# olehskip/resnet.c

Measured on AMD Instinct MI355X. Metric: images/sec ResNet-50 224x224 fp32 batch=256, higher is better.
Workload: dtype f32; 1 GPU; resnet50 fp32 forward, batch 256 per GPU, 224x224 (BASELINE.json configs[2]); global_batch=256, batch_per_gpu=256, mode=fused conv+bn+relu(+add) epilogues, streams_per_gpu=2, streams_configured=library default, front_parts=1, parallelism=batch split over 1 GPU(s), weights replicated, no collective

## Files before the change

### include/rn_hip.h

```cpp
#ifndef RN_HIP_H
#define RN_HIP_H

#include <stddef.h>
#include <stdint.h>

#ifdef __cplusplus
extern "C" {
#endif

#if defined(__GNUC__)
#define RN_API __attribute__((visibility("default")))
#else
#define RN_API
#endif

typedef struct rn_ctx rn_ctx;
typedef struct rn_model rn_model;
typedef struct rn_event rn_event;

enum {
    RN_OK = 0,
    RN_ERR_INVALID = 1,
    RN_ERR_HIP = 2,
    RN_ERR_IO = 3,
    RN_ERR_NOMEM = 4,
    RN_ERR_UNSUPPORTED = 5
};

enum { RN_LAYOUT_NCHW = 0, RN_LAYOUT_NHWC = 1 };

enum { RN_DTYPE_F32 = 0, RN_DTYPE_BF16 = 1 };

enum {
    RN_FWD_REFERENCE_OPS = 0,
    RN_FWD_FUSED = 1
};

RN_API int rn_ctx_create(rn_ctx **out, int device, void *hip_stream );
RN_API int rn_ctx_destroy(rn_ctx *ctx);
RN_API int rn_ctx_set_layout(rn_ctx *ctx, int layout);
RN_API int rn_ctx_get_layout(const rn_ctx *ctx);
RN_API int rn_ctx_set_sync_each_op(rn_ctx *ctx, int on);
RN_API int rn_ctx_set_deferred(rn_ctx *ctx, int on);
RN_API int rn_ctx_get_deferred(const rn_ctx *ctx);
RN_API int rn_flush(rn_ctx *ctx);
RN_API int rn_observe(rn_ctx *ctx, const void *dev_ptr);
RN_API int rn_ctx_deferred_stats(const rn_ctx *ctx, uint64_t *pending_ops, uint64_t *nhwc_buffers,
                                 uint64_t *fused_launches, uint64_t *literal_launches,
                                 uint64_t *transposes);
RN_API int rn_ctx_set_weight_cache(rn_ctx *ctx, int on);
RN_API uint64_t rn_ctx_launch_count(const rn_ctx *ctx);
RN_API int rn_conv_tile_candidates(void);
RN_API int rn_ctx_set_conv_tile(rn_ctx *ctx, int candidate);
RN_API int rn_ctx_set_split_k(rn_ctx *ctx, int max_splits);
RN_API int rn_ctx_set_stem_items(rn_ctx *ctx, int items);
RN_API int rn_ctx_set_xcd_groups(rn_ctx *ctx, int groups);
RN_API int rn_ctx_set_nchw_taps(rn_ctx *ctx, int mode);
RN_API int rn_ctx_set_tap_skip(rn_ctx *ctx, int mode);
RN_API int rn_ctx_tap_skip_stats(const rn_ctx *ctx, uint64_t *launches, uint64_t *k_tiles_skipped);
RN_API int rn_conv_tap_skip_plan(int dtype, uint64_t B, uint64_t in_channels, uint64_t out_channels, uint64_t H,
                                 uint64_t W, uint64_t kernel_size, uint64_t stride, uint64_t padding,
                                 uint64_t dilation, int tile, uint64_t *m_tiles, uint64_t *k_tiles,
                                 uint64_t *k_tiles_skipped, int *rule);
RN_API int rn_ctx_set_debug_stamps(rn_ctx *ctx, void *dev_buffer);
RN_API void *rn_ctx_stream(rn_ctx *ctx);
RN_API int rn_ctx_device(const rn_ctx *ctx);
RN_API int rn_sync(rn_ctx *ctx);
RN_API const char *rn_last_error(const rn_ctx *ctx);
RN_API const char *rn_status_string(int status);
RN_API int rn_device_count(int *count);
RN_API int rn_device_locality(int device, char *pci_bus_id, uint64_t pci_cap, int *numa_node,
                              char *cpulist, uint64_t cpulist_cap);
RN_API const char *rn_version(void);

RN_API int rn_malloc(rn_ctx *ctx, void **dev_ptr, uint64_t bytes);
RN_API int rn_free(rn_ctx *ctx, void *dev_ptr);
RN_API int rn_memcpy_h2d(rn_ctx *ctx, void *dev_dst, const void *host_src, uint64_t bytes);
RN_API int rn_memcpy_d2h(rn_ctx *ctx, void *host_dst, const void *dev_src, uint64_t bytes);
RN_API int rn_memcpy_d2d(rn_ctx *ctx, void *dev_dst, const void *dev_src, uint64_t bytes);
RN_API int rn_memset(rn_ctx *ctx, void *dev_ptr, int byte_value, uint64_t bytes);
RN_API int rn_load_f32_file(rn_ctx *ctx, const char *path, float **dev_ptr, uint64_t *numel);
RN_API int rn_save_f32_file(rn_ctx *ctx, const char *path, const float *dev_ptr, uint64_t numel);

RN_API int rn_event_create(rn_ctx *ctx, rn_event **out);
RN_API int rn_event_destroy(rn_event *ev);
RN_API int rn_event_record(rn_ctx *ctx, rn_event *ev);
RN_API int rn_event_elapsed_ms(rn_event *start, rn_event *stop, float *ms);

RN_API uint64_t rn_conv_output_size(uint64_t x, uint64_t kernel_size, uint64_t stride,
                                    uint64_t padding);
RN_API int rn_conv2d_forward(rn_ctx *ctx, const float *inp, float *out, const float *weight,
                             uint64_t kernel_size, uint64_t stride, uint64_t padding,
                             uint64_t h_out, uint64_t w_out, uint64_t B, uint64_t in_channels,
                             uint64_t out_channels, uint64_t H, uint64_t W);
RN_API int rn_maxpool2d_forward(rn_ctx *ctx, const float *inp, float *out, uint64_t kernel_size,
                                uint64_t stride, uint64_t padding, uint64_t h_out, uint64_t w_out,
                                uint64_t B, uint64_t channels, uint64_t H, uint64_t W);
RN_API int rn_avgpool2d_forward(rn_ctx *ctx, const float *inp, float *out, uint64_t kernel_size,
                                uint64_t stride, uint64_t padding, uint64_t h_out, uint64_t w_out,
                                uint64_t B, uint64_t channels, uint64_t H, uint64_t W);
RN_API int rn_linear_forward(rn_ctx *ctx, const float *inp, float *out, const float *weight,
                             const float *bias , uint64_t B, uint64_t in_features,
                             uint64_t out_features);
RN_API int rn_relu_forward(rn_ctx *ctx, const float *inp, float *out, uint64_t N);
RN_API int rn_batchnorm2d_forward(rn_ctx *ctx, const float *inp, float *out, const float *weight,
                                  const float *bias, const float *mean, const float *var,
                                  uint64_t B, uint64_t C, uint64_t N);
RN_API int rn_add_forward(rn_ctx *ctx, const float *inp1, const float *inp2, float *out,
                          uint64_t N);
RN_API int rn_argmax_forward(rn_ctx *ctx, const float *logits, uint64_t *idx, uint64_t B,
                             uint64_t classes);

RN_API int rn_softmax_forward(rn_ctx *ctx, const float *logits, float *probs, uint64_t B, uint64_t classes);
RN_API int rn_topk_forward(rn_ctx *ctx, const float *x, float *values, uint64_t *indices, uint64_t B,
                           uint64_t classes, uint64_t k);
RN_API int rn_softmax_topk_forward(rn_ctx *ctx, const float *logits, float *probs , float *topk_prob,
                                   uint64_t *topk_idx, uint64_t B, uint64_t classes, uint64_t k);

RN_API int rn_nchw_to_nhwc(rn_ctx *ctx, const float *src, float *dst, uint64_t B, uint64_t C,
                           uint64_t H, uint64_t W);
RN_API int rn_nhwc_to_nchw(rn_ctx *ctx, const float *src, float *dst, uint64_t B, uint64_t C,
                           uint64_t H, uint64_t W);
RN_API int rn_nhwc_to_nchw_dt(rn_ctx *ctx, int dtype, const void *src_nhwc, float *dst_nchw, uint64_t B,
                              uint64_t C, uint64_t H, uint64_t W);
RN_API uint64_t rn_conv2d_input_channels(uint64_t in_channels);
RN_API int rn_nchw_to_nhwc_pad(rn_ctx *ctx, const float *src, float *dst, uint64_t B, uint64_t C,
                               uint64_t H, uint64_t W, uint64_t Cpad);
RN_API uint64_t rn_conv2d_packed_weight_numel(uint64_t in_channels, uint64_t out_channels,
                                              uint64_t kernel_size);
RN_API int rn_conv2d_pack_weight(rn_ctx *ctx, const float *weight_oihw, float *packed,
                                 uint64_t in_channels, uint64_t out_channels,
                                 uint64_t kernel_size);
RN_API int rn_batchnorm2d_fold(rn_ctx *ctx, const float *weight, const float *bias,
                               const float *mean, const float *var, float *scale, float *shift,
                               uint64_t C);

typedef struct rn_epilogue {
    const float *scale;
    const float *shift;
    const void *residual;
    int relu;
} rn_epilogue;

RN_API int rn_conv2d_nhwc_forward(rn_ctx *ctx, const float *inp, float *out,
                                  const float *packed_weight, uint64_t kernel_size,
                                  uint64_t stride, uint64_t padding, uint64_t h_out,
                                  uint64_t w_out, uint64_t B, uint64_t in_channels,
                                  uint64_t out_channels, uint64_t H, uint64_t W,
                                  const rn_epilogue *epilogue );

RN_API uint64_t rn_conv2d_packed_weight_numel_dt(int dtype, uint64_t in_channels,
                                                 uint64_t out_channels, uint64_t kernel_size);
RN_API int rn_conv2d_pack_weight_dt(rn_ctx *ctx, int dtype, const float *weight_oihw, void *packed,
                                    uint64_t in_channels, uint64_t out_channels,
                                    uint64_t kernel_size);
RN_API int rn_nchw_to_nhwc_pad_dt(rn_ctx *ctx, int dtype, const float *src, void *dst, uint64_t B,
                                  uint64_t C, uint64_t H, uint64_t W, uint64_t Cpad,
                                  uint64_t border);
RN_API int rn_image_u8_to_nhwc_pad_dt(rn_ctx *ctx, int dtype, const uint8_t *img, void *dst,
                                      uint64_t B, uint64_t H, uint64_t W, uint64_t Cpad,
                                      uint64_t border, const float mean[3], const float std[3]);
RN_API int rn_resize_crop_geometry(uint64_t H, uint64_t W, uint64_t resize, uint64_t crop, uint64_t *nh,
                                   uint64_t *nw, uint64_t *top, uint64_t *left);
RN_API int rn_resize_coefficients(uint64_t in_size, uint64_t out_size, uint64_t first, uint64_t count,
                                  int32_t *bounds_out, int32_t *coeffs_out, uint64_t cap, uint64_t *ksize);
RN_API int rn_image_u8_resize_crop(rn_ctx *ctx, const uint8_t *packed_dev, const uint64_t *offsets,
                                   const uint64_t *heights, const uint64_t *widths, uint64_t B,
                                   uint8_t *dst_dev, uint64_t resize, uint64_t crop);
RN_API int rn_image_u8_resize_crop_table(const uint64_t *offsets, const uint64_t *heights,
                                         const uint64_t *widths, uint64_t B, uint64_t resize, uint64_t crop,
                                         void *table, uint64_t cap, uint64_t *bytes);
RN_API int rn_image_u8_resize_crop_launch(rn_ctx *ctx, const uint8_t *packed_dev, const void *table_dev,
                                          uint64_t B, uint8_t *dst_dev, uint64_t crop);
RN_API int rn_conv2d_nhwc_forward_dt(rn_ctx *ctx, int dtype, int out_dtype, const void *inp,
                                     void *out, const void *packed_weight, uint64_t kernel_size,
                                     uint64_t stride, uint64_t padding, uint64_t h_out,
                                     uint64_t w_out, uint64_t B, uint64_t in_channels,
                                     uint64_t out_channels, uint64_t H, uint64_t W,
                                     const rn_epilogue *epilogue );
RN_API int rn_maxpool2d_nhwc_forward_dt(rn_ctx *ctx, int dtype, const void *inp, void *out,
                                        uint64_t kernel_size, uint64_t stride, uint64_t padding,
                                        uint64_t h_out, uint64_t w_out, uint64_t B,
                                        uint64_t channels, uint64_t H, uint64_t W);
RN_API int rn_avgpool2d_nhwc_forward_dt(rn_ctx *ctx, int dtype, const void *inp, void *out,
                                        uint64_t kernel_size, uint64_t stride, uint64_t padding,
                                        uint64_t h_out, uint64_t w_out, uint64_t B,
                                        uint64_t channels, uint64_t H, uint64_t W);
RN_API int rn_global_avgpool_nhwc_forward_dt(rn_ctx *ctx, int dtype, const void *inp, void *out, uint64_t B,
                                             uint64_t channels, uint64_t H, uint64_t W);

RN_API int rn_conv2d_grouped_forward(rn_ctx *ctx, const float *inp, float *out, const float *weight,
                                     uint64_t kernel_size, uint64_t stride, uint64_t padding,
                                     uint64_t h_out, uint64_t w_out, uint64_t B, uint64_t in_channels,
                                     uint64_t out_channels, uint64_t H, uint64_t W, uint64_t groups);
RN_API uint64_t rn_conv2d_grouped_packed_weight_numel_dt(int dtype, uint64_t in_channels,
                                                         uint64_t out_channels, uint64_t kernel_size,
                                                         uint64_t groups);
RN_API int rn_conv2d_grouped_pack_weight_dt(rn_ctx *ctx, int dtype, const float *weight_oihw,
                                            void *packed, uint64_t in_channels, uint64_t out_channels,
                                            uint64_t kernel_size, uint64_t groups);
RN_API int rn_conv2d_grouped_nhwc_forward_dt(rn_ctx *ctx, int dtype, int out_dtype, const void *inp,
                                             void *out, const void *packed_weight, uint64_t kernel_size,
                                             uint64_t stride, uint64_t padding, uint64_t h_out,
                                             uint64_t w_out, uint64_t B, uint64_t in_channels,
                                             uint64_t out_channels, uint64_t H, uint64_t W,
                                             uint64_t groups, const rn_epilogue *epilogue );

#define RN_CONV_MAX_DILATION 1024
RN_API uint64_t rn_conv_output_size_dilated(uint64_t x, uint64_t kernel_size, uint64_t stride,
                                            uint64_t padding, uint64_t dilation);
RN_API int rn_conv2d_dilated_forward(rn_ctx *ctx, const float *inp, float *out, const float *weight,
                                     uint64_t kernel_size, uint64_t stride, uint64_t padding,
                                     uint64_t dilation, uint64_t h_out, uint64_t w_out, uint64_t B,
                                     uint64_t in_channels, uint64_t out_channels, uint64_t H, uint64_t W,
                                     uint64_t groups);
RN_API int rn_conv2d_dilated_nhwc_forward_dt(rn_ctx *ctx, int dtype, int out_dtype, const void *inp,
                                             void *out, const void *packed_weight, uint64_t kernel_size,
                                             uint64_t stride, uint64_t padding, uint64_t dilation,
                                             uint64_t h_out, uint64_t w_out, uint64_t B,
// ... 226 lines not shown
```

### resnet.c_amd/_lib.py

```python
from __future__ import annotations

import ctypes
import os
from ctypes import POINTER, c_char_p, c_double, c_float, c_int, c_uint64, c_void_p

_HERE = os.path.dirname(os.path.abspath(__file__))
LIB_PATH = os.environ.get("RN_HIP_LIB") or os.path.join(_HERE, "librn_hip.so")

RN_OK = 0
RN_ERR_INVALID, RN_ERR_HIP, RN_ERR_IO, RN_ERR_NOMEM, RN_ERR_UNSUPPORTED = 1, 2, 3, 4, 5
RN_LAYOUT_NCHW, RN_LAYOUT_NHWC = 0, 1
RN_FWD_REFERENCE_OPS, RN_FWD_FUSED = 0, 1
RN_DTYPE_F32, RN_DTYPE_BF16 = 0, 1
RN_CONV_MAX_DILATION = 1024

u64 = c_uint64
fptr = c_void_p


class ConvSecond(ctypes.Structure):
    _fields_ = [("inp", c_void_p), ("in_channels", c_uint64), ("H", c_uint64), ("W", c_uint64),
                ("stride", c_uint64)]


class ModelOutputs(ctypes.Structure):
    _fields_ = [("logits", c_void_p), ("features", c_void_p), ("probs", c_void_p), ("topk_prob", c_void_p),
                ("topk_idx", c_void_p), ("k", c_uint64)]


class ModelMaps(ctypes.Structure):
    _fields_ = [("layer", c_void_p * 4)]


class SegOutputs(ctypes.Structure):
    _fields_ = [("labels", c_void_p), ("scores", c_void_p)]


class FpnOutputs(ctypes.Structure):
    _fields_ = [("level", c_void_p * 5)]


class Epilogue(ctypes.Structure):
    _fields_ = [("scale", c_void_p), ("shift", c_void_p), ("residual", c_void_p),
                ("relu", c_int)]


SIGNATURES = {
    "rn_ctx_create": (c_int, [POINTER(c_void_p), c_int, c_void_p]),
    "rn_ctx_destroy": (c_int, [c_void_p]),
    "rn_ctx_set_layout": (c_int, [c_void_p, c_int]),
    "rn_ctx_get_layout": (c_int, [c_void_p]),
    "rn_ctx_set_sync_each_op": (c_int, [c_void_p, c_int]),
    "rn_ctx_set_deferred": (c_int, [c_void_p, c_int]),
    "rn_ctx_get_deferred": (c_int, [c_void_p]),
    "rn_flush": (c_int, [c_void_p]),
    "rn_observe": (c_int, [c_void_p, c_void_p]),
    "rn_ctx_deferred_stats": (c_int, [c_void_p] + [POINTER(u64)] * 5),
    "rn_ctx_set_weight_cache": (c_int, [c_void_p, c_int]),
    "rn_ctx_launch_count": (u64, [c_void_p]),
    "rn_conv_tile_candidates": (c_int, []),
    "rn_ctx_set_conv_tile": (c_int, [c_void_p, c_int]),
    "rn_ctx_set_split_k": (c_int, [c_void_p, c_int]),
    "rn_ctx_set_stem_items": (c_int, [c_void_p, c_int]),
    "rn_ctx_set_xcd_groups": (c_int, [c_void_p, c_int]),
    "rn_ctx_set_nchw_taps": (c_int, [c_void_p, c_int]),
    "rn_ctx_set_tap_skip": (c_int, [c_void_p, c_int]),
    "rn_ctx_tap_skip_stats": (c_int, [c_void_p, POINTER(u64), POINTER(u64)]),
    "rn_conv_tap_skip_plan": (c_int, [c_int] + [u64] * 9 + [c_int] + [POINTER(u64)] * 3 + [POINTER(c_int)]),
    "rn_ctx_set_debug_stamps": (c_int, [c_void_p, c_void_p]),
    "rn_ctx_stream": (c_void_p, [c_void_p]),
    "rn_ctx_device": (c_int, [c_void_p]),
    "rn_sync": (c_int, [c_void_p]),
    "rn_last_error": (c_char_p, [c_void_p]),
    "rn_status_string": (c_char_p, [c_int]),
    "rn_device_count": (c_int, [POINTER(c_int)]),
    "rn_device_locality": (c_int, [c_int, c_char_p, u64, POINTER(c_int), c_char_p, u64]),
    "rn_version": (c_char_p, []),
    "rn_malloc": (c_int, [c_void_p, POINTER(c_void_p), u64]),
    "rn_free": (c_int, [c_void_p, c_void_p]),
    "rn_memcpy_h2d": (c_int, [c_void_p, c_void_p, c_void_p, u64]),
    "rn_memcpy_d2h": (c_int, [c_void_p, c_void_p, c_void_p, u64]),
    "rn_memcpy_d2d": (c_int, [c_void_p, c_void_p, c_void_p, u64]),
    "rn_memset": (c_int, [c_void_p, c_void_p, c_int, u64]),
    "rn_load_f32_file": (c_int, [c_void_p, c_char_p, POINTER(c_void_p), POINTER(u64)]),
    "rn_save_f32_file": (c_int, [c_void_p, c_char_p, c_void_p, u64]),
    "rn_event_create": (c_int, [c_void_p, POINTER(c_void_p)]),
    "rn_event_destroy": (c_int, [c_void_p]),
    "rn_event_record": (c_int, [c_void_p, c_void_p]),
    "rn_event_elapsed_ms": (c_int, [c_void_p, c_void_p, POINTER(c_float)]),
    "rn_conv_output_size": (u64, [u64, u64, u64, u64]),
    "rn_conv2d_forward": (c_int, [c_void_p, fptr, fptr, fptr] + [u64] * 10),
    "rn_maxpool2d_forward": (c_int, [c_void_p, fptr, fptr] + [u64] * 9),
    "rn_avgpool2d_forward": (c_int, [c_void_p, fptr, fptr] + [u64] * 9),
    "rn_linear_forward": (c_int, [c_void_p, fptr, fptr, fptr, fptr] + [u64] * 3),
    "rn_relu_forward": (c_int, [c_void_p, fptr, fptr, u64]),
    "rn_batchnorm2d_forward": (c_int, [c_void_p] + [fptr] * 6 + [u64] * 3),
    "rn_add_forward": (c_int, [c_void_p, fptr, fptr, fptr, u64]),
    "rn_argmax_forward": (c_int, [c_void_p, fptr, c_void_p, u64, u64]),
    "rn_softmax_forward": (c_int, [c_void_p, fptr, fptr, u64, u64]),
    "rn_topk_forward": (c_int, [c_void_p, fptr, fptr, c_void_p, u64, u64, u64]),
    "rn_softmax_topk_forward": (c_int, [c_void_p, fptr, fptr, fptr, c_void_p, u64, u64, u64]),
    "rn_nchw_to_nhwc": (c_int, [c_void_p, fptr, fptr] + [u64] * 4),
    "rn_nhwc_to_nchw": (c_int, [c_void_p, fptr, fptr] + [u64] * 4),
    "rn_nhwc_to_nchw_dt": (c_int, [c_void_p, c_int, fptr, fptr] + [u64] * 4),
    "rn_conv2d_input_channels": (u64, [u64]),
    "rn_nchw_to_nhwc_pad": (c_int, [c_void_p, fptr, fptr] + [u64] * 5),
    "rn_conv2d_packed_weight_numel": (u64, [u64, u64, u64]),
    "rn_conv2d_pack_weight": (c_int, [c_void_p, fptr, fptr, u64, u64, u64]),
    "rn_batchnorm2d_fold": (c_int, [c_void_p] + [fptr] * 6 + [u64]),
    "rn_conv2d_nhwc_forward": (c_int, [c_void_p, fptr, fptr, fptr] + [u64] * 10
                               + [POINTER(Epilogue)]),
    "rn_conv2d_packed_weight_numel_dt": (u64, [c_int, u64, u64, u64]),
    "rn_conv2d_pack_weight_dt": (c_int, [c_void_p, c_int, fptr, fptr, u64, u64, u64]),
    "rn_nchw_to_nhwc_pad_dt": (c_int, [c_void_p, c_int, fptr, fptr] + [u64] * 6),
    "rn_image_u8_to_nhwc_pad_dt": (c_int, [c_void_p, c_int, c_void_p, c_void_p] + [u64] * 5
                                   + [POINTER(c_float), POINTER(c_float)]),
    "rn_resize_crop_geometry": (c_int, [u64] * 4 + [POINTER(u64)] * 4),
    "rn_resize_coefficients": (c_int, [u64] * 4 + [c_void_p, c_void_p, u64, POINTER(u64)]),
    "rn_image_u8_resize_crop": (c_int, [c_void_p, c_void_p, POINTER(u64), POINTER(u64), POINTER(u64), u64,
                                        c_void_p, u64, u64]),
    "rn_image_u8_resize_crop_table": (c_int, [POINTER(u64), POINTER(u64), POINTER(u64), u64, u64, u64, c_void_p,
                                              u64, POINTER(u64)]),
    "rn_image_u8_resize_crop_launch": (c_int, [c_void_p, c_void_p, c_void_p, u64, c_void_p, u64]),
    "rn_conv2d_nhwc_forward_dt": (c_int, [c_void_p, c_int, c_int, fptr, fptr, fptr] + [u64] * 10
                                  + [POINTER(Epilogue)]),
    "rn_conv2d_grouped_forward": (c_int, [c_void_p, fptr, fptr, fptr] + [u64] * 11),
    "rn_conv2d_grouped_packed_weight_numel_dt": (u64, [c_int, u64, u64, u64, u64]),
    "rn_conv2d_grouped_pack_weight_dt": (c_int, [c_void_p, c_int, fptr, fptr, u64, u64, u64, u64]),
    "rn_conv2d_grouped_nhwc_forward_dt": (c_int, [c_void_p, c_int, c_int, fptr, fptr, fptr] + [u64] * 11
                                          + [POINTER(Epilogue)]),
    "rn_conv_output_size_dilated": (u64, [u64, u64, u64, u64, u64]),
    "rn_conv2d_dilated_forward": (c_int, [c_void_p, fptr, fptr, fptr] + [u64] * 12),
    "rn_conv2d_dilated_nhwc_forward_dt": (c_int, [c_void_p, c_int, c_int, fptr, fptr, fptr] + [u64] * 12
                                          + [POINTER(Epilogue)]),
    "rn_conv2d_packed_weight_numel_exact": (u64, [u64, u64, u64]),
    "rn_conv2d_pack_weight_exact": (c_int, [c_void_p, fptr, fptr, u64, u64, u64]),
    "rn_conv2d_nhwc_exact_forward": (c_int, [c_void_p, fptr, fptr, fptr] + [u64] * 9
                                     + [POINTER(Epilogue)]),
    "rn_conv2d_packed_pair_weight_numel": (u64, [u64, u64, u64, u64]),
    "rn_conv2d_pack_weight_pair_dt": (c_int, [c_void_p, c_int, fptr, fptr, fptr, fptr, fptr]
                                      + [u64] * 4),
    "rn_conv2d_nhwc_pair_forward_dt": (c_int, [c_void_p, c_int, c_int, fptr, fptr, fptr] + [u64] * 10
                                       + [POINTER(ConvSecond), POINTER(Epilogue)]),
    "rn_model_set_pair_fusion": (c_int, [c_void_p, c_int]),
    "rn_model_set_stem_exact": (c_int, [c_void_p, c_int]),
    "rn_stem_pool_packed_weight_numel": (u64, [c_int]),
    "rn_stem_pool_pack_weight_dt": (c_int, [c_void_p, c_int, fptr, fptr, u64]),
    "rn_stem_pool_forward_dt": (c_int, [c_void_p, c_int, fptr, fptr, fptr, fptr, fptr, c_int, u64, u64, u64]),
    "rn_stem_pool_nchw_forward_dt": (c_int, [c_void_p, c_int, fptr, fptr, fptr, fptr, fptr, c_int, u64, u64, u64, u64]),
    "rn_stem_conv_pool_nchw_forward": (c_int, [c_void_p] + [fptr] * 6 + [u64] * 4),
    "rn_conv_chain_forward_dt": (c_int, [c_void_p, c_int] + [fptr] * 10 + [u64] * 4),
    "rn_conv_chain_pair_forward_dt": (c_int, [c_void_p, c_int] + [fptr] * 9 + [u64] * 5),
    "rn_model_set_chain": (c_int, [c_void_p, c_int]),
    "rn_model_set_stem_pool_fusion": (c_int, [c_void_p, c_int]),
    "rn_model_set_streams": (c_int, [c_void_p, c_int]),
    "rn_model_get_streams": (c_int, [c_void_p]),
    "rn_model_parts": (c_int, [c_void_p, u64]),
    "rn_model_set_front_parts": (c_int, [c_void_p, c_int]),
    "rn_maxpool2d_nhwc_forward_dt": (c_int, [c_void_p, c_int, fptr, fptr] + [u64] * 9),
    "rn_avgpool2d_nhwc_forward_dt": (c_int, [c_void_p, c_int, fptr, fptr] + [u64] * 9),
    "rn_global_avgpool_nhwc_forward_dt": (c_int, [c_void_p, c_int, fptr, fptr] + [u64] * 4),
    "rn_model_set_input_size": (c_int, [c_void_p, u64, u64]),
    "rn_model_input_size": (c_int, [c_void_p, POINTER(u64), POINTER(u64)]),
    "rn_model_max_sub_batch": (u64, [c_void_p]),
    "rn_model_set_dilation": (c_int, [c_void_p, c_int, c_int, c_int]),
    "rn_model_dilation": (c_int, [c_void_p, POINTER(c_int)]),
    "rn_model_output_stride": (c_int, [c_void_p]),
    "rn_model_create": (c_int, [c_void_p, POINTER(c_void_p), c_int]),
    "rn_model_create_ex": (c_int, [c_void_p, POINTER(c_void_p), c_int, c_int, c_int]),
    "rn_model_set_dtype": (c_int, [c_void_p, c_int]),
    "rn_model_set_classes": (c_int, [c_void_p, u64]),
    "rn_model_classes": (u64, [c_void_p]),
    "rn_model_features": (u64, [c_void_p]),
    "rn_model_forward_outputs": (c_int, [c_void_p, fptr, u64, POINTER(ModelOutputs), c_int]),
    "rn_model_forward_outputs_u8": (c_int, [c_void_p, c_void_p, u64, POINTER(ModelOutputs), c_int]),
    "rn_model_stage_shape": (c_int, [c_void_p, c_int, POINTER(u64), POINTER(u64), POINTER(u64)]),
    "rn_model_forward_maps": (c_int, [c_void_p, fptr, u64, POINTER(ModelOutputs), POINTER(ModelMaps), c_int]),
    "rn_model_forward_maps_u8": (c_int, [c_void_p, c_void_p, u64, POINTER(ModelOutputs), POINTER(ModelMaps), c_int]),
    "rn_upsample_bilinear_forward": (c_int, [c_void_p, fptr] + [u64] * 7 + [fptr, c_void_p]),
    "rn_seg_head_create": (c_int, [c_void_p, POINTER(c_void_p), u64, u64, u64]),
    "rn_concat_channels_forward_dt": (c_int, [c_void_p, c_int, u64, POINTER(c_void_p), POINTER(u64), c_void_p, u64,
                                              c_void_p, u64, u64]),
    "rn_seg_head_create_deeplab": (c_int, [c_void_p, POINTER(c_void_p), u64, u64, u64, u64, POINTER(u64)]),
    "rn_seg_head_set_center_tap": (c_int, [c_void_p, c_int]),
    "rn_seg_head_set_dtype": (c_int, [c_void_p, c_int]),
    "rn_seg_head_set_tensor": (c_int, [c_void_p, c_char_p, c_void_p, u64]),
    "rn_seg_head_finalize": (c_int, [c_void_p]),
    "rn_seg_head_destroy": (c_int, [c_void_p]),
    "rn_seg_head_forward": (c_int, [c_void_p, c_void_p] + [u64] * 5 + [fptr, c_void_p]),
    "rn_model_forward_segment": (c_int, [c_void_p, c_void_p, fptr, u64, POINTER(ModelOutputs), POINTER(SegOutputs),
                                         c_int]),
    "rn_model_forward_segment_u8": (c_int, [c_void_p, c_void_p, c_void_p, u64, POINTER(ModelOutputs),
                                            POINTER(SegOutputs), c_int]),
    "rn_upsample_nearest_add_forward_dt": (c_int, [c_void_p, c_int, c_void_p] + [u64] * 4 + [c_void_p, c_void_p, u64, u64]),
    "rn_fpn_create": (c_int, [c_void_p, POINTER(c_void_p), u64, POINTER(u64), u64, c_int]),
    "rn_fpn_set_dtype": (c_int, [c_void_p, c_int]),
    "rn_fpn_set_tensor": (c_int, [c_void_p, c_char_p, c_void_p, u64]),
    "rn_fpn_finalize": (c_int, [c_void_p]),
    "rn_fpn_destroy": (c_int, [c_void_p]),
    "rn_fpn_level_shape": (c_int, [c_void_p, c_int, u64, u64, POINTER(u64), POINTER(u64), POINTER(u64)]),
    "rn_fpn_forward": (c_int, [c_void_p, POINTER(c_void_p), u64, POINTER(u64), POINTER(u64), POINTER(c_void_p)]),
    "rn_model_forward_fpn": (c_int, [c_void_p, c_void_p, fptr, u64, POINTER(ModelOutputs), POINTER(c_int),
                                     POINTER(FpnOutputs), c_int]),
    "rn_model_forward_fpn_u8": (c_int, [c_void_p, c_void_p, c_void_p, u64, POINTER(ModelOutputs), POINTER(c_int),
                                        POINTER(FpnOutputs), c_int]),
    "rn_model_destroy": (c_int, [c_void_p]),
    "rn_model_set_tensor": (c_int, [c_void_p, c_char_p, c_void_p, u64]),
    "rn_model_load_dir": (c_int, [c_void_p, c_char_p]),
    "rn_model_finalize": (c_int, [c_void_p]),
    "rn_model_tensor_key": (c_char_p, [c_void_p, u64, POINTER(u64)]),
    "rn_model_forward": (c_int, [c_void_p, fptr, u64, fptr, c_int]),
    "rn_model_forward_u8": (c_int, [c_void_p, c_void_p, u64, fptr, c_int]),
    "rn_model_forward_images_u8": (c_int, [c_void_p, c_void_p, POINTER(u64), POINTER(u64), POINTER(u64), u64, fptr,
                                           c_int]),
    "rn_model_tune": (c_int, [c_void_p, fptr, u64, fptr, c_int]),
    "rn_model_export_tuning": (c_int, [c_void_p, POINTER(u64), u64, POINTER(u64)]),
    "rn_model_import_tuning": (c_int, [c_void_p, POINTER(u64), u64]),
    "rn_model_set_profiling": (c_int, [c_void_p, c_int]),
    "rn_model_profile_count": (u64, [c_void_p]),
    "rn_model_profile_get": (c_int, [c_void_p, u64, POINTER(c_char_p), POINTER(c_char_p),
                                     POINTER(c_float), POINTER(c_double), POINTER(c_double)]),
# ... 99 lines not shown
```

### resnet.c_amd/csrc/rn_conv.hip

```cpp
#include <type_traits>

#include "rn_conv_params.h"
#include "rn_private.h"

bool rn_conv_is_c4(uint64_t Cin, uint64_t k);

using namespace rn_gemm;

namespace {

constexpr int ROW_FLOATS = 32;

constexpr int tile_blocks_per_cu(int BM, int BN) { return BM * BN <= 64 * 64 ? 4 : BM * BN <= 64 * 128 ? 3 : 2; }

template <typename T, typename TO, int BM, int BN, bool DUAL = false, bool XK = false, bool CHUNK = false,
          bool DIL = false, bool PM = false>
__global__ __launch_bounds__(256, tile_blocks_per_cu(BM, BN)) void conv_gemm_kernel(const GemmParams p)
{
    constexpr int CH = Elem<T>::CH, ES = (int)sizeof(T);
    constexpr int AP = BM / 32;
    constexpr int BP = BN / 32;
    constexpr int MI = BM / 64;
    constexpr int NI = BN / 64;
    constexpr int STAGE = (BM + BN) * ROW_FLOATS;
// ... 604 lines not shown
            q /= (uint64_t)p.Wo;
            oh = (int)(q % (uint64_t)p.Ho);
            b = q / (uint64_t)p.Ho;
        } else {
            ow = (int)(i % (uint64_t)p.Wo);
            uint64_t q = i / (uint64_t)p.Wo;
            oh = (int)(q % (uint64_t)p.Ho);
            q /= (uint64_t)p.Ho;
            oc = (int)(q % (uint64_t)p.Cout);
            b = q / (uint64_t)p.Cout;
        }
        const int ih0 = oh * p.stride - p.pad, iw0 = ow * p.stride - p.pad;
        float sum = 0.f;
        for (int ic = 0; ic < p.Cin; ++ic) {
            for (int kh = 0; kh < p.k; ++kh) {
                const int ih = ih0 + kh * p.dil;
                if (ih < 0 || ih >= p.H) continue;
                for (int kw = 0; kw < p.k; ++kw) {
                    const int iw = iw0 + kw * p.dil;
                    if (iw < 0 || iw >= p.W) continue;
                    const uint64_t ii = p.nhwc ? (((b * p.H + ih) * p.W + iw) * p.Cs + ic)
                                               : (((b * p.Cin + ic) * p.H + ih) * p.W + iw);
                    uint64_t wi;
                    if (p.w_packed == 0)
                        wi = (((uint64_t)oc * p.Cin + ic) * p.k + kh) * p.k + kw;
                    else if (p.w_packed == 1)
                        wi = (((uint64_t)oc * p.k + kh) * p.k + kw) * p.Cin + ic;
                    else
                        wi = (((uint64_t)oc * p.k + kh) * 8 + kw) * 4 + ic;
                    sum = fmaf(p.in[ii], p.w[wi], sum);
                }
            }
        }
        if (p.scale) {
            sum = fmaf(sum, p.scale[oc], p.shift ? p.shift[oc] : 0.f);
        } else if (p.shift) {
            sum += p.shift[oc];
        }
        if (p.residual) sum += p.residual[i];
        if (p.relu) sum = fmaxf(sum, 0.f);
        p.out[i] = sum;
    }
}

struct FinishParams {
    const float *partial;
    void *out;
    const float *scale, *shift;
    const void *residual;
    int relu, splits, Cout;
    uint64_t slice;
    uint64_t stride;
};

template <typename TO>
__global__ __launch_bounds__(256) void splitk_finish_kernel(const FinishParams p)
{
    const uint64_t n4 = p.slice / 4, gstride = (uint64_t)gridDim.x * 256;
    for (uint64_t i = (uint64_t)blockIdx.x * 256 + threadIdx.x; i < n4; i += gstride) {
        float4 v = *reinterpret_cast<const float4 *>(p.partial + 4 * i);
        for (int s = 1; s < p.splits; ++s) {
            const float4 x = *reinterpret_cast<const float4 *>(p.partial + (uint64_t)s * p.stride + 4 * i);
            v.x += x.x, v.y += x.y, v.z += x.z, v.w += x.w;
        }
        const int n = (int)((4 * i) % (uint64_t)p.Cout);
        float y[4] = {v.x, v.y, v.z, v.w};
#pragma unroll
        for (int j = 0; j < 4; ++j) {
            const float sc = p.scale ? p.scale[n + j] : 1.f;
            const float sh = p.shift ? p.shift[n + j] : -0.f;
            float r = fmaf(y[j], sc, sh);
            if (p.residual) r += OutVec<TO>::load1(p.residual, 4 * i + j);
            y[j] = p.relu ? fmaxf(r, 0.f) : r;
        }
#pragma unroll
        for (int j = 0; j < 4; ++j) OutVec<TO>::store1(p.out, 4 * i + j, y[j]);
    }
}

bool fits_i32(uint64_t v) { return v < (1ull << 31); }

template <typename P>
void set_epilogue(P &p, const rn_epilogue *ep)
{
    p.scale = ep ? ep->scale : nullptr;
    p.shift = ep ? ep->shift : nullptr;
    p.residual = ep ? static_cast<decltype(p.residual)>(ep->residual) : nullptr;
    p.relu = ep ? ep->relu : 0;
}

struct Contraction {
    int dt_in, dt_out;
    const void *inp;
    void *out;
    const void *packed;
    uint64_t k, stride, pad, dil, h_out, w_out, B, Cin, Cout, H, W;
    const rn_epilogue *ep;
    const rn_conv_second *second;
    bool exact;
    bool out_nchw;
    const char *what;
};

GemmParams describe(const rn_ctx *ctx, const Contraction &d)
{
    const int es = d.dt_in == RN_DTYPE_BF16 ? 2 : 4;
    const int bke = 128 / es;
    const uint64_t k = d.k, Cin = d.Cin;
    GemmParams p{};
    p.out_nchw = d.out_nchw && d.dt_out == RN_DTYPE_F32 && !(d.ep && d.ep->residual) && d.h_out * d.w_out > 1;
    p.in = d.inp, p.w = d.packed, p.out = d.out;
    set_epilogue(p, d.ep);
    const bool c4 = !d.exact && rn_conv_is_c4(Cin, k);
    p.H = (int)d.H, p.W = (int)d.W, p.Cs = c4 ? 4 : (int)Cin;
    p.Ho = (int)d.h_out, p.Wo = (int)d.w_out, p.Cout = (int)d.Cout;
    const bool c4pair = c4 && d.dt_in == RN_DTYPE_BF16;
    p.tap_rows = c4pair ? 2 : 1, p.k_rows = (int)k;
    p.KH = c4pair ? (int)rn_ceil_div(k, 2) : (int)k;
    p.KW = c4 ? 1 : (int)k;
    p.stride = (int)d.stride, p.pad = (int)d.pad;
    p.dil = (int)d.dil;
    p.cseg = c4 ? 1 : (int)(Cin / bke);
    p.chunk_dw = c4 ? 16 / (4 * es) : 0;
    p.c4_chunks = c4 ? (int)rn_ceil_div(k, p.chunk_dw) : 0;
    p.M = (int)(d.B * d.h_out * d.w_out);
    p.nk = p.KH * p.KW * p.cseg;
    p.nk1 = p.nk;
    if (const rn_conv_second *s = d.second) {
        p.in2 = s->inp;
        p.H2 = (int)s->H, p.W2 = (int)s->W, p.Cs2 = (int)s->in_channels, p.stride2 = (int)s->stride;
        p.in2_bytes = (int)(d.B * s->H * s->W * s->in_channels * es);
        p.nk += (int)(s->in_channels / bke);
    }
    p.Ktot = p.nk * bke;
    if (d.exact) {
        p.kreal = (int)(k * k * Cin), p.kc = (int)(k * Cin), p.kskip = (int)((d.W - k) * Cin);
        p.nk = p.nk1 = (int)rn_ceil_div((uint64_t)p.kreal, 32);
        p.Ktot = p.nk * 32, p.cseg = 1;
        rn_fast_div((unsigned)p.kc, &p.mul_kc, &p.shr_kc);
    }
    p.HoWo = p.Ho * p.Wo;
    rn_fast_div((unsigned)p.HoWo, &p.mul_hw, &p.shr_hw);
    rn_fast_div((unsigned)p.Wo, &p.mul_w, &p.shr_w);
    rn_fast_div((unsigned)p.cseg, &p.mul_cs, &p.shr_cs);
    rn_fast_div((unsigned)p.KW, &p.mul_kw, &p.shr_kw);
    p.stamps = (unsigned long long *)ctx->debug_stamps;
    p.in_bytes = (int)(d.B * d.H * d.W * (uint64_t)p.Cs * es);
    p.w_bytes = (int)(d.Cout * (uint64_t)p.Ktot * es);
    p.out_bytes = (int)(d.B * d.h_out * d.w_out * d.Cout * (uint64_t)(d.dt_out == RN_DTYPE_BF16 ? 2 : 4));
    return p;
}

struct Choice {
    enum Family { STRIP, WIDE, FOUR_WAVE } family;
    int which;
    int BM, BN;
    bool persistent;
    bool chunked;
    bool pm;
};

Choice choose_four_wave(int conv_tile, const Contraction &d, const GemmParams &p)
{
    static const int cand[4][2] = {{128, 128}, {128, 64}, {64, 128}, {64, 64}};
    static const double eff_f32[4] = {0.84, 0.95, 0.96, 1.00}, eff_bf16[4] = {1.00, 0.92, 0.95, 0.80};
    const double *cand_eff = d.dt_in == RN_DTYPE_BF16 ? eff_bf16 : eff_f32;
    Choice c{};
    c.family = Choice::FOUR_WAVE, c.BM = c.BN = 128;
    if (conv_tile >= 1 && conv_tile <= 8) {
        c.BM = cand[(conv_tile - 1) & 3][0], c.BN = cand[(conv_tile - 1) & 3][1];
        c.persistent = conv_tile > 4;
    } else {
        double best = 1e300;
        for (int ci = 0; ci < 4; ++ci) {
            const uint64_t tm = rn_ceil_div((uint64_t)p.M, cand[ci][0]);
            const uint64_t tn = rn_ceil_div(d.Cout, cand[ci][1]);
            const double rounds = (double)rn_ceil_div(tm * tn, 256);
            const double cost = rounds * cand[ci][0] * cand[ci][1] / cand_eff[ci];
            if (cost < best * 0.999) {
                best = cost;
                c.BM = cand[ci][0], c.BN = cand[ci][1];
            }
        }
        c.persistent = true;
    }
    const bool chunk_bf16 = d.dt_in == RN_DTYPE_BF16 && d.dt_out == RN_DTYPE_F32;
    c.chunked = ((d.dt_in == RN_DTYPE_F32 && d.dt_out == RN_DTYPE_F32) || chunk_bf16) && !d.second && !d.exact &&
                p.nk >= 32 && d.Cout % 4 == 0;
    if (c.chunked && c.BM == 128 && c.BN == 128) c.BN = 64;
    if (c.chunked && chunk_bf16) c.BM = c.BN = 64;
    return c;
}

Choice choose(const rn_ctx *ctx, const Contraction &d, const GemmParams &p)
{
    if (d.dt_in == RN_DTYPE_BF16 && d.dt_out == RN_DTYPE_BF16 && ctx->split_k <= 1) {
        const int nwide = rn_conv_wide_count();
        Choice c{};
        if ((ctx->conv_tile == 9 + nwide || (ctx->conv_tile == 0 && p.M >= 256 * 256)) && d.second == nullptr &&
            rn_conv_strip_eligible(p)) {
            c.family = Choice::STRIP;
            return c;
        }
        c.family = Choice::WIDE, c.which = -1;
        if (ctx->conv_tile > 8 && ctx->conv_tile <= 8 + nwide) {
            if (rn_conv_wide_eligible(p, ctx->conv_tile - 9)) c.which = ctx->conv_tile - 9;
        } else if (ctx->conv_tile == 0 && p.nk >= 8 && d.Cout >= 128) {
            static const double eff_wide[6] = {1.00, 0.80, 0.80, 0.50, 0.90, 0.55};
            double best = 1e300;
            for (int wi = 0; wi < nwide; ++wi) {
                int bm, bn;
                rn_conv_wide_tile(wi, &bm, &bn);
                if (!rn_conv_wide_eligible(p, wi) || (uint64_t)bn > 2 * d.Cout) continue;
                const uint64_t tiles = rn_ceil_div((uint64_t)p.M, bm) * rn_ceil_div(d.Cout, bn);
                if (tiles < 128) continue;
                const double cost = (double)rn_ceil_div(tiles, 256) * bm * bn / eff_wide[wi];
                if (cost < best * 0.999) {
                    best = cost;
                    c.which = wi;
                }
            }
        }
        if (c.which >= 0) {
            rn_conv_wide_tile(c.which, &c.BM, &c.BN);
            return c;
        }
    }
    return choose_four_wave(ctx->conv_tile, d, p);
}

struct TapSkipPlan {
    bool eligible;
    bool rule;
    uint64_t m_tiles, k_tiles, k_skipped;
};

constexpr double kTapSkipMinShare = 0.02, kTapSkipMaxWaste = 0.02;
constexpr uint64_t kTapSkipMinStridedPixels = 784;

TapSkipPlan plan_tap_skip(const Contraction &d, const GemmParams &p, int BM, int BN, bool split_k)
{
    TapSkipPlan t{};
    if (d.dt_in != RN_DTYPE_F32 || d.dt_out != RN_DTYPE_F32 || d.k <= 1 || d.pad == 0 || d.Cin % 32 != 0 ||
        d.dil != 1 || d.second || d.exact || p.out_nchw || split_k)
        return t;
    uint64_t sum[2] = {0, 0};
    const uint64_t n_out[2] = {d.h_out, d.w_out}, n_in[2] = {d.H, d.W};
    for (int ax = 0; ax < 2; ++ax)
        for (uint64_t o = 0; o < n_out[ax]; ++o) {
            const int64_t x0 = (int64_t)(o * d.stride) - (int64_t)d.pad;
            const int64_t lo = x0 < 0 ? -x0 : 0, hi = (int64_t)n_in[ax] - x0 < (int64_t)d.k ? (int64_t)n_in[ax] - x0 : (int64_t)d.k;
            if (hi <= lo) return t;
            sum[ax] += (uint64_t)(hi - lo);
        }
    const uint64_t blocks = rn_ceil_div(d.B, (uint64_t)BM), tiles_n = rn_ceil_div(d.Cout, (uint64_t)BN);
    const uint64_t pixels = d.h_out * d.w_out, cseg = d.Cin / 32;
    t.eligible = true;
    t.m_tiles = pixels * blocks;
    t.k_tiles = t.m_tiles * tiles_n * (d.k * d.k * cseg);
    t.k_skipped = blocks * tiles_n * cseg * (pixels * d.k * d.k - sum[0] * sum[1]);
    const double share = (double)t.k_skipped / (double)t.k_tiles;
    const double waste = 1.0 - (double)d.B / (double)(blocks * (uint64_t)BM);
    t.rule = share >= kTapSkipMinShare && waste <= kTapSkipMaxWaste &&
             (d.stride == 1 || pixels >= kTapSkipMinStridedPixels);
    return t;
}

bool split_whole_tiles(GemmParams &p, int BM, int BN)
{
    p.tiles_n = (int)rn_ceil_div((uint64_t)p.Cout, BN);
    const uint64_t total = rn_ceil_div((uint64_t)p.M, BM) * (uint64_t)p.tiles_n;
    if (!fits_i32(total)) return false;
    p.total_tiles = p.total_work = p.grid_items = p.full_tiles = (unsigned)total;
    p.ksplit = 1, p.kchunk = p.chunk_L = p.nk;
    return true;
}

bool split_pixel_major(GemmParams &p, const Contraction &d, int BM, int BN)
{
    p.tiles_n = (int)rn_ceil_div((uint64_t)p.Cout, BN);
    const uint64_t total = (uint64_t)p.HoWo * rn_ceil_div(d.B, (uint64_t)BM) * (uint64_t)p.tiles_n;
    if (!fits_i32(total * (uint64_t)BM / (uint64_t)p.tiles_n)) return false;
    if (!fits_i32(total)) return false;
    p.total_tiles = p.total_work = p.grid_items = p.full_tiles = (unsigned)total;
    p.ksplit = 1, p.kchunk = p.nk;
    return true;
}

FinishParams finish_params(const Contraction &d, const void *partial, int splits, uint64_t row0, uint64_t slice)
{
    const uint64_t skip = row0 * d.Cout * (d.dt_out == RN_DTYPE_BF16 ? 2 : 4);
    FinishParams f{};
    set_epilogue(f, d.ep);
    f.partial = (const float *)partial;
    f.out = (char *)d.out + skip;
    if (f.residual) f.residual = (const char *)f.residual + skip;
    f.splits = splits, f.Cout = (int)d.Cout, f.slice = f.stride = slice;
    return f;
}

int split_k_loop(rn_ctx *ctx, const Contraction &d, GemmParams &p, FinishParams *fin)
{
    if (!(ctx->split_k > 1 && p.total_tiles < 512 && p.nk >= 8 && d.Cout % 4 == 0 && !p.out_nchw &&
          !(d.second && d.dt_in == RN_DTYPE_BF16)))
        return RN_OK;
    int S = (int)rn_ceil_div(1024, p.total_tiles);
    if (S > ctx->split_k) S = ctx->split_k;
    if (S > p.nk / 4) S = p.nk / 4;
    if (S <= 1) return RN_OK;
    const int chunk = (int)rn_ceil_div((uint64_t)p.nk, (uint64_t)S);
    S = (int)rn_ceil_div((uint64_t)p.nk, (uint64_t)chunk);
    const uint64_t slice = (uint64_t)p.M * d.Cout;
    void *ws = nullptr;
    RN_TRY(rn_scratch(ctx, 4, (uint64_t)S * slice * sizeof(float), &ws));
    *fin = finish_params(d, ws, S, 0, slice);
    p.out = ws;
    set_epilogue(p, nullptr);
    p.ksplit = S, p.kchunk = chunk;
    p.total_work = p.grid_items = p.total_tiles * (unsigned)S;
    p.split_stride = (long long)(slice * sizeof(float));
    p.out_bytes = (int)(slice * sizeof(float));
    return RN_OK;
}

int split_chunked_tail(rn_ctx *ctx, const Contraction &d, int BM, GemmParams &p, FinishParams *fin)
{
    p.chunk_L = 2 * (int)rn_ceil_div((uint64_t)p.nk, 16);
    const int S = (int)rn_ceil_div((uint64_t)p.nk, (uint64_t)p.chunk_L);
    unsigned tail = p.total_tiles > 256 ? p.total_tiles % 256 : p.total_tiles;
    tail -= tail % (unsigned)p.tiles_n;
    const bool cut = ctx->split_k <= 1 && tail > 0 && !p.out_nchw &&
                     rn_ceil_div((uint64_t)tail * S, 256) < (uint64_t)S;
    if (!cut) return RN_OK;
    const uint64_t row0 = (uint64_t)((p.total_tiles - tail) / (unsigned)p.tiles_n) * (uint64_t)BM;
    const uint64_t tail_elems = ((uint64_t)p.M - row0) * d.Cout;
    void *ws = nullptr;
    RN_TRY(rn_scratch(ctx, 4, (uint64_t)S * tail_elems * sizeof(float), &ws));
    *fin = finish_params(d, ws, S, row0, tail_elems);
    p.ws = reinterpret_cast<void *>(reinterpret_cast<uintptr_t>(ws) - row0 * d.Cout * sizeof(float));
    p.ws_stride = (long long)(tail_elems * sizeof(float));
    p.tail_tiles = tail, p.full_tiles = p.total_tiles - tail;
    p.total_work = p.grid_items = p.full_tiles + tail * (unsigned)S;
    return RN_OK;
}

void choose_tile_order(rn_ctx *ctx, GemmParams &p, unsigned remap_tiles, int BM, int BN)
{
    const unsigned tn = (unsigned)p.tiles_n;
    if (tn < 2 || remap_tiles < 8 * tn) return;
    int groups = ctx->xcd_groups;
    if (groups <= 0) {
        const double es = p.w_bytes / ((double)p.Cout * p.Ktot);
        const double w_slab = (double)BN * p.Ktot * es;
        const double a_slab = (double)BM * es * (p.Cs + (p.in2 ? p.Cs2 : 0));
        const double R = 32.0 * tile_blocks_per_cu(BM, BN);
        const double A = (double)p.in_bytes + (p.in2 ? (double)p.in2_bytes / (p.stride2 * p.stride2) : 0.0);
        const double Wb = (double)p.w_bytes, MB = 1024.0 * 1024.0;
        const double panels = (double)(remap_tiles / tn);
        const bool taps = p.KH * p.KW > 1;
        auto cost = [&](int g) {
            const double nt = (double)tn / g, mp = R / nt < 1 ? 1 : R / nt;
            const bool stays = taps ? nt * w_slab + mp * a_slab <= 3.8 * MB : nt * w_slab <= 2.5 * MB;
            const double generations = panels / (8.0 / g) / mp;
            const double again = stays ? 1.0 : 3.0 * (generations < 1 ? 1 : generations);
            if (taps && !stays && g > 1) return 1e300;
            return (g > 1 ? 1.3 : 1.0) * g * A + 8.0 * (Wb / g) * again;
        };
        groups = 1;
        double best = cost(1);
        for (int g = 2; g <= 8; g *= 2) {
            if (tn % (unsigned)g) break;
            const double c = cost(g);
            if (c < 0.8 * best) best = c, groups = g;
        }
    }
    if (groups > 8) groups = 8;
    while (groups > 1 && tn % (unsigned)groups) groups /= 2;
    if (groups <= 1) return;
    p.xg = (int)(tn / (unsigned)groups);
    p.xrows = remap_tiles / tn;
}

template <typename T, typename TO, int BM, int BN, bool DUAL, bool XK, bool CHUNK, bool DIL, bool PM>
void launch_one(rn_ctx *ctx, const GemmParams &p, bool persistent, int *occupancy)
{
    unsigned grid = p.grid_items;
    if (persistent) {
        if (*occupancy == 0) {
            int nb = 0;
            if (hipOccupancyMaxActiveBlocksPerMultiprocessor(
                    &nb, conv_gemm_kernel<T, TO, BM, BN, DUAL, XK, CHUNK, DIL, PM>, 256, 0) != hipSuccess ||
                nb < 1)
                nb = 1;
            *occupancy = nb;
        }
        const unsigned slots = 256u * (unsigned)*occupancy;
        if (grid > slots) grid = slots;
    }
    conv_gemm_kernel<T, TO, BM, BN, DUAL, XK, CHUNK, DIL, PM><<<dim3(grid), dim3(256), 0, ctx->stream>>>(p);
}

struct KernelRow {
    int dt_in, dt_out, BM, BN;
    bool dual, xk, chunk, dil, pm;
    void (*launch)(rn_ctx *, const GemmParams &, bool persistent, int *occupancy);
};

template <typename T>
constexpr int dtype_of = std::is_same<T, float>::value ? RN_DTYPE_F32 : RN_DTYPE_BF16;

template <int BM, int BN, typename T, typename TO, bool DUAL = false, bool XK = false, bool CHUNK = false,
          bool DIL = false, bool PM = false>
constexpr KernelRow row()
{
    return {dtype_of<T>, dtype_of<TO>, BM, BN, DUAL, XK, CHUNK, DIL, PM,
            launch_one<T, TO, BM, BN, DUAL, XK, CHUNK, DIL, PM>};
}
#define FOUR_TILES(...) \
    row<128, 128, __VA_ARGS__>(), row<128, 64, __VA_ARGS__>(), row<64, 128, __VA_ARGS__>(), row<64, 64, __VA_ARGS__>()

constexpr KernelRow kKernels[] = {
    FOUR_TILES(float, float, false, false, false, false),   FOUR_TILES(float, float, false, false, false, true),
    FOUR_TILES(float, float, true, false, false, false),    FOUR_TILES(float, float, true, false, false, true),
    FOUR_TILES(float, float, false, true, false, false),
    FOUR_TILES(bf16_t, bf16_t, false, false, false, false), FOUR_TILES(bf16_t, bf16_t, false, false, false, true),
    FOUR_TILES(bf16_t, bf16_t, true, false, false, false),  FOUR_TILES(bf16_t, bf16_t, true, false, false, true),
    FOUR_TILES(bf16_t, float, false, false, false, false),  FOUR_TILES(bf16_t, float, false, false, false, true),
    row<128, 64, float, float, false, false, true, false>(), row<128, 64, float, float, false, false, true, true>(),
    row<64, 128, float, float, false, false, true, false>(), row<64, 128, float, float, false, false, true, true>(),
    row<64, 64, float, float, false, false, true, false>(),  row<64, 64, float, float, false, false, true, true>(),
    row<64, 64, bf16_t, float, false, false, true, false>(), row<64, 64, bf16_t, float, false, false, true, true>(),
    FOUR_TILES(float, float, false, false, false, false, true),
    row<128, 64, float, float, false, false, true, false, true>(),
    row<64, 128, float, float, false, false, true, false, true>(),
    row<64, 64, float, float, false, false, true, false, true>(),
};
#undef FOUR_TILES
static_assert(sizeof(kKernels) / sizeof(kKernels[0]) == RN_CONV_GEMM_KERNELS, "one rn_ctx::occupancy slot per row");

int dispatch(rn_ctx *ctx, const Contraction &d, const Choice &c, const GemmParams &p, bool fp32_partials)
{
    const bool xk = d.exact, dual = d.second && !xk;
    const int dt_out = fp32_partials ? RN_DTYPE_F32 : d.dt_out;
    const bool chunk = c.chunked && !fp32_partials, dil = p.dil != 1 && !xk;
    for (const KernelRow &r : kKernels) {
        if (r.dt_in != d.dt_in || r.dt_out != dt_out || r.BM != c.BM || r.BN != c.BN || r.dual != dual ||
            r.xk != xk || r.chunk != chunk || r.dil != dil || r.pm != c.pm)
            continue;
        r.launch(ctx, p, c.persistent, &ctx->occupancy[&r - kKernels]);
        return rn_after_launch(ctx, d.what);
    }
    if (d.second) return rn_set_error(ctx, RN_ERR_UNSUPPORTED, "%s: fused pair needs equal in/out dtype", d.what);
    return rn_set_error(ctx, RN_ERR_UNSUPPORTED, "%s: dtype combination %d -> %d", d.what, d.dt_in, d.dt_out);
}

int launch_gemm(rn_ctx *ctx, const Contraction &d)
{
    GemmParams p = describe(ctx, d);
    const Choice c = choose(ctx, d, p);
    if (c.family == Choice::STRIP) {
        rn_conv_strip_launch(ctx, p);
        return rn_after_launch(ctx, d.what);
    }
    if (c.family == Choice::FOUR_WAVE && ctx->tap_skip != 1) {
        const TapSkipPlan t = plan_tap_skip(d, p, c.BM, c.BN, ctx->split_k > 1);
        if (t.eligible && (ctx->tap_skip == 2 || t.rule)) {
            Choice cp = c;
            cp.pm = true;
            RN_REQUIRE(ctx, split_pixel_major(p, d, c.BM, c.BN), "too many tiles");
            if (c.chunked) p.chunk_L = 2 * (int)rn_ceil_div((uint64_t)p.nk, 16);
            else p.chunk_L = p.nk;
            choose_tile_order(ctx, p, p.full_tiles, c.BM, c.BN);
            RN_TRY(dispatch(ctx, d, cp, p, false));
            ctx->tap_skip_launches += 1, ctx->tap_skip_k_tiles += t.k_skipped;
            return RN_OK;
        }
    }
    RN_REQUIRE(ctx, split_whole_tiles(p, c.BM, c.BN), "too many tiles");
    if (c.family == Choice::WIDE) {
        rn_conv_wide_launch(ctx, p, c.which, d.second != nullptr);
        return rn_after_launch(ctx, d.what);
    }
    FinishParams fin{};
    RN_TRY(split_k_loop(ctx, d, p, &fin));
    const bool k_split = fin.splits > 0;
    if (!k_split) {
        if (c.chunked) RN_TRY(split_chunked_tail(ctx, d, c.BM, p, &fin));
        choose_tile_order(ctx, p, p.full_tiles, c.BM, c.BN);
    }
    RN_TRY(dispatch(ctx, d, c, p, k_split));
    if (fin.splits == 0) return RN_OK;
    const unsigned fgrid = rn_stream_grid(fin.slice / 4, 256);
    if (d.dt_out == RN_DTYPE_BF16)
        splitk_finish_kernel<bf16_t><<<fgrid, 256, 0, ctx->stream>>>(fin);
    else
        splitk_finish_kernel<float><<<fgrid, 256, 0, ctx->stream>>>(fin);
    return rn_after_launch(ctx, d.what);
}

int launch_direct(rn_ctx *ctx, const float *inp, float *out, const float *w, uint64_t k,
                  uint64_t stride, uint64_t pad, uint64_t h_out, uint64_t w_out, uint64_t B,
                  uint64_t Cin, uint64_t Cs, uint64_t Cout, uint64_t H, uint64_t W, int nhwc,
                  int w_packed, const rn_epilogue *ep, const char *what, uint64_t dil)
{
    DirectParams p;
    p.in = inp, p.w = w, p.out = out;
    set_epilogue(p, ep);
    p.k = (int)k, p.stride = (int)stride, p.pad = (int)pad, p.dil = (int)dil;
    p.Ho = (int)h_out, p.Wo = (int)w_out, p.H = (int)H, p.W = (int)W;
    p.Cin = (int)Cin, p.Cs = (int)Cs, p.Cout = (int)Cout;
    p.nhwc = nhwc, p.w_packed = w_packed;
    p.total = B * Cout * h_out * w_out;
    conv_direct_kernel<<<rn_stream_grid(p.total, 256), 256, 0, ctx->stream>>>(p);
    return rn_after_launch(ctx, what);
}

int check_conv_args(rn_ctx *ctx, const float *inp, const float *out, const float *weight,
                    uint64_t k, uint64_t stride, uint64_t pad, uint64_t h_out, uint64_t w_out,
                    uint64_t B, uint64_t Cin, uint64_t Cout, uint64_t H, uint64_t W)
{
    RN_REQUIRE(ctx, inp && out && weight, "null tensor");
    RN_REQUIRE(ctx, inp != out, "conv2d cannot run in place");
    RN_REQUIRE(ctx, k >= 1 && stride >= 1, "kernel_size and stride must be >= 1");
    RN_REQUIRE(ctx, k < (1u << 12) && stride < (1u << 12) && pad < (1u << 12), "dimension too large");
    const uint64_t cs = Cin < 4 ? 4 : Cin;
    RN_REQUIRE(ctx, fits_i32(B * H * W * cs) && fits_i32(B * h_out * w_out * Cout) &&
                        fits_i32(Cout * k * k * cs + 64),
               "tensor has 2^31 or more elements");
    return RN_OK;
}

bool gemm_eligible(const void *inp, const void *out, const void *w, uint64_t Cin, uint64_t k,
                   uint64_t in_elems, uint64_t w_elems, uint64_t out_elems)
{
    if (in_elems >= (1ull << 29) || w_elems >= (1ull << 29) || out_elems >= (1ull << 29))
        return false;
    const bool al = ((reinterpret_cast<uintptr_t>(inp) | reinterpret_cast<uintptr_t>(out) |
                      reinterpret_cast<uintptr_t>(w)) & 15) == 0;
    return al && k <= 15 && (Cin % 32 == 0 || rn_conv_is_c4(Cin, k));
}

bool epilogue_aligned(const rn_epilogue *ep, uintptr_t mask)
{
    return !ep || ((reinterpret_cast<uintptr_t>(ep->scale) | reinterpret_cast<uintptr_t>(ep->shift) |
                    reinterpret_cast<uintptr_t>(ep->residual)) & mask) == 0;
}

int nhwc_forward(rn_ctx *ctx, const float *inp, float *out, const float *packed_weight,
                 uint64_t kernel_size, uint64_t stride, uint64_t padding, uint64_t dil, uint64_t h_out,
                 uint64_t w_out, uint64_t B, uint64_t in_channels, uint64_t out_channels,
                 uint64_t H, uint64_t W, const rn_epilogue *epilogue)
{
    RN_ENTER(ctx);
    if (B * out_channels * h_out * w_out == 0) return RN_OK;
    RN_TRY(check_conv_args(ctx, inp, out, packed_weight, kernel_size, stride, padding, h_out, w_out,
                           B, in_channels, out_channels, H, W));
    RN_REQUIRE(ctx, in_channels >= 1, "in_channels must be >= 1");
    RN_REQUIRE(ctx, epilogue_aligned(epilogue, 3),
               "misaligned scale / shift / residual (fp32 tensors sit on 4-byte boundaries)");
    if (epilogue_aligned(epilogue, 15) && (dil == 1 || in_channels % 32 == 0) &&
        gemm_eligible(inp, out, packed_weight, in_channels, kernel_size,
                      B * H * W * rn_conv2d_input_channels(in_channels),
                      rn_conv2d_packed_weight_numel(in_channels, out_channels, kernel_size),
                      B * h_out * w_out * out_channels)) {
        Contraction d{};
        d.dt_in = d.dt_out = RN_DTYPE_F32, d.inp = inp, d.out = out, d.packed = packed_weight;
        d.k = kernel_size, d.stride = stride, d.pad = padding, d.dil = dil, d.h_out = h_out, d.w_out = w_out;
        d.B = B, d.Cin = in_channels, d.Cout = out_channels, d.H = H, d.W = W;
        d.ep = epilogue, d.what = "rn_conv2d_nhwc_forward";
        return launch_gemm(ctx, d);
    }
    const bool c4 = rn_conv_is_c4(in_channels, kernel_size);
    return launch_direct(ctx, inp, out, packed_weight, kernel_size, stride, padding, h_out, w_out,
                         B, in_channels, rn_conv2d_input_channels(in_channels), out_channels, H, W,
                         1, c4 ? 2 : 1, epilogue, "rn_conv2d_nhwc_forward(direct)", dil);
}

int conv2d_forward(rn_ctx *ctx, const float *inp, float *out, const float *weight,
                   uint64_t kernel_size, uint64_t stride, uint64_t padding, uint64_t dil, uint64_t h_out,
                   uint64_t w_out, uint64_t B, uint64_t in_channels, uint64_t out_channels,
                   uint64_t H, uint64_t W)
{
    if (!ctx) return RN_ERR_INVALID;
    if (B * out_channels * h_out * w_out == 0) return RN_OK;
    RN_TRY(check_conv_args(ctx, inp, out, weight, kernel_size, stride, padding, h_out, w_out, B,
                           in_channels, out_channels, H, W));
    RN_REQUIRE(ctx, in_channels >= 1, "in_channels must be >= 1");
    if (dil == 1 && RN_DEFERS(ctx))
        return rn_defer_conv(ctx, inp, out, weight, kernel_size, stride, padding, h_out, w_out, B, in_channels,
                             out_channels, H, W);
    RN_ENTER(ctx);
    const bool c4 = dil == 1 && rn_conv_is_c4(in_channels, kernel_size);
    const bool fast = (in_channels % 32 == 0 || c4) && kernel_size <= 15 &&
                      B * H * W * rn_conv2d_input_channels(in_channels) < (1ull << 29) &&
                      B * h_out * w_out * out_channels < (1ull << 29) &&
                      rn_conv2d_packed_weight_numel(in_channels, out_channels, kernel_size) <
                          (1ull << 29);
    if (!fast || (ctx->layout == RN_LAYOUT_NHWC && in_channels < 4)) {
        return launch_direct(ctx, inp, out, weight, kernel_size, stride, padding, h_out, w_out, B,
                             in_channels, in_channels, out_channels, H, W,
                             ctx->layout == RN_LAYOUT_NHWC, 0, nullptr,
                             "rn_conv2d_forward(direct)", dil);
    }
    const bool native = dil == 1 && ctx->layout == RN_LAYOUT_NCHW && h_out == (H + 2 * padding - kernel_size) / stride + 1 &&
                        w_out == (W + 2 * padding - kernel_size) / stride + 1 &&
                        rn_conv_nchw_eligible(kernel_size, stride, padding, B, in_channels, out_channels, H, W);
    if (native && kernel_size == 1 && padding == 0 && (reinterpret_cast<uintptr_t>(weight) & 15) == 0)
        return rn_conv_nchw_launch(ctx, inp, out, weight, 1, stride, 0, B, in_channels, out_channels, H, W);
    const bool taps = native && (ctx->nchw_taps >= 2 || (ctx->nchw_taps == 1 && H * W >= 2048));
    const uintptr_t wide = ctx->layout == RN_LAYOUT_NHWC
                               ? (reinterpret_cast<uintptr_t>(inp) | reinterpret_cast<uintptr_t>(out))
                               : reinterpret_cast<uintptr_t>(out);
    if (!taps && (wide & 15) != 0)
        return launch_direct(ctx, inp, out, weight, kernel_size, stride, padding, h_out, w_out, B, in_channels,
                             in_channels, out_channels, H, W, ctx->layout == RN_LAYOUT_NHWC, 0, nullptr,
                             "rn_conv2d_forward(direct)", dil);
    const uint64_t wn = rn_conv2d_packed_weight_numel(in_channels, out_channels, kernel_size);
    void *wp = ctx->wcache_on ? rn_wcache_find(ctx, weight, in_channels, out_channels, kernel_size) : nullptr;
    if (!wp) {
        if (ctx->wcache_on)
            RN_TRY(rn_wcache_add(ctx, weight, in_channels, out_channels, kernel_size, wn * sizeof(float), &wp));
        else
            RN_TRY(rn_scratch(ctx, 1, wn * sizeof(float), &wp));
        const int pst = rn_conv2d_pack_weight(ctx, weight, (float *)wp, in_channels, out_channels, kernel_size);
        if (pst != RN_OK) {
            if (ctx->wcache_on) rn_wcache_remove(ctx, wp);
            return pst;
        }
    }
    Contraction d{};
    d.dt_in = d.dt_out = RN_DTYPE_F32, d.inp = inp, d.out = out, d.packed = wp;
    d.k = kernel_size, d.stride = stride, d.pad = padding, d.dil = dil, d.h_out = h_out, d.w_out = w_out;
    d.B = B, d.Cin = in_channels, d.Cout = out_channels, d.H = H, d.W = W;
    d.what = "rn_conv2d_forward(nhwc)";
    if (ctx->layout == RN_LAYOUT_NHWC) return launch_gemm(ctx, d);
    if (taps)
        return rn_conv_nchw_launch(ctx, inp, out, (const float *)wp, kernel_size, stride, padding, B, in_channels,
                                   out_channels, H, W);
    const uint64_t cs = rn_conv2d_input_channels(in_channels);
    void *xin = nullptr;
    RN_TRY(rn_scratch(ctx, 2, B * H * W * cs * sizeof(float), &xin));
    if (cs != in_channels) {
        RN_TRY(rn_nchw_to_nhwc_pad(ctx, inp, (float *)xin, B, in_channels, H, W, cs));
    } else {
        RN_TRY(rn_nchw_to_nhwc(ctx, inp, (float *)xin, B, in_channels, H, W));
    }
    d.inp = xin, d.out_nchw = true, d.what = "rn_conv2d_forward(gemm)";
    return launch_gemm(ctx, d);
}

int nhwc_forward_dt(rn_ctx *ctx, int dtype, int out_dtype, const void *inp, void *out,
                    const void *packed_weight, uint64_t kernel_size, uint64_t stride,
                    uint64_t padding, uint64_t dil, uint64_t h_out, uint64_t w_out, uint64_t B,
                    uint64_t in_channels, uint64_t out_channels, uint64_t H, uint64_t W,
                    const rn_epilogue *epilogue)
{
    RN_ENTER(ctx);
    if (dtype == RN_DTYPE_F32) {
        RN_REQUIRE(ctx, out_dtype == RN_DTYPE_F32, "fp32 input implies fp32 output");
        return nhwc_forward(ctx, (const float *)inp, (float *)out, (const float *)packed_weight, kernel_size,
                            stride, padding, dil, h_out, w_out, B, in_channels, out_channels, H, W, epilogue);
    }
    RN_REQUIRE(ctx, dtype == RN_DTYPE_BF16, "unknown dtype");
    if (B * out_channels * h_out * w_out == 0) return RN_OK;
    RN_REQUIRE(ctx, inp && out && packed_weight && inp != out, "null or aliased tensor");
    RN_REQUIRE(ctx, kernel_size >= 1 && kernel_size <= 15 && stride >= 1 && stride < (1u << 12) &&
                        padding < (1u << 12),
               "kernel_size / stride / padding out of range");
    const bool c4 = rn_conv_is_c4(in_channels, kernel_size);
    const uint64_t cs = c4 ? 4 : in_channels;
    if (c4 && dil != 1)
        return rn_set_error(ctx, RN_ERR_UNSUPPORTED, "the bf16 small-Cin form has no dilation");
    if (c4) {
        RN_REQUIRE(ctx, padding == 0 && stride % 2 == 0 && W % 2 == 0,
                   "bf16 small-Cin form needs a physically padded image, even stride and width");
    } else if (in_channels % 64 != 0) {
        return rn_set_error(ctx, RN_ERR_UNSUPPORTED,
                            "bf16 convolution needs in_channels %% 64 == 0 (got %llu)",
                            (unsigned long long)in_channels);
    }
    const uint64_t ktot = c4 ? rn_ceil_div(kernel_size, 2) * 64 : kernel_size * kernel_size * in_channels;
    RN_REQUIRE(ctx, B * H * W * cs < (1ull << 30) && out_channels * ktot < (1ull << 30) &&
                        B * h_out * w_out * out_channels < (1ull << 29),
               "tensor too large");
    RN_REQUIRE(ctx, ((reinterpret_cast<uintptr_t>(inp) | reinterpret_cast<uintptr_t>(out) |
                      reinterpret_cast<uintptr_t>(packed_weight)) & 15) == 0,
               "bf16 tensors must be 16-byte aligned");
    RN_REQUIRE(ctx, epilogue_aligned(epilogue, 15), "misaligned scale / shift / residual (16-byte alignment)");
    Contraction d{};
    d.dt_in = RN_DTYPE_BF16, d.dt_out = out_dtype, d.inp = inp, d.out = out, d.packed = packed_weight;
    d.k = kernel_size, d.stride = stride, d.pad = padding, d.dil = dil, d.h_out = h_out, d.w_out = w_out;
    d.B = B, d.Cin = in_channels, d.Cout = out_channels, d.H = H, d.W = W;
    d.ep = epilogue, d.what = "rn_conv2d_nhwc_forward_dt";
    return launch_gemm(ctx, d);
}

int check_dilation(rn_ctx *ctx, uint64_t k, uint64_t stride, uint64_t pad, uint64_t *dil, uint64_t h_out,
                   uint64_t w_out, uint64_t H, uint64_t W)
{
    RN_REQUIRE(ctx, *dil >= 1 && *dil <= RN_CONV_MAX_DILATION, "dilation must be 1..RN_CONV_MAX_DILATION");
    RN_REQUIRE(ctx, k >= 1 && k < (1u << 12) && stride >= 1 && stride < (1u << 12) && pad < (1u << 12),
               "kernel_size / stride / padding out of range");
    RN_REQUIRE(ctx, H < (1ull << 31) && W < (1ull << 31), "dimension too large");
    RN_REQUIRE(ctx, rn_conv_output_size_dilated(H, k, stride, pad, *dil) == h_out &&
                        rn_conv_output_size_dilated(W, k, stride, pad, *dil) == w_out,
               "h_out / w_out are not the dilated convolution's output size");
    if (k == 1) *dil = 1;
    return RN_OK;
}

}

extern "C" {

uint64_t rn_conv_output_size_dilated(uint64_t x, uint64_t kernel_size, uint64_t stride, uint64_t padding,
                                     uint64_t dilation)
{
    if (kernel_size == 0 || stride == 0 || dilation == 0) return 0;
    const uint64_t span = dilation * (kernel_size - 1) + 1;
    if (x + 2 * padding < span) return 0;
    return (x + 2 * padding - span) / stride + 1;
}

int rn_conv_tap_skip_plan(int dtype, uint64_t B, uint64_t in_channels, uint64_t out_channels, uint64_t H, uint64_t W,
                          uint64_t kernel_size, uint64_t stride, uint64_t padding, uint64_t dilation, int tile,
                          uint64_t *m_tiles, uint64_t *k_tiles, uint64_t *k_tiles_skipped, int *rule)
{
    if (m_tiles) *m_tiles = 0;
    if (k_tiles) *k_tiles = 0;
    if (k_tiles_skipped) *k_tiles_skipped = 0;
    if (rule) *rule = 0;
    if ((dtype != RN_DTYPE_F32 && dtype != RN_DTYPE_BF16) || tile < 0 || tile > 8 || B == 0 || in_channels == 0 ||
        out_channels == 0 || kernel_size == 0 || kernel_size > 15 || stride == 0 || dilation == 0)
        return -1;
    const uint64_t h_out = rn_conv_output_size_dilated(H, kernel_size, stride, padding, dilation);
    const uint64_t w_out = rn_conv_output_size_dilated(W, kernel_size, stride, padding, dilation);
    if (h_out == 0 || w_out == 0) return -1;
    if (dtype != RN_DTYPE_F32 || in_channels % 32 != 0 ||
        !gemm_eligible(nullptr, nullptr, nullptr, in_channels, kernel_size, B * H * W * in_channels,
                       out_channels * kernel_size * kernel_size * in_channels, B * h_out * w_out * out_channels))
        return 0;
    Contraction d{};
    d.dt_in = d.dt_out = dtype;
    d.k = kernel_size, d.stride = stride, d.pad = padding, d.dil = kernel_size == 1 ? 1 : dilation;
    d.h_out = h_out, d.w_out = w_out, d.B = B, d.Cin = in_channels, d.Cout = out_channels, d.H = H, d.W = W;
    rn_ctx none{};
    const GemmParams p = describe(&none, d);
    const Choice c = choose_four_wave(tile, d, p);
    const TapSkipPlan t = plan_tap_skip(d, p, c.BM, c.BN, false);
    if (!t.eligible) return 0;
    if (m_tiles) *m_tiles = t.m_tiles;
    if (k_tiles) *k_tiles = t.k_tiles;
    if (k_tiles_skipped) *k_tiles_skipped = t.k_skipped;
    if (rule) *rule = t.rule ? 1 : 0;
    return 1;
}

int rn_conv2d_nhwc_forward(rn_ctx *ctx, const float *inp, float *out, const float *packed_weight,
                           uint64_t kernel_size, uint64_t stride, uint64_t padding, uint64_t h_out,
                           uint64_t w_out, uint64_t B, uint64_t in_channels, uint64_t out_channels,
                           uint64_t H, uint64_t W, const rn_epilogue *epilogue)
{
    return nhwc_forward(ctx, inp, out, packed_weight, kernel_size, stride, padding, 1, h_out, w_out, B, in_channels,
                        out_channels, H, W, epilogue);
}

int rn_conv2d_forward(rn_ctx *ctx, const float *inp, float *out, const float *weight,
                      uint64_t kernel_size, uint64_t stride, uint64_t padding, uint64_t h_out,
                      uint64_t w_out, uint64_t B, uint64_t in_channels, uint64_t out_channels,
                      uint64_t H, uint64_t W)
{
    return conv2d_forward(ctx, inp, out, weight, kernel_size, stride, padding, 1, h_out, w_out, B, in_channels,
                          out_channels, H, W);
}

int rn_conv2d_nhwc_forward_dt(rn_ctx *ctx, int dtype, int out_dtype, const void *inp, void *out,
                              const void *packed_weight, uint64_t kernel_size, uint64_t stride,
                              uint64_t padding, uint64_t h_out, uint64_t w_out, uint64_t B,
                              uint64_t in_channels, uint64_t out_channels, uint64_t H, uint64_t W,
                              const rn_epilogue *epilogue)
{
    return nhwc_forward_dt(ctx, dtype, out_dtype, inp, out, packed_weight, kernel_size, stride, padding, 1, h_out,
                           w_out, B, in_channels, out_channels, H, W, epilogue);
}

int rn_conv2d_dilated_forward(rn_ctx *ctx, const float *inp, float *out, const float *weight, uint64_t kernel_size,
                              uint64_t stride, uint64_t padding, uint64_t dilation, uint64_t h_out, uint64_t w_out,
                              uint64_t B, uint64_t in_channels, uint64_t out_channels, uint64_t H, uint64_t W,
                              uint64_t groups)
{
    if (!ctx) return RN_ERR_INVALID;
    RN_TRY(check_dilation(ctx, kernel_size, stride, padding, &dilation, h_out, w_out, H, W));
    if (groups != 1)
        return rn_conv_group_forward(ctx, inp, out, weight, kernel_size, stride, padding, dilation, h_out, w_out, B,
                                     in_channels, out_channels, H, W, groups);
    return conv2d_forward(ctx, inp, out, weight, kernel_size, stride, padding, dilation, h_out, w_out, B, in_channels,
                          out_channels, H, W);
}

int rn_conv2d_dilated_nhwc_forward_dt(rn_ctx *ctx, int dtype, int out_dtype, const void *inp, void *out,
                                      const void *packed_weight, uint64_t kernel_size, uint64_t stride,
                                      uint64_t padding, uint64_t dilation, uint64_t h_out, uint64_t w_out, uint64_t B,
                                      uint64_t in_channels, uint64_t out_channels, uint64_t H, uint64_t W,
                                      uint64_t groups, const rn_epilogue *epilogue)
{
    if (!ctx) return RN_ERR_INVALID;
    RN_TRY(check_dilation(ctx, kernel_size, stride, padding, &dilation, h_out, w_out, H, W));
    if (groups != 1)
        return rn_conv_group_nhwc_forward_dt(ctx, dtype, out_dtype, inp, out, packed_weight, kernel_size, stride,
                                             padding, dilation, h_out, w_out, B, in_channels, out_channels, H, W,
                                             groups, epilogue);
    return nhwc_forward_dt(ctx, dtype, out_dtype, inp, out, packed_weight, kernel_size, stride, padding, dilation,
                           h_out, w_out, B, in_channels, out_channels, H, W, epilogue);
}

int rn_conv_dense_nhwc_forward_dt(rn_ctx *ctx, int dtype, int out_dtype, const void *inp, void *out,
                                  const void *packed_weight, uint64_t kernel_size, uint64_t stride, uint64_t padding,
                                  uint64_t dilation, uint64_t h_out, uint64_t w_out, uint64_t B, uint64_t in_channels,
                                  uint64_t out_channels, uint64_t H, uint64_t W, const rn_epilogue *epilogue)
{
    return nhwc_forward_dt(ctx, dtype, out_dtype, inp, out, packed_weight, kernel_size, stride, padding, dilation,
                           h_out, w_out, B, in_channels, out_channels, H, W, epilogue);
}

int rn_conv2d_nhwc_exact_forward(rn_ctx *ctx, const float *inp_padded, float *out,
                                 const float *packed_exact_weight, uint64_t kernel_size,
                                 uint64_t stride, uint64_t h_out, uint64_t w_out, uint64_t B,
                                 uint64_t in_channels, uint64_t out_channels, uint64_t Hp,
                                 uint64_t Wp, const rn_epilogue *epilogue)
{
    RN_ENTER(ctx);
    if (B * out_channels * h_out * w_out == 0) return RN_OK;
    RN_REQUIRE(ctx, inp_padded && out && packed_exact_weight && inp_padded != out,
               "null or aliased tensor");
    RN_REQUIRE(ctx, kernel_size >= 1 && kernel_size <= 15 && stride >= 1 && stride < (1u << 12) &&
                        in_channels >= 1 && in_channels <= 16,
               "kernel_size / stride / in_channels out of range");
    RN_REQUIRE(ctx, Hp >= kernel_size && Wp >= kernel_size &&
                        rn_conv_output_size(Hp, kernel_size, stride, 0) == h_out &&
                        rn_conv_output_size(Wp, kernel_size, stride, 0) == w_out,
               "h_out / w_out do not match the padded image");
    const uint64_t ktot = rn_ceil_div(kernel_size * kernel_size * in_channels, 32) * 32;
    RN_REQUIRE(ctx, B * Hp * Wp * in_channels < (1ull << 29) && out_channels * ktot < (1ull << 29) &&
                        B * h_out * w_out * out_channels < (1ull << 29),
               "tensor too large");
    RN_REQUIRE(ctx, ((reinterpret_cast<uintptr_t>(out) |
                      reinterpret_cast<uintptr_t>(packed_exact_weight)) & 15) == 0 &&
                        (reinterpret_cast<uintptr_t>(inp_padded) & 3) == 0,
               "misaligned tensor");
    RN_REQUIRE(ctx, epilogue_aligned(epilogue, 15), "misaligned scale / shift / residual (16-byte alignment)");
    Contraction d{};
    d.dt_in = d.dt_out = RN_DTYPE_F32, d.inp = inp_padded, d.out = out, d.packed = packed_exact_weight;
    d.k = kernel_size, d.stride = stride, d.pad = 0, d.dil = 1, d.h_out = h_out, d.w_out = w_out;
    d.B = B, d.Cin = in_channels, d.Cout = out_channels, d.H = Hp, d.W = Wp;
    d.ep = epilogue, d.exact = true, d.what = "rn_conv2d_nhwc_exact_forward";
    return launch_gemm(ctx, d);
}

int rn_conv2d_nhwc_pair_forward_dt(rn_ctx *ctx, int dtype, int out_dtype, const void *inp, void *out,
                                   const void *packed_pair_weight, uint64_t kernel_size,
                                   uint64_t stride, uint64_t padding, uint64_t h_out,
                                   uint64_t w_out, uint64_t B, uint64_t in_channels,
                                   uint64_t out_channels, uint64_t H, uint64_t W,
                                   const rn_conv_second *second, const rn_epilogue *epilogue)
{
    RN_ENTER(ctx);
    RN_REQUIRE(ctx, second && second->inp, "second source missing");
    RN_REQUIRE(ctx, dtype == RN_DTYPE_F32 || dtype == RN_DTYPE_BF16, "unknown dtype");
    RN_REQUIRE(ctx, out_dtype == dtype, "the fused pair keeps one element type");
    if (B * out_channels * h_out * w_out == 0) return RN_OK;
    RN_REQUIRE(ctx, inp && out && packed_pair_weight && inp != out && second->inp != out,
               "null or aliased tensor");
    RN_REQUIRE(ctx, kernel_size >= 1 && kernel_size <= 15 && stride >= 1 && stride < (1u << 12) &&
                        padding < (1u << 12) && second->stride >= 1 && second->stride < (1u << 12),
               "kernel_size / stride / padding out of range");
    const uint64_t seg = dtype == RN_DTYPE_BF16 ? 64 : 32;
    if (in_channels % seg != 0 || second->in_channels % seg != 0 || in_channels == 0 ||
        second->in_channels == 0)
        return rn_set_error(ctx, RN_ERR_UNSUPPORTED,
                            "fused pair needs both channel counts to be multiples of %llu",
                            (unsigned long long)seg);
    RN_REQUIRE(ctx, rn_conv_output_size(H, kernel_size, stride, padding) == h_out &&
                        rn_conv_output_size(W, kernel_size, stride, padding) == w_out,
               "h_out / w_out do not match the first convolution");
    RN_REQUIRE(ctx, rn_conv_output_size(second->H, 1, second->stride, 0) == h_out &&
                        rn_conv_output_size(second->W, 1, second->stride, 0) == w_out,
               "the second (1x1) convolution has a different output size");
    const uint64_t ktot = kernel_size * kernel_size * in_channels + second->in_channels;
    RN_REQUIRE(ctx, B * H * W * in_channels < (1ull << 29) &&
                        B * second->H * second->W * second->in_channels < (1ull << 29) &&
                        out_channels * ktot < (1ull << 29) &&
                        B * h_out * w_out * out_channels < (1ull << 29),
               "tensor too large");
    RN_REQUIRE(ctx, ((reinterpret_cast<uintptr_t>(inp) | reinterpret_cast<uintptr_t>(out) |
                      reinterpret_cast<uintptr_t>(packed_pair_weight) |
                      reinterpret_cast<uintptr_t>(second->inp)) & 15) == 0,
               "tensors must be 16-byte aligned");
    RN_REQUIRE(ctx, epilogue_aligned(epilogue, 15), "misaligned scale / shift / residual (16-byte alignment)");
    Contraction d{};
    d.dt_in = dtype, d.dt_out = out_dtype, d.inp = inp, d.out = out, d.packed = packed_pair_weight;
    d.k = kernel_size, d.stride = stride, d.pad = padding, d.dil = 1, d.h_out = h_out, d.w_out = w_out;
    d.B = B, d.Cin = in_channels, d.Cout = out_channels, d.H = H, d.W = W;
    d.ep = epilogue, d.second = second, d.what = "rn_conv2d_nhwc_pair_forward_dt";
    return launch_gemm(ctx, d);
}

int rn_linear_forward(rn_ctx *ctx, const float *inp, float *out, const float *weight,
// ... 44 lines not shown
```

### resnet.c_amd/csrc/rn_conv_params.h

```cpp
#ifndef RN_CONV_PARAMS_H
#define RN_CONV_PARAMS_H

#include "rn_internal.h"

namespace rn_gemm {

typedef float f32x16 __attribute__((ext_vector_type(16)));
typedef unsigned int u32x4 __attribute__((ext_vector_type(4)));

struct GemmParams {
    const void *in;
    const void *w;
    void *out;
    const float *scale;
    const float *shift;
    const void *residual;
    int relu;
    int H, W, Cs;
    int Ho, Wo, Cout;
    int KH, KW;
    int stride, pad;
    int cseg;
    int chunk_dw;
    int c4_chunks;
    int tap_rows, k_rows;
    int M;
    int Ktot;
    int nk;
    int tiles_n;
    unsigned total_tiles;
    int xg;
    unsigned xrows;
    int HoWo;
    unsigned mul_hw, shr_hw, mul_w, shr_w;
    unsigned mul_cs, shr_cs, mul_kw, shr_kw;
    int in_bytes, w_bytes, out_bytes;
    const void *in2;
    int in2_bytes, H2, W2, Cs2, stride2, nk1;
    int ksplit, kchunk;
    unsigned total_work;
    unsigned grid_items;
    long long split_stride;
    int chunk_L;
    unsigned full_tiles, tail_tiles;
    void *ws;
    long long ws_stride;
    int kc, kskip, kreal;
    unsigned mul_kc, shr_kc;
    int out_nchw;
    unsigned long long *stamps;
    int dil;
};

typedef __bf16 bf16_t;
typedef bf16_t bf16x8 __attribute__((ext_vector_type(8)));

template <typename T>
struct Elem;
template <>
struct Elem<float> {
    static constexpr int CH = 4;
};
template <>
struct Elem<bf16_t> {
    static constexpr int CH = 8;
};

#ifdef __HIPCC__
__device__ __forceinline__ int tap_mask(int x0, int K, int X, int d)
{
    int m = 0;
    for (int t = 0; t < K; ++t) {
        const int x = x0 + t * d;
        if (x >= 0 && x < X) m |= 1 << t;
    }
    return m;
}
#endif

}

#include "rn_tile.h"

inline void rn_fast_div(unsigned d, unsigned *mul, unsigned *shr)
{
    if (d <= 1) {
        *mul = 0;
        *shr = 0;
        return;
    }
    unsigned lg = 0;
    while ((1u << lg) < d) ++lg;
    const unsigned p = 31 + lg;
    const uint64_t m = ((1ull << p) + d - 1) / d;
    *mul = (unsigned)m;
    *shr = p - 32;
}

int rn_conv_wide_count(void);
bool rn_conv_wide_eligible(const rn_gemm::GemmParams &p, int which);
void rn_conv_wide_tile(int which, int *bm, int *bn);
void rn_conv_wide_launch(rn_ctx *ctx, rn_gemm::GemmParams &p, int which, bool dual);
bool rn_conv_strip_eligible(const rn_gemm::GemmParams &p);
void rn_conv_strip_launch(rn_ctx *ctx, const rn_gemm::GemmParams &p);

bool rn_conv_nchw_eligible(uint64_t kernel_size, uint64_t stride, uint64_t padding, uint64_t B, uint64_t Cin,
                           uint64_t Cout, uint64_t H, uint64_t W);
int rn_conv_nchw_launch(rn_ctx *ctx, const float *inp, float *out, const float *weight, uint64_t kernel_size,
                        uint64_t stride, uint64_t padding, uint64_t B, uint64_t Cin, uint64_t Cout, uint64_t H, uint64_t W);

#endif
```

### resnet.c_amd/csrc/rn_ctx.hip

```cpp
#include <errno.h>
#include <stdarg.h>
#include <stdio.h>
#include <stdlib.h>
#include <string.h>

#include "rn_conv_params.h"
#include "rn_private.h"

int rn_set_error(rn_ctx *ctx, int status, const char *fmt, ...)
{
    if (ctx) {
        va_list ap;
        va_start(ap, fmt);
        vsnprintf(ctx->err, sizeof(ctx->err), fmt, ap);
        va_end(ap);
    }
    return status;
}

int rn_check_hip(rn_ctx *ctx, hipError_t e, const char *what)
{
    if (e == hipSuccess) return RN_OK;
    return rn_set_error(ctx, RN_ERR_HIP, "HIP error %d (%s) in %s", (int)e, hipGetErrorString(e),
                        what);
// ... 33 lines not shown
{
    for (int i = 0; i < ctx->wcache_n; ++i) {
        const rn_wcache_entry &e = ctx->wcache[i];
        if (e.key == weight && e.cin == cin && e.cout == cout && e.k == k) return e.packed;
    }
    return nullptr;
}

int rn_wcache_add(rn_ctx *ctx, const void *weight, uint64_t cin, uint64_t cout, uint64_t k,
                  uint64_t bytes, void **packed)
{
    if (ctx->wcache_n == ctx->wcache_cap) {
        const int ncap = ctx->wcache_cap ? 2 * ctx->wcache_cap : 64;
        rn_wcache_entry *ne = (rn_wcache_entry *)realloc(ctx->wcache, (size_t)ncap * sizeof(rn_wcache_entry));
        if (!ne) return rn_set_error(ctx, RN_ERR_NOMEM, "weight cache table");
        ctx->wcache = ne;
        ctx->wcache_cap = ncap;
    }
    void *p = nullptr;
    RN_HIP_TRY(ctx, hipMalloc(&p, bytes));
    rn_wcache_entry &e = ctx->wcache[ctx->wcache_n++];
    e.key = weight;
    e.cin = cin;
    e.cout = cout;
    e.k = k;
    e.packed = p;
    *packed = p;
    return RN_OK;
}

void rn_wcache_remove(rn_ctx *ctx, const void *packed)
{
    for (int i = 0; i < ctx->wcache_n; ++i) {
        if (ctx->wcache[i].packed != packed) continue;
        (void)hipStreamSynchronize(ctx->stream);
        (void)hipFree(ctx->wcache[i].packed);
        ctx->wcache[i] = ctx->wcache[--ctx->wcache_n];
        return;
    }
}

void rn_wcache_drop(rn_ctx *ctx, const void *lo, uint64_t bytes)
{
    const uintptr_t a = (uintptr_t)lo;
    const uintptr_t b = bytes >= ~(uintptr_t)0 - a ? ~(uintptr_t)0 : a + (bytes ? bytes : 1);
    int kept = 0, dropped = 0;
    for (int i = 0; i < ctx->wcache_n; ++i) {
        const rn_wcache_entry &e = ctx->wcache[i];
        const uintptr_t key = (uintptr_t)e.key;
        const uintptr_t end = key + (uintptr_t)(e.cin * e.cout * e.k * e.k * sizeof(float));
        if (key < b && end > a) {
            if (!dropped++) (void)hipStreamSynchronize(ctx->stream);
            (void)hipFree(ctx->wcache[i].packed);
        } else {
            ctx->wcache[kept++] = ctx->wcache[i];
        }
    }
    ctx->wcache_n = kept;
}

int rn_bind_device(rn_ctx *ctx)
{
    int cur = -1;
    if (hipGetDevice(&cur) == hipSuccess && cur == ctx->device) return RN_OK;
    return rn_check_hip(ctx, hipSetDevice(ctx->device), "hipSetDevice");
}

extern "C" {

const char *rn_version(void) { return "resnet.c_amd 0.1 (gfx950)"; }

const char *rn_status_string(int status)
{
    switch (status) {
        case RN_OK: return "ok";
        case RN_ERR_INVALID: return "invalid argument";
        case RN_ERR_HIP: return "HIP runtime error";
        case RN_ERR_IO: return "I/O error";
        case RN_ERR_NOMEM: return "out of memory";
        case RN_ERR_UNSUPPORTED: return "unsupported";
        default: return "unknown status";
    }
}

int rn_device_count(int *count)
{
    if (!count) return RN_ERR_INVALID;
    hipError_t e = hipGetDeviceCount(count);
    if (e != hipSuccess) {
        *count = 0;
        return RN_ERR_HIP;
    }
    return RN_OK;
}

int rn_device_locality(int device, char *pci_bus_id, uint64_t pci_cap, int *numa_node, char *cpulist,
                       uint64_t cpulist_cap)
{
    char addr[32] = {0}, path[128];
    if (numa_node) *numa_node = -1;
    if (cpulist && cpulist_cap) cpulist[0] = 0;
    if (pci_bus_id && pci_cap) pci_bus_id[0] = 0;
    if (hipDeviceGetPCIBusId(addr, (int)sizeof(addr) - 1, device) != hipSuccess) return RN_ERR_HIP;
    for (char *c = addr; *c; ++c)
        if (*c >= 'A' && *c <= 'F') *c = (char)(*c - 'A' + 'a');
    if (pci_bus_id && pci_cap) snprintf(pci_bus_id, (size_t)pci_cap, "%s", addr);
    snprintf(path, sizeof(path), "/sys/bus/pci/devices/%s/numa_node", addr);
    if (FILE *f = fopen(path, "r")) {
        int node = -1;
        if (fscanf(f, "%d", &node) == 1 && numa_node) *numa_node = node;
        fclose(f);
    }
    snprintf(path, sizeof(path), "/sys/bus/pci/devices/%s/local_cpulist", addr);
    if (FILE *f = fopen(path, "r")) {
        if (cpulist && cpulist_cap && fgets(cpulist, (int)cpulist_cap, f)) {
            for (char *c = cpulist; *c; ++c)
                if (*c == '\n') *c = 0;
        }
        fclose(f);
    }
    return RN_OK;
}

int rn_ctx_create(rn_ctx **out, int device, void *hip_stream)
{
    if (!out) return RN_ERR_INVALID;
    *out = nullptr;
    int n = 0;
    if (hipGetDeviceCount(&n) != hipSuccess || n <= 0) return RN_ERR_HIP;
    if (device < 0 || device >= n) return RN_ERR_INVALID;
    if (hipSetDevice(device) != hipSuccess) return RN_ERR_HIP;
    rn_ctx *ctx = (rn_ctx *)calloc(1, sizeof(rn_ctx));
    if (!ctx) return RN_ERR_NOMEM;
    ctx->device = device;
    ctx->cus = 256;
    {
        int v = 0;
        if (hipDeviceGetAttribute(&v, hipDeviceAttributeMultiprocessorCount, device) == hipSuccess && v > 0) ctx->cus = v;
    }
    ctx->layout = RN_LAYOUT_NCHW;
    if (const char *xg = getenv("RN_XCD_NGROUPS")) {
        const int g = atoi(xg);
        if (g == 1 || g == 2 || g == 4 || g == 8) ctx->xcd_groups = g;
    }
    ctx->nchw_taps = 1;
    if (const char *nt = getenv("RN_NCHW_TAPS")) {
        const int v = atoi(nt);
        if (v >= 0 && v <= 2) ctx->nchw_taps = v;
    }
    if (const char *ts = getenv("RN_TAP_SKIP")) {
        const int v = atoi(ts);
        if (v >= 0 && v <= 2) ctx->tap_skip = v;
    }
    if (hip_stream) {
        ctx->stream = (hipStream_t)hip_stream;
        ctx->own_stream = false;
    } else {
        if (hipStreamCreateWithFlags(&ctx->stream, hipStreamNonBlocking) != hipSuccess) {
            free(ctx);
            return RN_ERR_HIP;
        }
        ctx->own_stream = true;
    }
    *out = ctx;
    return RN_OK;
}

int rn_ctx_destroy(rn_ctx *ctx)
{
    if (!ctx) return RN_OK;
    (void)hipSetDevice(ctx->device);
    (void)rn_defer_flush(ctx);
    (void)hipStreamSynchronize(ctx->stream);
    rn_defer_destroy(ctx);
    for (int i = 0; i < 6; ++i) {
        if (ctx->scratch[i]) (void)hipFree(ctx->scratch[i]);
    }
    for (int i = 0; i < ctx->wcache_n; ++i) (void)hipFree(ctx->wcache[i].packed);
    free(ctx->wcache);
    if (ctx->own_stream) (void)hipStreamDestroy(ctx->stream);
    free(ctx);
    return RN_OK;
}

int rn_ctx_set_layout(rn_ctx *ctx, int layout)
{
    if (!ctx) return RN_ERR_INVALID;
    if (layout != RN_LAYOUT_NCHW && layout != RN_LAYOUT_NHWC)
        return rn_set_error(ctx, RN_ERR_INVALID, "unknown layout %d", layout);
    if (ctx->ds && !ctx->defer_running && layout != ctx->layout) {
        RN_TRY(rn_bind_device(ctx));
        RN_TRY(rn_defer_barrier(ctx));
    }
    ctx->layout = layout;
    return RN_OK;
}

int rn_ctx_get_layout(const rn_ctx *ctx) { return ctx ? ctx->layout : -1; }

int rn_ctx_set_sync_each_op(rn_ctx *ctx, int on)
{
    if (!ctx) return RN_ERR_INVALID;
    ctx->sync_each_op = on ? 1 : 0;
    return RN_OK;
}

int rn_ctx_set_conv_tile(rn_ctx *ctx, int candidate)
{
    if (!ctx) return RN_ERR_INVALID;
    if (candidate < 0 || candidate > rn_conv_tile_candidates())
        return rn_set_error(ctx, RN_ERR_INVALID, "conv tile candidate %d out of range", candidate);
    ctx->conv_tile = candidate;
    return RN_OK;
}

int rn_conv_tile_candidates(void) { return 8 + rn_conv_wide_count() + 1; }

int rn_ctx_graphs_live(const rn_ctx *ctx) { return ctx ? ctx->graphs_live : 0; }
int rn_ctx_tap_skip_mode(const rn_ctx *ctx) { return ctx ? ctx->tap_skip : 0; }
int rn_ctx_scratch_slot(rn_ctx *ctx, int slot, uint64_t bytes, void **ptr)
{
    if (!ctx || !ptr) return RN_ERR_INVALID;
    RN_TRY(rn_bind_device(ctx));
    return rn_scratch(ctx, slot, bytes, ptr);
}
int rn_ctx_set_error(rn_ctx *ctx, int status, const char *msg) { return rn_set_error(ctx, status, "%s", msg); }

int rn_ctx_is_capturing(rn_ctx *ctx)
{
    hipStreamCaptureStatus cap = hipStreamCaptureStatusNone;
    if (!ctx || rn_bind_device(ctx) != RN_OK) return 0;
    if (hipStreamIsCapturing(ctx->stream, &cap) != hipSuccess) return 0;
    return cap != hipStreamCaptureStatusNone;
}
int rn_ctx_upload_sync(rn_ctx *ctx, void *dev, const void *host, uint64_t bytes)
{
    if (!ctx || !dev || !host) return RN_ERR_INVALID;
    RN_TRY(rn_bind_device(ctx));
    RN_HIP_TRY(ctx, hipMemcpyAsync(dev, host, bytes, hipMemcpyHostToDevice, ctx->stream));
    RN_HIP_TRY(ctx, hipStreamSynchronize(ctx->stream));
    return RN_OK;
}

int rn_ctx_set_split_k(rn_ctx *ctx, int max_splits)
{
    if (!ctx) return RN_ERR_INVALID;
    if (max_splits < 0 || max_splits > 64)
        return rn_set_error(ctx, RN_ERR_INVALID, "split_k %d out of range [0, 64]", max_splits);
    ctx->split_k = max_splits <= 1 ? 0 : max_splits;
    return RN_OK;
}

int rn_ctx_set_xcd_groups(rn_ctx *ctx, int groups)
{
    if (!ctx) return RN_ERR_INVALID;
    if (groups != 0 && groups != 1 && groups != 2 && groups != 4 && groups != 8)
        return rn_set_error(ctx, RN_ERR_INVALID, "xcd groups %d: 0 (chosen per launch), 1, 2, 4 or 8", groups);
    ctx->xcd_groups = groups;
    return RN_OK;
}

int rn_ctx_set_nchw_taps(rn_ctx *ctx, int mode)
{
    if (!ctx) return RN_ERR_INVALID;
    if (mode < 0 || mode > 2) return rn_set_error(ctx, RN_ERR_INVALID, "nchw taps mode %d: 0 (never), 1 (large planes) or 2 (always)", mode);
    ctx->nchw_taps = mode;
    return RN_OK;
}

int rn_ctx_set_tap_skip(rn_ctx *ctx, int mode)
{
    if (!ctx) return RN_ERR_INVALID;
    if (mode < 0 || mode > 2)
        return rn_set_error(ctx, RN_ERR_INVALID, "tap skip mode %d: 0 (the library's rule), 1 (never) or 2 (wherever eligible)", mode);
    ctx->tap_skip = mode;
    return RN_OK;
}

int rn_ctx_tap_skip_stats(const rn_ctx *ctx, uint64_t *launches, uint64_t *k_tiles_skipped)
{
    if (!ctx) return RN_ERR_INVALID;
    if (launches) *launches = ctx->tap_skip_launches;
    if (k_tiles_skipped) *k_tiles_skipped = ctx->tap_skip_k_tiles;
    return RN_OK;
}

int rn_ctx_set_stem_items(rn_ctx *ctx, int items)
{
    if (!ctx) return RN_ERR_INVALID;
    if (items < 0) return rn_set_error(ctx, RN_ERR_INVALID, "stem items %d: 0 (chosen per launch) or a positive count", items);
    ctx->stem_items = items;
    return RN_OK;
}

int rn_ctx_wait_event(rn_ctx *ctx, rn_event *ev)
{
    if (!ctx || !ev) return RN_ERR_INVALID;
    RN_TRY(rn_bind_device(ctx));
    RN_HIP_TRY(ctx, hipStreamWaitEvent(ctx->stream, ev->ev, 0));
    return RN_OK;
}

uint64_t rn_ctx_launch_count(const rn_ctx *ctx) { return ctx ? ctx->launches : 0; }

int rn_ctx_set_weight_cache(rn_ctx *ctx, int on)
{
    if (!ctx) return RN_ERR_INVALID;
    ctx->wcache_on = on ? 1 : 0;
    if (!on && ctx->wcache_n) {
        RN_TRY(rn_bind_device(ctx));
        rn_wcache_drop(ctx, nullptr, ~(uint64_t)0);
    }
    return RN_OK;
}

int rn_ctx_set_debug_stamps(rn_ctx *ctx, void *dev_buffer)
{
    if (!ctx) return RN_ERR_INVALID;
    ctx->debug_stamps = dev_buffer;
    return RN_OK;
}

void *rn_ctx_stream(rn_ctx *ctx) { return ctx ? (void *)ctx->stream : nullptr; }
int rn_ctx_device(const rn_ctx *ctx) { return ctx ? ctx->device : -1; }

int rn_sync(rn_ctx *ctx)
{
    if (!ctx) return RN_ERR_INVALID;
    RN_TRY(rn_bind_device(ctx));
    RN_TRY(rn_defer_flush(ctx));
    RN_HIP_TRY(ctx, hipStreamSynchronize(ctx->stream));
    RN_HIP_TRY(ctx, hipGetLastError());
    return RN_OK;
}

const char *rn_last_error(const rn_ctx *ctx) { return ctx ? ctx->err : "no context"; }

int rn_malloc(rn_ctx *ctx, void **dev_ptr, uint64_t bytes)
{
    if (!ctx || !dev_ptr) return RN_ERR_INVALID;
    *dev_ptr = nullptr;
    if (bytes == 0) return RN_OK;
    RN_TRY(rn_bind_device(ctx));
    hipError_t e = hipMalloc(dev_ptr, bytes);
    if (e == hipErrorOutOfMemory) {
        (void)hipGetLastError();
        return rn_set_error(ctx, RN_ERR_NOMEM, "hipMalloc(%llu) out of memory",
                            (unsigned long long)bytes);
    }
    return rn_check_hip(ctx, e, "hipMalloc");
}

int rn_free(rn_ctx *ctx, void *dev_ptr)
{
    if (!ctx) return RN_ERR_INVALID;
    RN_TRY(rn_bind_device(ctx));
    if (!dev_ptr) return RN_OK;
    if (ctx->ds) {
        hipDeviceptr_t base = nullptr;
        size_t size = 0;
        if (hipMemGetAddressRange(&base, &size, dev_ptr) == hipSuccess) {
            RN_TRY(rn_defer_before_write(ctx, base, size, 1));
        } else {
            (void)hipGetLastError();
            RN_TRY(rn_defer_before_write(ctx, dev_ptr, 1, 1));
        }
    }
    RN_HIP_TRY(ctx, hipStreamSynchronize(ctx->stream));
    if (ctx->wcache_n) {
        hipDeviceptr_t base = nullptr;
        size_t size = 0;
        if (hipMemGetAddressRange(&base, &size, dev_ptr) == hipSuccess)
            rn_wcache_drop(ctx, base, size);
        else
            (void)hipGetLastError(), rn_wcache_drop(ctx, dev_ptr, 1);
    }
    RN_HIP_TRY(ctx, hipFree(dev_ptr));
    return RN_OK;
}

int rn_memcpy_h2d(rn_ctx *ctx, void *dev_dst, const void *host_src, uint64_t bytes)
{
    if (!ctx || (bytes && (!dev_dst || !host_src))) return RN_ERR_INVALID;
    RN_TRY(rn_bind_device(ctx));
    if (!bytes) return RN_OK;
    if (ctx->ds) RN_TRY(rn_defer_before_write(ctx, dev_dst, bytes, 0));
    if (ctx->wcache_n) rn_wcache_drop(ctx, dev_dst, bytes);
    RN_HIP_TRY(ctx, hipMemcpyAsync(dev_dst, host_src, bytes, hipMemcpyHostToDevice, ctx->stream));
    RN_HIP_TRY(ctx, hipStreamSynchronize(ctx->stream));
    return RN_OK;
}

int rn_memcpy_d2h(rn_ctx *ctx, void *host_dst, const void *dev_src, uint64_t bytes)
{
    if (!ctx || (bytes && (!host_dst || !dev_src))) return RN_ERR_INVALID;
    RN_TRY(rn_bind_device(ctx));
    if (!bytes) return RN_OK;
    if (ctx->ds) RN_TRY(rn_defer_before_read(ctx, dev_src, bytes, &dev_src));
    RN_HIP_TRY(ctx, hipMemcpyAsync(host_dst, dev_src, bytes, hipMemcpyDeviceToHost, ctx->stream));
    RN_HIP_TRY(ctx, hipStreamSynchronize(ctx->stream));
    return RN_OK;
}

int rn_memcpy_d2d(rn_ctx *ctx, void *dev_dst, const void *dev_src, uint64_t bytes)
{
    if (!ctx || (bytes && (!dev_dst || !dev_src))) return RN_ERR_INVALID;
    RN_TRY(rn_bind_device(ctx));
    if (!bytes) return RN_OK;
    if (ctx->ds) {
        RN_TRY(rn_defer_before_read(ctx, dev_src, bytes, nullptr));
        RN_TRY(rn_defer_before_write(ctx, dev_dst, bytes, 0));
    }
    if (ctx->wcache_n) rn_wcache_drop(ctx, dev_dst, bytes);
    RN_HIP_TRY(ctx,
               hipMemcpyAsync(dev_dst, dev_src, bytes, hipMemcpyDeviceToDevice, ctx->stream));
    return RN_OK;
}

int rn_memset(rn_ctx *ctx, void *dev_ptr, int byte_value, uint64_t bytes)
{
    if (!ctx || (bytes && !dev_ptr)) return RN_ERR_INVALID;
    RN_TRY(rn_bind_device(ctx));
    if (!bytes) return RN_OK;
    if (ctx->ds) RN_TRY(rn_defer_before_write(ctx, dev_ptr, bytes, 0));
    if (ctx->wcache_n) rn_wcache_drop(ctx, dev_ptr, bytes);
    RN_HIP_TRY(ctx, hipMemsetAsync(dev_ptr, byte_value, bytes, ctx->stream));
    return RN_OK;
}

int rn_load_f32_file(rn_ctx *ctx, const char *path, float **dev_ptr, uint64_t *numel)
{
    if (!ctx || !path || !dev_ptr || !numel) return RN_ERR_INVALID;
    *dev_ptr = nullptr;
    *numel = 0;
    FILE *f = fopen(path, "rb");
    if (!f) return rn_set_error(ctx, RN_ERR_IO, "Can't open %s: %s", path, strerror(errno));
// ... 97 lines not shown
```

### resnet.c_amd/csrc/rn_internal.h

```cpp
#ifndef RN_INTERNAL_H
#define RN_INTERNAL_H

#include <hip/hip_runtime.h>
#include <stdint.h>
#include <stdio.h>

#include "rn_hip.h"

struct rn_wcache_entry {
    const void *key;
    uint64_t cin, cout, k;
    void *packed;
};

#define RN_CONV_GEMM_KERNELS 59

struct rn_ctx {
    int device;
    int cus;
    hipStream_t stream;
    bool own_stream;
    int layout;
    int sync_each_op;
    int conv_tile;
    int graphs_live;
    int split_k;
    int stem_items;
    int nchw_taps;
    int xcd_groups;
    int tap_skip;
    uint64_t tap_skip_launches, tap_skip_k_tiles;
    void *debug_stamps;
    void *scratch[6];
    uint64_t scratch_bytes[6];
    int occupancy[RN_CONV_GEMM_KERNELS];
    int stem_lds_allowed[5];
    uint64_t launches;
    int wcache_on, wcache_n, wcache_cap;
    struct rn_wcache_entry *wcache;
    int defer;
    int defer_running;
    struct rn_defer_state *ds;
    char err[512];
};

struct rn_event {
    hipEvent_t ev;
};

int rn_set_error(rn_ctx *ctx, int status, const char *fmt, ...);
int rn_bind_device(rn_ctx *ctx);
int rn_check_hip(rn_ctx *ctx, hipError_t e, const char *what);
int rn_scratch(rn_ctx *ctx, int slot, uint64_t bytes, void **ptr);
void *rn_wcache_find(rn_ctx *ctx, const void *weight, uint64_t cin, uint64_t cout, uint64_t k);
int rn_wcache_add(rn_ctx *ctx, const void *weight, uint64_t cin, uint64_t cout, uint64_t k,
                  uint64_t bytes, void **packed);
void rn_wcache_remove(rn_ctx *ctx, const void *packed);
void rn_wcache_drop(rn_ctx *ctx, const void *lo, uint64_t bytes);
int rn_after_launch(rn_ctx *ctx, const char *what);

#define RN_HIP_TRY(ctx, expr)                                  \
    do {                                                       \
        int rn_st_ = rn_check_hip((ctx), (expr), #expr);       \
        if (rn_st_ != RN_OK) return rn_st_;                    \
    } while (0)

int rn_defer_flush(rn_ctx *ctx);
int rn_defer_barrier(rn_ctx *ctx);
int rn_defer_before_write(rn_ctx *ctx, const void *ptr, uint64_t bytes, int whole_allocation);
int rn_defer_before_read(rn_ctx *ctx, const void *ptr, uint64_t bytes, const void **alt);
void rn_defer_destroy(rn_ctx *ctx);
int rn_defer_conv(rn_ctx *ctx, const float *inp, float *out, const float *w, uint64_t k, uint64_t s, uint64_t p,
                  uint64_t ho, uint64_t wo, uint64_t B, uint64_t Cin, uint64_t Cout, uint64_t H, uint64_t W);
int rn_defer_bn(rn_ctx *ctx, const float *inp, float *out, const float *w, const float *b, const float *mean,
                const float *var, uint64_t B, uint64_t C, uint64_t N);
int rn_defer_eltwise(rn_ctx *ctx, int is_add, const float *a, const float *b, float *out, uint64_t N);
int rn_defer_pool(rn_ctx *ctx, int is_max, const float *inp, float *out, uint64_t k, uint64_t s, uint64_t p,
                  uint64_t ho, uint64_t wo, uint64_t B, uint64_t C, uint64_t H, uint64_t W);
int rn_defer_linear(rn_ctx *ctx, const float *inp, float *out, const float *w, const float *b, uint64_t B,
                    uint64_t in_f, uint64_t out_f);
#define RN_DEFERS(ctx) ((ctx)->defer && !(ctx)->defer_running && (ctx)->layout == RN_LAYOUT_NCHW)

#define RN_ENTER(ctx)                                  \
    do {                                               \
        if (!(ctx)) return RN_ERR_INVALID;             \
        int rn_en_ = rn_bind_device(ctx);              \
        if (rn_en_ != RN_OK) return rn_en_;            \
        if ((ctx)->ds && !(ctx)->defer_running) {      \
            rn_en_ = rn_defer_barrier(ctx);            \
            if (rn_en_ != RN_OK) return rn_en_;        \
        }                                              \
    } while (0)

#define RN_TRY(expr)                       \
    do {                                   \
        int rn_st_ = (expr);               \
        if (rn_st_ != RN_OK) return rn_st_; \
    } while (0)

#define RN_REQUIRE(ctx, cond, msg)                                   \
    do {                                                             \
        if (!(cond)) return rn_set_error((ctx), RN_ERR_INVALID, "%s: %s", __func__, (msg)); \
    } while (0)

static inline uint64_t rn_ceil_div(uint64_t a, uint64_t b) { return (a + b - 1) / b; }

static inline unsigned rn_stream_grid(uint64_t work_items, unsigned block)
{
    uint64_t g = rn_ceil_div(work_items, block);
    if (g > 2048) g = 2048;
    if (g == 0) g = 1;
    return (unsigned)g;
}

bool rn_conv_is_c4(uint64_t Cin, uint64_t k);


#endif
```

### resnet.c_amd/csrc/rn_model.c

```c
#include <stdio.h>
#include <stdlib.h>
#include <string.h>

#include "rn_hip.h"
#include "rn_private.h"

#define RN_MAX_KEY 96
#define RN_DEFAULT_SIDE 224
#define RN_MIN_SIDE 32
#define RN_MAX_SIDE 2048
#define RN_RESIZE_SIDE 256
#define RN_STEM_WIDTH 64
#define RN_DEFAULT_CLASSES 1000
#define RN_MAX_CLASSES 65536

#define RN_MAX_STREAMS 4

typedef struct {
    char key[RN_MAX_KEY];
    uint64_t numel;
    float *dev;
    int is_set;
} rn_param;

// ... 774 lines not shown
{
    struct rn_model_share *sh = (struct rn_model_share *)cell;
    if (!sh) return;
    --sh->pipelines;
    if (!sh->model_alive && sh->pipelines == 0) free(sh);
}

void rn_model_graph_ref(rn_model *m, int delta)
{
    if (m) m->graphs_live += delta;
}

int rn_model_set_pair_fusion(rn_model *m, int on)
{
    if (!m) return RN_ERR_INVALID;
    m->pair_fusion = on ? 1 : 0;
    m->tuned_B = 0;
    return RN_OK;
}

int rn_model_set_streams(rn_model *m, int streams)
{
    if (!m || (streams != 0 && streams != 1 && streams != 2 && streams != 4)) return RN_ERR_INVALID;
    if (streams == 0) {
        m->streams = 2;
        m->streams_set = 0;
        return RN_OK;
    }
    m->streams = streams;
    m->streams_set = 1;
    return RN_OK;
}

int rn_model_get_streams(const rn_model *m) { return m ? m->streams : 0; }

static int parts_of(const rn_model *m, uint64_t B);
int rn_model_parts(const rn_model *m, uint64_t B) { return m && B ? parts_of(m, B) : 0; }

int rn_model_set_stem_pool_fusion(rn_model *m, int on)
{
    if (!m) return RN_ERR_INVALID;
    m->stem_pool = on < 0 ? 0 : on > 2 ? 2 : on;
    m->tuned_B = 0;
    return RN_OK;
}

int rn_model_set_chain(rn_model *m, int on)
{
    if (!m) return RN_ERR_INVALID;
    m->chain = on ? 1 : 0;
    return RN_OK;
}

int rn_model_set_front_parts(rn_model *m, int parts)
{
    if (!m || parts < 1 || parts > 16 || (parts & (parts - 1))) return RN_ERR_INVALID;
    m->front_parts = parts;
    m->tuned_B = 0;
    return RN_OK;
}

int rn_model_set_stem_exact(rn_model *m, int on)
{
    if (!m) return RN_ERR_INVALID;
    m->stem_exact = on ? 1 : 0;
    m->tuned_B = 0;
    return RN_OK;
}

int rn_model_profiling_enabled(const rn_model *m) { return m ? m->profiling : 0; }

static int prof_begin(rn_model *m, const char *op, const char *layer, double flops, double bytes)
{
    rn_prof *r;
    if (!m->profiling) return RN_OK;
    if (m->n_prof == m->cap_prof) {
        const uint64_t ncap = m->cap_prof ? m->cap_prof * 2 : 256;
        rn_prof *np = (rn_prof *)realloc(m->prof, ncap * sizeof(rn_prof));
        uint64_t i;
        if (!np) return RN_ERR_NOMEM;
        m->prof = np;
        for (i = m->cap_prof; i < ncap; ++i) {
            int st;
            memset(&np[i], 0, sizeof(rn_prof));
            st = rn_event_create(m->run.ctx, &np[i].start);
            if (st == RN_OK) st = rn_event_create(m->run.ctx, &np[i].stop);
            if (st != RN_OK) {
                m->cap_prof = i;
                return st;
            }
        }
        m->cap_prof = ncap;
    }
    r = &m->prof[m->n_prof];
    r->op = op;
    snprintf(r->layer, RN_MAX_KEY, "%s", layer);
    r->flops = flops;
    r->bytes = bytes;
    r->ms = -1.f;
    return rn_event_record(m->run.ctx, r->start);
}

static int prof_end(rn_model *m)
{
    if (!m->profiling) return RN_OK;
    return rn_event_record(m->run.ctx, m->prof[m->n_prof++].stop);
}

int rn_model_set_profiling(rn_model *m, int on)
{
    if (!m) return RN_ERR_INVALID;
    m->profiling = on ? 1 : 0;
    return RN_OK;
}

uint64_t rn_model_profile_count(const rn_model *m) { return m ? m->n_prof : 0; }

int rn_model_profile_get(const rn_model *m, uint64_t index, const char **op_name,
                         const char **layer_name, float *ms, double *flops, double *bytes)
{
    rn_prof *r;
    if (!m || index >= m->n_prof) return RN_ERR_INVALID;
    r = &m->prof[index];
    if (r->ms < 0.f) {
        int st = rn_event_elapsed_ms(r->start, r->stop, &r->ms);
        if (st != RN_OK) return st;
    }
    if (op_name) *op_name = r->op;
    if (layer_name) *layer_name = r->layer;
    if (ms) *ms = r->ms;
    if (flops) *flops = r->flops;
    if (bytes) *bytes = r->bytes;
    return RN_OK;
}

#define TRY(expr)                   \
    do {                            \
        int st_ = (expr);           \
        if (st_ != RN_OK) return st_; \
    } while (0)

static rn_conv_call *next_call(rn_model *m)
{
    if (m->n_calls == m->cap_calls) {
        const int ncap = 2 * m->cap_calls + 16;
        rn_conv_call *nc = (rn_conv_call *)realloc(m->calls, (size_t)ncap * sizeof(rn_conv_call));
        if (!nc) return NULL;
        m->calls = nc;
        m->cap_calls = ncap;
    }
    return &m->calls[m->n_calls++];
}

static int tuned_tile(const rn_model *m, const int tile[2], const uint64_t tile_B[2], uint64_t B)
{
    if (!m->tuned_B || m->tuned_mode != m->run.mode) return 0;
    return tile_B[0] == B ? tile[0] : tile_B[1] == B ? tile[1] : 0;
}

static int launch_call(const rn_model *m, rn_ctx *ctx, const rn_conv_call *k)
{
    const rn_conv *cv = &m->convs[k->conv];
    const rn_epilogue *ep = k->has_ep ? &k->ep : NULL;
    const uint64_t ho = conv_side(cv, k->H, k->pad), wo = conv_side(cv, k->W, k->pad);
    if (k->pair_block >= 0) {
        const rn_block *pb = &m->blocks[k->pair_block];
        const rn_conv *cd = &m->convs[pb->ds];
        rn_conv_second second;
        second.inp = k->x2; second.in_channels = cd->cin; second.H = k->H2; second.W = k->W2;
        second.stride = cd->stride;
        return rn_conv2d_nhwc_pair_forward_dt(ctx, m->dtype, m->dtype, k->x, k->y, pb->pair_packed, cv->k,
                                              cv->stride, k->pad, ho, wo, k->B, cv->cin, cv->cout, k->H, k->W,
                                              &second, ep);
    }
    if (k->exact)
        return rn_conv2d_nhwc_exact_forward(ctx, (const float *)k->x, (float *)k->y, m->stem_packed_exact, cv->k,
                                            cv->stride, ho, wo, k->B, cv->cin, cv->cout, k->H, k->W, ep);
    if (cv->dil > 1)
        return rn_conv2d_dilated_nhwc_forward_dt(ctx, m->dtype, m->dtype, k->x, k->y, cv->packed, cv->k, cv->stride,
                                                 k->pad, cv->dil, ho, wo, k->B, cv->cin, cv->cout, k->H, k->W,
                                                 cv->groups, ep);
    if (cv->groups > 1)
        return rn_conv2d_grouped_nhwc_forward_dt(ctx, m->dtype, m->dtype, k->x, k->y, cv->packed, cv->k, cv->stride,
                                                 k->pad, ho, wo, k->B, cv->cin, cv->cout, k->H, k->W, cv->groups, ep);
    return rn_conv2d_nhwc_forward_dt(ctx, m->dtype, m->dtype, k->x, k->y, cv->packed, cv->k, cv->stride, k->pad, ho,
                                     wo, k->B, cv->cin, cv->cout, k->H, k->W, ep);
}

static int op_call(rn_model *m, const rn_conv_call *k, const char *op, const char *layer, double flops,
                   double bytes, const int tile[2], const uint64_t tile_B[2])
{
    int st;
    if (m->recording) {
        rn_conv_call *c = next_call(m);
        if (!c) return RN_ERR_NOMEM;
        *c = *k;
    }
    TRY(prof_begin(m, op, layer, flops, bytes));
    rn_ctx_set_conv_tile(m->run.ctx, tuned_tile(m, tile, tile_B, k->B));
    st = launch_call(m, m->run.ctx, k);
    rn_ctx_set_conv_tile(m->run.ctx, 0);
    if (st != RN_OK) return st;
    return prof_end(m);
}

static int op_conv_at(rn_model *m, const rn_conv *cv, const void *x, void *y, uint64_t B, uint64_t H,
                      uint64_t W, const rn_epilogue *ep, uint64_t pad, int exact)
{
    const uint64_t ho = conv_side(cv, H, pad), wo = conv_side(cv, W, pad);
    const double M = (double)(B * ho * wo), K = (double)(cv->cin / cv->groups * cv->k * cv->k);
    const double es = (double)elem_size(m);
    double bytes = es * ((double)(B * H * W * cv->cin) + K * (double)cv->cout +
                         M * (double)cv->cout);
    rn_conv_call k;
    if (ep && ep->residual) bytes += es * M * (double)cv->cout;
    memset(&k, 0, sizeof(k));
    k.conv = (int)(cv - m->convs);
    k.pair_block = -1;
    k.exact = exact;
    k.x = x; k.y = y;
    k.B = B; k.H = H; k.W = W; k.pad = pad;
    k.has_ep = ep != NULL;
    if (ep) k.ep = *ep;
    return op_call(m, &k, ep ? "conv2d+epilogue" : "conv2d", cv->name, 2.0 * M * (double)cv->cout * K, bytes,
                   cv->tile, cv->tile_B);
}

static int op_conv(rn_model *m, const rn_conv *cv, const void *x, void *y, uint64_t B, uint64_t H,
                   uint64_t W, const rn_epilogue *ep)
{
    return op_conv_at(m, cv, x, y, B, H, W, ep, cv->pad, 0);
}

static int op_pair(rn_model *m, rn_block *b, const void *t, const void *x, void *y, uint64_t B,
                   uint64_t H, uint64_t W, uint64_t H2, uint64_t W2)
{
    const rn_conv *c3 = &m->convs[b->tail], *cd = &m->convs[b->ds];
    const double M = (double)(B * H * W), K = (double)(c3->cin * c3->k * c3->k + cd->cin);
    const double es = (double)elem_size(m);
    const double bytes = es * ((double)(B * H * W * c3->cin) + (double)(B * H2 * W2 * cd->cin) +
                               K * (double)c3->cout + M * (double)c3->cout);
    char name[RN_MAX_KEY];
    rn_conv_call k;
    memset(&k, 0, sizeof(k));
    k.conv = b->tail;
    k.pair_block = (int)(b - m->blocks);
    k.x = t; k.x2 = x; k.y = y;
    k.B = B; k.H = H; k.W = W; k.pad = c3->pad; k.H2 = H2; k.W2 = W2;
    k.has_ep = 1;
    k.ep.scale = NULL; k.ep.shift = b->pair_shift; k.ep.residual = NULL; k.ep.relu = 1;
    snprintf(name, sizeof(name), "%.*s+downsample", (int)(RN_MAX_KEY - 12), c3->name);
    return op_call(m, &k, "conv2d+epilogue", name, 2.0 * M * (double)c3->cout * K, bytes, b->pair_tile,
                   b->pair_tile_B);
}

static int chain_applies(const rn_model *m, const rn_block *b, int mode)
{
    const int bi = (int)(b - m->blocks);
    const rn_conv *c3, *n1;
    if (m->basic) return 0;
    c3 = &m->convs[b->conv3];
    if (!m->chain || mode != RN_FWD_FUSED || m->recording) return 0;
    if (b->ds >= 0) {
        const rn_conv *cd = &m->convs[b->ds];
        if (!m->pair_fusion || cd->stride != 1 || cd->cin != 64) return 0;
    }
    if (bi + 1 >= m->n_blocks) return 0;
    if (m->front_parts > 1 && bi + 1 == m->depths[0]) return 0;
    n1 = &m->convs[m->blocks[bi + 1].conv1];
    if (c3->k != 1 || c3->stride != 1 || n1->k != 1 || n1->stride != 1 || n1->cin != c3->cout) return 0;
    if (c3->cin == 64 && c3->cout == 256) return n1->cout == 64 || n1->cout == 128;
    if (m->dtype != RN_DTYPE_BF16 || b->ds >= 0) return 0;
    return c3->cin == 128 && c3->cout == 512 && n1->cout == 128;
}

static int op_chain(rn_model *m, const rn_block *b, const void *t2, const void *shortcut, void *y,
                    uint64_t B, uint64_t H, uint64_t W)
{
    const rn_conv *c3 = &m->convs[b->conv3];
    const rn_conv *n1 = &m->convs[m->blocks[(b - m->blocks) + 1].conv1];
    const double M = (double)(B * H * W), es = (double)elem_size(m);
    char name[RN_MAX_KEY];
    snprintf(name, sizeof(name), "%.*s%s+next.conv1", (int)(RN_MAX_KEY - 24), c3->name, b->ds >= 0 ? "+downsample" : "");
    {
        const double k1 = (double)c3->cin + (b->ds >= 0 ? (double)m->convs[b->ds].cin : 0.0);
        const double op2 = b->ds >= 0 ? (double)m->convs[b->ds].cin : (double)c3->cout;
        TRY(prof_begin(m, "conv2d+epilogue+conv2d", name,
                       2.0 * M * ((double)c3->cout * k1 + (double)n1->cout * (double)n1->cin),
                       es * (M * ((double)c3->cin + op2 + (double)c3->cout + (double)n1->cout) +
                             (double)c3->cout * k1 + (double)(n1->cout * n1->cin))));
    }
    if (b->ds >= 0)
        TRY(rn_conv_chain_pair_forward_dt(m->run.ctx, m->dtype, t2, shortcut, y, b->pair_packed, b->pair_shift,
                                          m->run.t1, n1->packed, n1->scale, n1->shift, B * H * W, c3->cin,
                                          m->convs[b->ds].cin, c3->cout, n1->cout));
    else
        TRY(rn_conv_chain_forward_dt(m->run.ctx, m->dtype, t2, shortcut, y, c3->packed, c3->scale, c3->shift,
                                     m->run.t1, n1->packed, n1->scale, n1->shift, B * H * W, c3->cin,
                                     c3->cout, n1->cout));
    m->run.t1_ready = 1;
    return prof_end(m);
}

static int op_bn(rn_model *m, const rn_conv *cv, float *y, uint64_t B, uint64_t HW)
{
    const double n = (double)(B * cv->cout * HW);
    TRY(prof_begin(m, "batchnorm2d", cv->name, 0.0, 8.0 * n + 16.0 * (double)cv->cout));
    TRY(rn_batchnorm2d_forward(m->run.ctx, y, y, m->params[cv->bn_w].dev, m->params[cv->bn_b].dev,
                               m->params[cv->bn_m].dev, m->params[cv->bn_v].dev, B, cv->cout, HW));
    return prof_end(m);
}

static int op_relu(rn_model *m, const char *layer, float *y, uint64_t n)
{
    TRY(prof_begin(m, "relu", layer, 0.0, 8.0 * (double)n));
    TRY(rn_relu_forward(m->run.ctx, y, y, n));
    return prof_end(m);
}

static int op_add(rn_model *m, const char *layer, float *y, const float *shortcut, uint64_t n)
{
    TRY(prof_begin(m, "add", layer, 0.0, 12.0 * (double)n));
    TRY(rn_add_forward(m->run.ctx, y, shortcut, y, n));
    return prof_end(m);
}

static int op_downsample(rn_model *m, const rn_conv *cd, const float *x, uint64_t B, uint64_t h, uint64_t w,
                         uint64_t HWo)
{
    TRY(op_conv(m, cd, x, m->run.dsb, B, h, w, NULL));
    return op_bn(m, cd, m->run.dsb, B, HWo);
}

static int block_forward(rn_model *m, rn_block *b, const float *x, float *y, uint64_t B,
                         uint64_t *H, uint64_t *W, int mode)
{
    const rn_conv *c1 = &m->convs[b->conv1], *ct = &m->convs[b->tail];
    const rn_conv *c2 = m->basic ? NULL : &m->convs[b->conv2];
    const rn_conv *cd = b->ds >= 0 ? &m->convs[b->ds] : NULL;
    const rn_conv *cs = c2 ? c2 : c1;
    const uint64_t h = *H, w = *W;
    const uint64_t ho = conv_side(cs, h, cs->pad), wo = conv_side(cs, w, cs->pad);
    const uint64_t h1 = c2 ? h : ho, w1 = c2 ? w : wo;
    float *mid = c2 ? m->run.t2 : m->run.t1;
    const float *shortcut = x;
    if (mode == RN_FWD_FUSED) {
        rn_epilogue ep;
        const int pair = cd && m->pair_fusion;
        if (cd && !pair) {
            ep.scale = cd->scale; ep.shift = cd->shift; ep.residual = NULL; ep.relu = 0;
            TRY(op_conv(m, cd, x, m->run.dsb, B, h, w, &ep));
            shortcut = m->run.dsb;
        }
        ep.scale = c1->scale; ep.shift = c1->shift; ep.residual = NULL; ep.relu = 1;
// ... 180 lines not shown
    const int pool = m->fpn_extra && out[n];
    int j;
    for (j = n - 1; j >= 1; --j) TRY(op_fpn(m, RN_FPN_TOPDOWN, j, kFpnTopdownOps[j], NULL, B, NULL));
    for (j = 0; j < n; ++j)
        if (out[j] || (pool && j == n - 1)) TRY(op_fpn(m, RN_FPN_LAYER, j, kFpnLayerOps[j], NULL, B, NULL));
    if (pool) TRY(op_fpn(m, RN_FPN_POOL, n - 1, "fpn_pool", NULL, B, NULL));
    for (j = 0; j <= n; ++j) {
        uint64_t H, W;
        if (j == n ? !pool : !out[j]) continue;
        TRY(rn_fpn_level_shape(m->fpn, j, m->fpn_h[j < n ? j : n - 1], m->fpn_w[j < n ? j : n - 1], NULL, &H, &W));
        TRY(op_fpn(m, RN_FPN_EXPORT, j, j < n ? kFpnExportOps[j] : "fpn_export_pool", NULL, B,
                   out[j] + m->run.img0 * m->fpn_a * H * W));
    }
    return RN_OK;
}

static int run_blocks(rn_model *m, int first, int last, uint64_t B, uint64_t *H, uint64_t *W, int mode)
{
    int bi, li = 0, end = m->depths[0];
    for (bi = first; bi < last; ++bi) {
        TRY(block_forward(m, &m->blocks[bi], block_input(m, bi), block_input(m, bi + 1), B, H, W, mode));
        while (bi >= end) end += m->depths[++li];
        if (m->maps && bi + 1 == end && m->maps->layer[li]) TRY(op_stage_map(m, li, block_input(m, bi + 1), B, *H, *W));
        if (m->seg_head && bi + 1 == m->n_blocks) TRY(op_segment(m, block_input(m, bi + 1), B, *H, *W));
        if (m->fpn && bi + 1 == end) TRY(op_fpn_lateral(m, li, block_input(m, bi + 1), B));
        if (m->fpn && bi + 1 == m->n_blocks) TRY(op_fpn_rest(m, B));
    }
    return RN_OK;
}

static int run_head(rn_model *m, const float *x, uint64_t B, uint64_t H, uint64_t W, float *logits)
{
    const double es = (double)elem_size(m);
    TRY(prof_begin(m, "avgpool2d", "avgpool", 0.0, es * (double)(B * m->feat * (H * W + 1))));
    TRY(rn_global_avgpool_nhwc_forward_dt(m->run.ctx, m->dtype, x, m->run.pooled, B, m->feat, H, W));
    TRY(prof_end(m));
    TRY(prof_begin(m, "linear", "fc", 2.0 * (double)B * (double)m->feat * (double)m->classes,
                   es * ((double)(B * m->feat) + (double)m->feat * (double)m->classes) +
                       4.0 * ((double)m->classes + (double)B * (double)m->classes)));
    if (m->dtype == RN_DTYPE_BF16) {
        rn_epilogue ep;
        ep.scale = NULL; ep.shift = m->params[m->fc_b].dev; ep.residual = NULL; ep.relu = 0;
        TRY(rn_conv2d_nhwc_forward_dt(m->run.ctx, m->dtype, RN_DTYPE_F32, m->run.pooled, logits, m->fc_packed, 1, 1, 0,
                                      1, 1, B, m->feat, m->classes, 1, 1, &ep));
    } else if (m->classes % 4 != 0) {
        TRY(rn_linear_direct_forward(m->run.ctx, m->run.pooled, logits, m->params[m->fc_w].dev,
                                     m->params[m->fc_b].dev, B, m->feat, m->classes));
    } else {
        TRY(rn_linear_forward(m->run.ctx, m->run.pooled, logits, m->params[m->fc_w].dev, m->params[m->fc_b].dev, B,
                              m->feat, m->classes));
    }
    return prof_end(m);
}

static void run_begin(rn_model *m, rn_ctx *ctx, uint64_t img_off, uint64_t slice_off, int mode)
{
    const uint64_t es = elem_size(m);
    const uint64_t p_off = img_off * m->p_img + slice_off * m->s1_img;
    rn_run *r = &m->run;
    img_off += slice_off;
    r->ctx = ctx;
    r->mode = mode;
    r->t1_ready = 0;
    r->img0 = m->maps_done + img_off;
    r->sub0 = img_off;
    r->x4 = (float *)((char *)m->x4 + img_off * m->x4_img * es);
    r->p0 = (float *)((char *)m->p0 + p_off * es);
    r->p1 = (float *)((char *)m->p1 + p_off * es);
    r->dsb = (float *)((char *)m->dsb + img_off * m->ds_img * es);
    r->t1 = (float *)((char *)m->t1 + img_off * m->t1_img * es);
    r->t2 = m->t2 ? (float *)((char *)m->t2 + img_off * m->t2_img * es) : NULL;
    r->pooled = (float *)((char *)m->pooled + img_off * m->feat * es);
}

enum { RN_PHASE_ALL = 0, RN_PHASE_FRONT = 1, RN_PHASE_BACK = 2 };

static int forward_phase(rn_model *m, const void *input, int in_u8, uint64_t B, float *logits, int mode,
                         int phase)
{
    const int first = phase == RN_PHASE_BACK ? m->depths[0] : 0;
    const int last = phase == RN_PHASE_FRONT ? m->depths[0] : m->n_blocks;
    uint64_t H = m->pool_h, W = m->pool_w;
    if (phase != RN_PHASE_BACK) TRY(run_front(m, input, in_u8, B, mode));
    TRY(run_blocks(m, first, last, B, &H, &W, mode));
    if (phase != RN_PHASE_FRONT) TRY(run_head(m, block_input(m, last), B, H, W, logits));
    return RN_OK;
}

static int forward_sub(rn_model *m, rn_ctx *run, uint64_t img_off, uint64_t slice_off, const void *input,
                       int in_u8, uint64_t B, float *logits, int mode, int phase)
{
    const int saved_layout = rn_ctx_get_layout(run);
    int st;
    run_begin(m, run, img_off, slice_off, mode);
    rn_ctx_set_layout(run, RN_LAYOUT_NHWC);
    st = forward_phase(m, input, in_u8, B, logits, mode, phase);
    rn_ctx_set_layout(run, saved_layout);
    return st;
}

#define RN_STREAM_MIN_PART(m) ((m)->dtype == RN_DTYPE_F32 && !(m)->streams_set ? 128u : 64u)

static int parts_of(const rn_model *m, uint64_t B)
{
    int parts = m->streams;
    if (B > m->max_sub) B = m->max_sub;
    while (parts > 1 && B / (uint64_t)parts < RN_STREAM_MIN_PART(m)) parts /= 2;
    return parts;
}
#define RN_FRONT_MIN_SLICE 16

static const void *input_at(const rn_model *m, const void *input, int in_u8, uint64_t lo)
{
    return (const char *)input + lo * 3 * m->H * m->W * (in_u8 ? 1 : sizeof(float));
}

static int forward_part(rn_model *m, rn_ctx *run, uint64_t img_off, const void *input, int in_u8,
                        uint64_t B, float *logits, int mode)
{
    int fp = m->front_parts, j;
    uint64_t lo = 0;
    while (fp > 1 && B / (uint64_t)fp < RN_FRONT_MIN_SLICE) fp /= 2;
    if (fp < 2) return forward_sub(m, run, img_off, 0, input, in_u8, B, logits, mode, RN_PHASE_ALL);
    for (j = 0; j < fp; ++j) {
        const uint64_t hi = B * (uint64_t)(j + 1) / (uint64_t)fp;
        TRY(forward_sub(m, run, img_off, lo, input_at(m, input, in_u8, lo), in_u8, hi - lo, logits, mode,
                        RN_PHASE_FRONT));
        lo = hi;
    }
    return forward_sub(m, run, img_off, 0, input, in_u8, B, logits, mode, RN_PHASE_BACK);
}

static int forward_chunk(rn_model *m, const void *input, int in_u8, uint64_t B, float *logits, int mode,
                         int prof_keep)
{
    uint64_t lo = 0;
    int parts = parts_of(m, B), i;
    TRY(ensure_acts(m, B));
    if (!prof_keep) m->n_prof = 0;
    if (parts < 2 || m->profiling || m->single_stream_only || m->recording)
        return forward_part(m, m->ctx, 0, input, in_u8, B, logits, mode);
    if (!m->ev_fork) TRY(rn_event_create(m->ctx, &m->ev_fork));
    for (i = 0; i < parts - 1; ++i) {
        if (m->ctxn[i]) continue;
        TRY(rn_ctx_create(&m->ctxn[i], rn_ctx_device(m->ctx), NULL));
        TRY(rn_event_create(m->ctxn[i], &m->ev_join[i]));
    }
    TRY(rn_event_record(m->ctx, m->ev_fork));
    for (i = 0; i < parts; ++i) {
        const uint64_t hi = B * (uint64_t)(i + 1) / (uint64_t)parts;
        rn_ctx *run = i == 0 ? m->ctx : m->ctxn[i - 1];
        if (i > 0) {
            TRY(rn_ctx_set_tap_skip(run, rn_ctx_tap_skip_mode(m->ctx)));
            TRY(rn_ctx_wait_event(run, m->ev_fork));
        }
        TRY(forward_part(m, run, lo, input_at(m, input, in_u8, lo), in_u8, hi - lo, logits + lo * m->classes,
                         mode));
        if (i > 0) TRY(rn_event_record(run, m->ev_join[i - 1]));
        lo = hi;
    }
    for (i = 0; i < parts - 1; ++i) TRY(rn_ctx_wait_event(m->ctx, m->ev_join[i]));
    return RN_OK;
}

static int head_outputs(rn_model *m, const rn_model_outputs *o, uint64_t done, uint64_t nb, const float *logits)
{
    const uint64_t C = m->classes;
    m->run.ctx = m->ctx;
    if (o->features) {
        float *dst = o->features + done * m->feat;
        TRY(prof_begin(m, "features", "head", 0.0, (double)(nb * m->feat) * (double)(elem_size(m) + 4)));
        if (m->dtype == RN_DTYPE_BF16)
            TRY(rn_widen_bf16_forward(m->ctx, m->pooled, dst, nb * m->feat));
        else
            TRY(rn_memcpy_d2d(m->ctx, dst, m->pooled, nb * m->feat * sizeof(float)));
        TRY(prof_end(m));
    }
    if (o->k > 0) {
        const double bytes = 4.0 * (double)(nb * C) * (o->probs ? 2.0 : 1.0) + 12.0 * (double)(nb * o->k);
        TRY(prof_begin(m, "softmax_topk", "head", 0.0, bytes));
        TRY(rn_softmax_topk_forward(m->ctx, logits, o->probs ? o->probs + done * C : NULL, o->topk_prob + done * o->k,
                                    o->topk_idx + done * o->k, nb, C, o->k));
        TRY(prof_end(m));
    } else if (o->probs) {
        TRY(prof_begin(m, "softmax", "head", 0.0, 8.0 * (double)(nb * C)));
        TRY(rn_softmax_forward(m->ctx, logits, o->probs + done * C, nb, C));
        TRY(prof_end(m));
    }
    return RN_OK;
}

static int forward_outputs(rn_model *m, const void *input, int in_u8, uint64_t B, float *logits,
                           const rn_model_outputs *outs, int mode, int prof_keep)
{
    uint64_t done = 0;
    if (!m || !input || (!logits && !outs) || B == 0) return RN_ERR_INVALID;
    if (mode != RN_FWD_REFERENCE_OPS && mode != RN_FWD_FUSED) return RN_ERR_INVALID;
    if (!m->finalized) return RN_ERR_INVALID;
    if (m->dtype != RN_DTYPE_F32 && mode != RN_FWD_FUSED) return RN_ERR_UNSUPPORTED;
    if (outs) {
        if (!logits && !outs->features && !outs->probs && outs->k == 0 && !m->maps && !m->seg_head && !m->fpn) return RN_ERR_INVALID;
        if (outs->k > 0 && (!outs->topk_prob || !outs->topk_idx || outs->k > 64 || outs->k > m->classes))
            return RN_ERR_INVALID;
    }
    if (!logits) {
        const uint64_t need = B < m->max_sub ? B : m->max_sub;
        if (need > m->own_logits_cap) {
            if (rn_ctx_is_capturing(m->ctx)) return RN_ERR_UNSUPPORTED;
            if (m->own_logits_cap > 0 && rn_ctx_graphs_live(m->ctx) > 0) return RN_ERR_INVALID;
            if (m->own_logits) TRY(rn_free(m->ctx, m->own_logits));
            m->own_logits = NULL;
            m->own_logits_cap = 0;
            TRY(rn_malloc(m->ctx, (void **)&m->own_logits, need * m->classes * sizeof(float)));
            m->own_logits_cap = need;
        }
    }
    while (done < B) {
        const uint64_t nb = B - done < m->max_sub ? B - done : m->max_sub;
        float *sub = logits ? logits + done * m->classes : m->own_logits;
        m->maps_done = done;
        TRY(forward_chunk(m, input_at(m, input, in_u8, done), in_u8, nb, sub, mode, prof_keep && done == 0));
        if (outs) TRY(head_outputs(m, outs, done, nb, sub));
        done += nb;
    }
    return RN_OK;
}

static int forward_any(rn_model *m, const void *input, int in_u8, uint64_t B, float *logits, int mode,
                       int prof_keep)
{
    return forward_outputs(m, input, in_u8, B, logits, NULL, mode, prof_keep);
}

int rn_model_forward(rn_model *m, const float *input_nchw, uint64_t B, float *logits, int mode)
{
    return forward_any(m, input_nchw, 0, B, logits, mode, 0);
}

int rn_model_forward_u8(rn_model *m, const uint8_t *input_nhwc, uint64_t B, float *logits, int mode)
{
    return forward_any(m, input_nhwc, 1, B, logits, mode, 0);
}

int rn_model_forward_outputs(rn_model *m, const float *input_nchw, uint64_t B, const rn_model_outputs *outs, int mode)
{
    if (!outs) return RN_ERR_INVALID;
    return forward_outputs(m, input_nchw, 0, B, outs->logits, outs, mode, 0);
}

int rn_model_forward_outputs_u8(rn_model *m, const uint8_t *input_nhwc, uint64_t B, const rn_model_outputs *outs,
                                int mode)
{
    if (!outs) return RN_ERR_INVALID;
    return forward_outputs(m, input_nhwc, 1, B, outs->logits, outs, mode, 0);
}

static int forward_maps(rn_model *m, const void *input, int in_u8, uint64_t B, const rn_model_outputs *outs,
                        const rn_model_maps *maps, int mode)
{
    rn_model_outputs none;
    int li, wanted = 0, st;
    if (!m) return RN_ERR_INVALID;
    if (!maps) return rn_ctx_set_error(m->ctx, RN_ERR_INVALID, "rn_model_forward_maps: maps is NULL");
    for (li = 0; li < 4; ++li) {
        if (!maps->layer[li]) continue;
        wanted = 1;
        if ((uintptr_t)maps->layer[li] & 3) {
            char msg[96];
            snprintf(msg, sizeof(msg), "rn_model_forward_maps: the map of layer%d must be 4-byte aligned", li + 1);
            return rn_ctx_set_error(m->ctx, RN_ERR_INVALID, msg);
        }
    }
    if (!wanted && !(outs && (outs->logits || outs->features || outs->probs || outs->k)))
        return rn_ctx_set_error(m->ctx, RN_ERR_INVALID, "rn_model_forward_maps: nothing to write");
    memset(&none, 0, sizeof(none));
    if (!outs) outs = &none;
    m->maps = wanted ? maps : NULL;
    st = forward_outputs(m, input, in_u8, B, outs->logits, outs, mode, 0);
    m->maps = NULL;
    m->maps_done = 0;
    return st;
}

int rn_model_forward_maps(rn_model *m, const float *input_nchw, uint64_t B, const rn_model_outputs *outs,
                          const rn_model_maps *maps, int mode)
{
    return forward_maps(m, input_nchw, 0, B, outs, maps, mode);
}

int rn_model_forward_maps_u8(rn_model *m, const uint8_t *input_nhwc, uint64_t B, const rn_model_outputs *outs,
                             const rn_model_maps *maps, int mode)
{
    return forward_maps(m, input_nhwc, 1, B, outs, maps, mode);
}

static int forward_segment(rn_model *m, rn_seg_head *hd, const void *input, int in_u8, uint64_t B,
                           const rn_model_outputs *outs, const rn_seg_outputs *seg, int mode)
{
    rn_model_outputs none;
    const char *why = NULL;
    uint64_t h = 0, w = 0;
    int st;
    if (!m) return RN_ERR_INVALID;
    if (!seg) return rn_ctx_set_error(m->ctx, RN_ERR_INVALID, "rn_model_forward_segment: seg is NULL");
    if (!seg->labels && !seg->scores)
        return rn_ctx_set_error(m->ctx, RN_ERR_INVALID, "rn_model_forward_segment: seg names nothing (labels and scores are NULL)");
// ... 10 lines not shown
    TRY(rn_model_stage_shape(m, 4, NULL, &h, &w));
    TRY(rn_seg_head_reserve(hd, B < m->max_sub ? B : m->max_sub, h * w));
    memset(&none, 0, sizeof(none));
    if (!outs) outs = &none;
    m->seg_head = hd;
    m->seg = seg;
    st = forward_outputs(m, input, in_u8, B, outs->logits, outs, mode, 0);
    m->seg_head = NULL;
    m->seg = NULL;
    m->maps_done = 0;
    return st;
}

int rn_model_forward_segment(rn_model *m, rn_seg_head *hd, const float *input_nchw, uint64_t B,
                             const rn_model_outputs *outs, const rn_seg_outputs *seg, int mode)
{
    return forward_segment(m, hd, input_nchw, 0, B, outs, seg, mode);
}

int rn_model_forward_segment_u8(rn_model *m, rn_seg_head *hd, const uint8_t *input_nhwc, uint64_t B,
                                const rn_model_outputs *outs, const rn_seg_outputs *seg, int mode)
{
    return forward_segment(m, hd, input_nhwc, 1, B, outs, seg, mode);
}

static int forward_fpn(rn_model *m, rn_fpn *fpn, const void *input, int in_u8, uint64_t B, const rn_model_outputs *outs,
                       const int *stages, const rn_fpn_outputs *fo, int mode)
{
    rn_model_outputs none;
    const char *why = NULL;
    char msg[200];
    uint64_t cin[4], a = 0, h[4], w[4];
    int n = 0, extra = 0, j, wanted = 0, st;
    if (!m) return RN_ERR_INVALID;
    if (!m->finalized) return rn_ctx_set_error(m->ctx, RN_ERR_INVALID, "rn_model_forward_fpn: the model is not finalized");
    if (!rn_fpn_matches(fpn, m->ctx, m->dtype, &why)) {
        snprintf(msg, sizeof(msg), "rn_model_forward_fpn: %s", why);
        return rn_ctx_set_error(m->ctx, RN_ERR_INVALID, msg);
    }
    if (!stages) return rn_ctx_set_error(m->ctx, RN_ERR_INVALID, "rn_model_forward_fpn: stages is NULL");
    if (!fo) return rn_ctx_set_error(m->ctx, RN_ERR_INVALID, "rn_model_forward_fpn: fpn_out is NULL");
    rn_fpn_dims(fpn, &n, &extra, &a, cin);
    for (j = 0; j < n; ++j)
        if (stages[j] < 1 || stages[j] > 4 || (j > 0 && stages[j] <= stages[j - 1]))
            return rn_ctx_set_error(m->ctx, RN_ERR_INVALID, "rn_model_forward_fpn: stages must be ascending, each 1..4");
    for (j = 0; j < n; ++j) {
        uint64_t C = 0;
        TRY(rn_model_stage_shape(m, stages[j], &C, &h[j], &w[j]));
        if (C != cin[j]) {
            snprintf(msg, sizeof(msg), "rn_model_forward_fpn: in_channels of level %d is %llu, layer%d has %llu channels", j,
                     (unsigned long long)cin[j], stages[j], (unsigned long long)C);
            return rn_ctx_set_error(m->ctx, RN_ERR_INVALID, msg);
        }
    }
    for (j = 0; j < n + extra; ++j) {
        if (!fo->level[j]) continue;
        wanted = 1;
        if ((uintptr_t)fo->level[j] & 3) {
            snprintf(msg, sizeof(msg), "rn_model_forward_fpn: fpn_out->level[%d] must be 4-byte aligned", j);
            return rn_ctx_set_error(m->ctx, RN_ERR_INVALID, msg);
        }
    }
    if (!wanted) return rn_ctx_set_error(m->ctx, RN_ERR_INVALID, "rn_model_forward_fpn: nothing wanted (every level is NULL)");
    if (!input || B == 0 || (mode != RN_FWD_REFERENCE_OPS && mode != RN_FWD_FUSED)) return RN_ERR_INVALID;
    if (m->dtype != RN_DTYPE_F32 && mode != RN_FWD_FUSED)
        return rn_ctx_set_error(m->ctx, RN_ERR_UNSUPPORTED, "rn_model_forward_fpn: a bf16 model runs RN_FWD_FUSED only");
    TRY(rn_fpn_reserve(fpn, B < m->max_sub ? B : m->max_sub, h, w));
    memset(&none, 0, sizeof(none));
    if (!outs) outs = &none;
    m->fpn = fpn;
    m->fpn_out = fo;
    m->fpn_n = n, m->fpn_extra = extra, m->fpn_a = a;
    for (j = 0; j < n; ++j) m->fpn_stage[j] = stages[j], m->fpn_h[j] = h[j], m->fpn_w[j] = w[j];
    st = forward_outputs(m, input, in_u8, B, outs->logits, outs, mode, 0);
    m->fpn = NULL;
    m->fpn_out = NULL;
    m->maps_done = 0;
    return st;
}

int rn_model_forward_fpn(rn_model *m, rn_fpn *fpn, const float *input_nchw, uint64_t B, const rn_model_outputs *outs,
                         const int *stages, const rn_fpn_outputs *fpn_out, int mode)
{
    return forward_fpn(m, fpn, input_nchw, 0, B, outs, stages, fpn_out, mode);
}

int rn_model_forward_fpn_u8(rn_model *m, rn_fpn *fpn, const uint8_t *input_nhwc, uint64_t B, const rn_model_outputs *outs,
                            const int *stages, const rn_fpn_outputs *fpn_out, int mode)
{
    return forward_fpn(m, fpn, input_nhwc, 1, B, outs, stages, fpn_out, mode);
}

static int default_size(const rn_model *m) { return m->H == RN_DEFAULT_SIDE && m->W == RN_DEFAULT_SIDE; }

static int images_need_default(rn_model *m)
{
    return rn_ctx_set_error(m->ctx, RN_ERR_UNSUPPORTED,
                            "decoded images are resized to 256 and cropped to 224 x 224: the model's input size is "
                            "another (rn_model_set_input_size); crop them yourself and use rn_model_forward_u8");
}

int rn_model_forward_images_table(rn_model *m, const uint8_t *packed_dev, const void *table_dev, uint64_t B,
                                  double src_bytes, float *logits, int mode)
{
    if (!m || !packed_dev || !table_dev || !logits || B == 0) return RN_ERR_INVALID;
    if (mode != RN_FWD_REFERENCE_OPS && mode != RN_FWD_FUSED) return RN_ERR_INVALID;
    if (!m->finalized) return RN_ERR_INVALID;
    if (m->dtype != RN_DTYPE_F32 && mode != RN_FWD_FUSED) return RN_ERR_UNSUPPORTED;
    if (!default_size(m)) return images_need_default(m);
    if (B > m->crops_cap) {
        if (m->crops_cap > 0 && rn_ctx_graphs_live(m->ctx) > 0) return RN_ERR_INVALID;
        if (m->crops) TRY(rn_free(m->ctx, m->crops));
        m->crops = NULL;
        m->crops_cap = 0;
        TRY(rn_malloc(m->ctx, (void **)&m->crops, B * 3 * RN_DEFAULT_SIDE * RN_DEFAULT_SIDE));
        m->crops_cap = B;
    }
    run_begin(m, m->ctx, 0, 0, mode);
    m->n_prof = 0;
    TRY(prof_begin(m, "image_u8_resize_crop", "input", 0.0,
                   src_bytes + (double)B * 3.0 * RN_DEFAULT_SIDE * RN_DEFAULT_SIDE));
    TRY(rn_image_u8_resize_crop_launch(m->ctx, packed_dev, table_dev, B, m->crops, RN_DEFAULT_SIDE));
    TRY(prof_end(m));
    return forward_any(m, m->crops, 1, B, logits, mode, 1);
}

int rn_model_forward_images_u8(rn_model *m, const uint8_t *packed_dev, const uint64_t *offsets,
                               const uint64_t *heights, const uint64_t *widths, uint64_t B, float *logits, int mode)
{
    const double crop = (double)RN_DEFAULT_SIDE / RN_RESIZE_SIDE;
    uint64_t bytes = 0, i;
    double src_bytes = 0.0;
    void *host, *dev = NULL;
    int st;
    if (!m || !packed_dev || !offsets || !heights || !widths || !logits || B == 0) return RN_ERR_INVALID;
    if (!default_size(m)) return images_need_default(m);
    if (rn_image_u8_resize_crop_table(offsets, heights, widths, B, RN_RESIZE_SIDE, RN_DEFAULT_SIDE, NULL, 0, &bytes) !=
        RN_OK)
        return RN_ERR_INVALID;
    if (rn_ctx_is_capturing(m->ctx)) return RN_ERR_UNSUPPORTED;
    host = malloc(bytes);
    if (!host) return RN_ERR_NOMEM;
    st = rn_image_u8_resize_crop_table(offsets, heights, widths, B, RN_RESIZE_SIDE, RN_DEFAULT_SIDE, host, bytes, &bytes);
    if (st == RN_OK) st = rn_ctx_scratch_slot(m->ctx, 5, bytes, &dev);
    if (st == RN_OK) st = rn_ctx_upload_sync(m->ctx, dev, host, bytes);
    free(host);
    if (st != RN_OK) return st;
    for (i = 0; i < B; ++i) src_bytes += 3.0 * (double)heights[i] * (double)widths[i] * crop * crop;
    return rn_model_forward_images_table(m, packed_dev, dev, B, src_bytes, logits, mode);
}

#define RN_TUNE_ROUNDS 6

static int tune_at(rn_model *m, const float *input_nchw, uint64_t B, float *logits, int mode, int slot)
{
    rn_event *e0 = NULL, *e1 = NULL;
    const int ncand = rn_conv_tile_candidates();
    float cand_ms[64];
    int i, c, r, st;
    if (ncand + 1 > 64) return RN_ERR_INVALID;
    m->single_stream_only = 1;
    m->n_calls = 0;
    m->recording = 1;
    st = rn_model_forward(m, input_nchw, B, logits, mode);
    m->recording = 0;
    m->single_stream_only = 0;
    if (st != RN_OK) return st;
    st = rn_event_create(m->ctx, &e0);
    if (st == RN_OK) st = rn_event_create(m->ctx, &e1);
    for (i = 0; st == RN_OK && i < m->n_calls; ++i) {
        const rn_conv_call *k = &m->calls[i];
        rn_conv *cv = &m->convs[k->conv];
        float best = 1e30f;
        int best_c = 0, seen = 0, j;
        for (j = 0; j < i; ++j)
            seen |= m->calls[j].conv == k->conv && m->calls[j].pair_block == k->pair_block &&
                    m->calls[j].B == k->B;
        if (seen) continue;
        for (c = 0; c <= ncand; ++c) cand_ms[c] = 1e30f;
        for (r = 0; r < RN_TUNE_ROUNDS && st == RN_OK; ++r) {
            for (c = 0; c <= ncand && st == RN_OK; ++c) {
                float t = 0.f;
                rn_ctx_set_conv_tile(m->ctx, c);
                st = rn_event_record(m->ctx, e0);
                if (st == RN_OK) st = launch_call(m, m->ctx, k);
                if (st == RN_OK) st = rn_event_record(m->ctx, e1);
                if (st == RN_OK) st = rn_event_elapsed_ms(e0, e1, &t);
                if (r > 0 && t < cand_ms[c]) cand_ms[c] = t;
            }
        }
        for (c = 0; c <= ncand; ++c) {
            if (cand_ms[c] < best * 0.995f) {
                best = cand_ms[c];
                best_c = c;
            }
        }
        if (k->pair_block >= 0) {
            m->blocks[k->pair_block].pair_tile[slot] = best_c;
            m->blocks[k->pair_block].pair_tile_B[slot] = k->B;
        } else {
            cv->tile[slot] = best_c;
            cv->tile_B[slot] = k->B;
        }
    }
    rn_ctx_set_conv_tile(m->ctx, 0);
    rn_event_destroy(e0);
    rn_event_destroy(e1);
    return st;
}

int rn_model_tune(rn_model *m, const float *input_nchw, uint64_t B, float *logits, int mode)
{
    const uint64_t B_all = B;
    uint64_t Bp;
    int c, st;
    if (!m) return RN_ERR_INVALID;
    if (B > m->max_sub) B = m->max_sub;
    Bp = B;
    {
        const int parts = parts_of(m, B);
        if (parts > 1) Bp = B / (uint64_t)parts;
    }
    m->tuned_B = 0;
    for (c = 0; c < m->n_convs; ++c) m->convs[c].tile_B[0] = m->convs[c].tile_B[1] = 0;
    for (c = 0; c < m->n_blocks; ++c) m->blocks[c].pair_tile_B[0] = m->blocks[c].pair_tile_B[1] = 0;
    st = tune_at(m, input_nchw, Bp, logits, mode, 0);
    if (st == RN_OK && Bp != B) st = tune_at(m, input_nchw, B, logits, mode, 1);
    if (st != RN_OK) return st;
    m->tuned_B = B;
    m->tuned_mode = mode;
    return rn_model_forward(m, input_nchw, B_all, logits, mode);
}

#define RN_TUNING_MAGIC 0x726e54554e453034ull
#define RN_TUNING_HEADER 10

static uint64_t tuning_family(const rn_model *m)
{
    return m->groups == 1 && m->width_per_group == 64 ? 0 : (uint64_t)m->groups << 32 | (uint64_t)m->width_per_group;
}

static uint64_t tuning_size(const rn_model *m)
{
    return m->H == RN_DEFAULT_SIDE && m->W == RN_DEFAULT_SIDE ? 0 : m->H << 32 | m->W;
}

static uint64_t tuning_dilation(const rn_model *m)
{
    const uint64_t flags = (uint64_t)(m->dilate[0] | m->dilate[1] << 1 | m->dilate[2] << 2);
    return flags ? 0xD1ull << 56 | flags : 0;
}

static uint64_t tuning_header(const rn_model *m)
{
    return RN_TUNING_HEADER + (tuning_size(m) ? 1 : 0) + (tuning_dilation(m) ? 1 : 0);
}

static uint64_t tuning_settings(const rn_model *m)
{
    return (uint64_t)m->pair_fusion | (uint64_t)m->stem_exact << 1 | (uint64_t)m->stem_pool << 2 |
           (uint64_t)m->chain << 4 | (uint64_t)m->front_parts << 8;
}

int rn_model_export_tuning(const rn_model *m, uint64_t *words, uint64_t cap, uint64_t *n_words)
{
    uint64_t need, at = 0;
    int c, k;
    if (!m || !n_words) return RN_ERR_INVALID;
    need = tuning_header(m) + 4 * ((uint64_t)m->n_convs + (uint64_t)m->n_blocks);
    *n_words = need;
    if (!words) return RN_OK;
    if (cap < need || !m->tuned_B) return RN_ERR_INVALID;
    words[at++] = RN_TUNING_MAGIC;
    words[at++] = (uint64_t)m->arch;
    words[at++] = (uint64_t)m->dtype;
    words[at++] = tuning_settings(m);
    words[at++] = m->tuned_B;
    words[at++] = (uint64_t)m->tuned_mode;
    words[at++] = (uint64_t)m->n_convs;
    words[at++] = (uint64_t)m->n_blocks;
    words[at++] = (uint64_t)rn_conv_tile_candidates();
    words[at++] = tuning_family(m);
    if (tuning_size(m)) words[at++] = tuning_size(m);
    if (tuning_dilation(m)) words[at++] = tuning_dilation(m);
    for (c = 0; c < m->n_convs; ++c)
        for (k = 0; k < 2; ++k) {
            words[at++] = (uint64_t)m->convs[c].tile[k];
            words[at++] = m->convs[c].tile_B[k];
        }
    for (c = 0; c < m->n_blocks; ++c)
        for (k = 0; k < 2; ++k) {
            words[at++] = (uint64_t)m->blocks[c].pair_tile[k];
            words[at++] = m->blocks[c].pair_tile_B[k];
        }
    return RN_OK;
}

int rn_model_import_tuning(rn_model *m, const uint64_t *words, uint64_t n_words)
{
    uint64_t at;
    int c, k;
    if (!m || !words || n_words < tuning_header(m)) return RN_ERR_INVALID;
    at = tuning_header(m);
    if (words[0] != RN_TUNING_MAGIC || words[1] != (uint64_t)m->arch || words[2] != (uint64_t)m->dtype ||
        words[3] != tuning_settings(m) || words[6] != (uint64_t)m->n_convs || words[7] != (uint64_t)m->n_blocks ||
        words[8] != (uint64_t)rn_conv_tile_candidates() || words[9] != tuning_family(m) ||
        (tuning_size(m) && words[RN_TUNING_HEADER] != tuning_size(m)) ||
        (tuning_dilation(m) && words[at - 1] != tuning_dilation(m)) ||
        n_words != at + 4 * ((uint64_t)m->n_convs + (uint64_t)m->n_blocks))
        return RN_ERR_INVALID;
    for (c = 0; c < m->n_convs + m->n_blocks; ++c)
        if (words[at + 4 * (uint64_t)c] > (uint64_t)rn_conv_tile_candidates() ||
            words[at + 4 * (uint64_t)c + 2] > (uint64_t)rn_conv_tile_candidates())
            return RN_ERR_INVALID;
    for (c = 0; c < m->n_convs; ++c)
        for (k = 0; k < 2; ++k) {
            m->convs[c].tile[k] = (int)words[at++];
            m->convs[c].tile_B[k] = words[at++];
        }
    for (c = 0; c < m->n_blocks; ++c)
        for (k = 0; k < 2; ++k) {
            m->blocks[c].pair_tile[k] = (int)words[at++];
            m->blocks[c].pair_tile_B[k] = words[at++];
        }
    m->tuned_B = words[4];
    m->tuned_mode = (int)words[5];
    return RN_OK;
}
```

### resnet.c_amd/csrc/rn_private.h

```cpp
#ifndef RN_PRIVATE_H
#define RN_PRIVATE_H

#include "rn_hip.h"

#ifdef __cplusplus
extern "C" {
#endif

int rn_ctx_graphs_live(const rn_ctx *ctx);
int rn_ctx_tap_skip_mode(const rn_ctx *ctx);
int rn_ctx_wait_event(rn_ctx *ctx, rn_event *ev);
int rn_ctx_scratch_slot(rn_ctx *ctx, int slot, uint64_t bytes, void **ptr);
int rn_ctx_is_capturing(rn_ctx *ctx);
int rn_ctx_set_error(rn_ctx *ctx, int status, const char *msg);
int rn_ctx_upload_sync(rn_ctx *ctx, void *dev, const void *host, uint64_t bytes);

int rn_linear_direct_forward(rn_ctx *ctx, const float *inp, float *out, const float *weight, const float *bias,
                             uint64_t B, uint64_t in_features, uint64_t out_features);
int rn_widen_bf16_forward(rn_ctx *ctx, const void *src_bf16, float *dst, uint64_t n);

int rn_conv_dense_nhwc_forward_dt(rn_ctx *ctx, int dtype, int out_dtype, const void *inp, void *out,
                                  const void *packed_weight, uint64_t kernel_size, uint64_t stride, uint64_t padding,
                                  uint64_t dilation, uint64_t h_out, uint64_t w_out, uint64_t B, uint64_t in_channels,
                                  uint64_t out_channels, uint64_t H, uint64_t W, const rn_epilogue *epilogue);
int rn_conv_group_forward(rn_ctx *ctx, const float *inp, float *out, const float *weight, uint64_t kernel_size,
                          uint64_t stride, uint64_t padding, uint64_t dilation, uint64_t h_out, uint64_t w_out,
                          uint64_t B, uint64_t in_channels, uint64_t out_channels, uint64_t H, uint64_t W,
                          uint64_t groups);
int rn_conv_group_nhwc_forward_dt(rn_ctx *ctx, int dtype, int out_dtype, const void *inp, void *out,
                                  const void *packed_weight, uint64_t kernel_size, uint64_t stride, uint64_t padding,
                                  uint64_t dilation, uint64_t h_out, uint64_t w_out, uint64_t B, uint64_t in_channels,
                                  uint64_t out_channels, uint64_t H, uint64_t W, uint64_t groups,
                                  const rn_epilogue *epilogue);

int rn_seg_head_matches(const rn_seg_head *hd, uint64_t in_channels, int dtype, const char **why);
void rn_seg_head_dims(const rn_seg_head *hd, uint64_t dims[4]);
int rn_seg_head_plan(const rn_seg_head *hd, uint64_t B, uint64_t h, uint64_t w, uint64_t H, uint64_t W, int want_scores,
                     int want_labels, int step, const char **name, double *flops, double *bytes);
int rn_seg_head_reserve(rn_seg_head *hd, uint64_t images, uint64_t pixels);
int rn_seg_head_step(rn_seg_head *hd, rn_ctx *ctx, int step, const void *x_nhwc, uint64_t img0, uint64_t B, uint64_t h,
                     uint64_t w, uint64_t H, uint64_t W, float *scores_nchw, uint8_t *labels);

enum { RN_FPN_INNER = 0, RN_FPN_TOPDOWN = 1, RN_FPN_LAYER = 2, RN_FPN_POOL = 3, RN_FPN_EXPORT = 4 };
int rn_fpn_matches(const rn_fpn *fpn, const rn_ctx *ctx, int dtype, const char **why);
void rn_fpn_dims(const rn_fpn *fpn, int *n_levels, int *extra, uint64_t *out_channels, uint64_t in_channels[4]);
int rn_fpn_reserve(rn_fpn *fpn, uint64_t images, const uint64_t *h, const uint64_t *w);
void rn_fpn_cost(const rn_fpn *fpn, int kind, int level, uint64_t B, const uint64_t *h, const uint64_t *w, double *flops,
                 double *bytes);
int rn_fpn_step(rn_fpn *fpn, rn_ctx *ctx, int kind, int level, const void *x_nhwc, uint64_t img0, uint64_t B,
                const uint64_t *h, const uint64_t *w, float *dst_nchw);

int rn_stem_pool_applies(int dtype, uint64_t Hp, uint64_t Wp, int nchw);

rn_ctx *rn_model_context(rn_model *m);
int rn_model_profiling_enabled(const rn_model *m);
int rn_model_contexts(rn_model *m, rn_ctx **out, int cap);
void rn_model_graph_ref(rn_model *m, int delta);
void *rn_model_pipeline_attach(rn_model *m);
void rn_model_pipeline_detach(void *cell);
int rn_model_forward_images_table(rn_model *m, const uint8_t *packed_dev, const void *table_dev, uint64_t B,
                                  double src_bytes, float *logits, int mode);

#ifdef __cplusplus
}
#endif

#endif
```

### resnet.c_amd/tensor.py

```python
from __future__ import annotations

import ctypes
import enum
import threading
from functools import reduce
from typing import Optional, Sequence

import numpy as np

from . import _lib as L


class Device(enum.Enum):
    CPU = 0
    GPU = 1


class Shape(tuple):

    def __new__(cls, dims: Sequence[int] = ()):
        return super().__new__(cls, (int(d) for d in dims))

    def numel(self) -> int:
        assert len(self) != 0
        return reduce(lambda a, b: a * b, self, 1)

    def as_tuple(self, n: int) -> tuple:
        if len(self) != n:
            raise ValueError(f"shape {tuple(self)} does not have {n} dimensions")
        return tuple(self)

    def __repr__(self) -> str:
        return "(" + ", ".join(str(d) for d in self) + ")"


class Context:
    def __init__(self, device: int = 0, stream: Optional[int] = None):
        lib = L.lib()
        h = ctypes.c_void_p()
        L.check(lib.rn_ctx_create(ctypes.byref(h), device, stream), "rn_ctx_create")
        self.handle = h
        self.device = device

    def sync(self) -> None:
        L.check(L.lib().rn_sync(self.handle), "rn_sync", self.handle)

    def set_layout(self, layout: int) -> None:
        L.check(L.lib().rn_ctx_set_layout(self.handle, layout), "rn_ctx_set_layout", self.handle)

    def set_sync_each_op(self, on: bool) -> None:
        L.check(L.lib().rn_ctx_set_sync_each_op(self.handle, int(on)), "rn_ctx_set_sync_each_op")

    def set_deferred(self, on: bool) -> None:
        L.check(L.lib().rn_ctx_set_deferred(self.handle, int(on)), "rn_ctx_set_deferred", self.handle)

    def flush(self) -> None:
        L.check(L.lib().rn_flush(self.handle), "rn_flush", self.handle)

    def observe(self, dev_ptr) -> None:
        L.check(L.lib().rn_observe(self.handle, dev_ptr), "rn_observe", self.handle)

    def deferred_stats(self) -> dict:
        import ctypes
        v = [ctypes.c_uint64() for _ in range(5)]
        L.check(L.lib().rn_ctx_deferred_stats(self.handle, *(ctypes.byref(x) for x in v)), "rn_ctx_deferred_stats")
        return dict(zip(("pending_ops", "nhwc_buffers", "fused_launches", "literal_launches", "transposes"),
                        (int(x.value) for x in v)))

    def set_xcd_groups(self, groups: int) -> None:
        L.check(L.lib().rn_ctx_set_xcd_groups(self.handle, int(groups)), "rn_ctx_set_xcd_groups", self.handle)

    def set_nchw_taps(self, mode: int) -> None:
        L.check(L.lib().rn_ctx_set_nchw_taps(self.handle, int(mode)), "rn_ctx_set_nchw_taps", self.handle)

    def set_tap_skip(self, mode: int) -> None:
        L.check(L.lib().rn_ctx_set_tap_skip(self.handle, int(mode)), "rn_ctx_set_tap_skip", self.handle)

    def tap_skip_stats(self) -> dict:
        import ctypes
        n, k = ctypes.c_uint64(), ctypes.c_uint64()
        L.check(L.lib().rn_ctx_tap_skip_stats(self.handle, ctypes.byref(n), ctypes.byref(k)), "rn_ctx_tap_skip_stats")
        return {"launches": int(n.value), "k_tiles_skipped": int(k.value)}

    def set_weight_cache(self, on: bool) -> None:
        L.check(L.lib().rn_ctx_set_weight_cache(self.handle, int(on)), "rn_ctx_set_weight_cache")

    def set_split_k(self, max_splits: int) -> None:
        L.check(L.lib().rn_ctx_set_split_k(self.handle, int(max_splits)), "rn_ctx_set_split_k",
                self.handle)

    def close(self) -> None:
        if self.handle:
            L.lib().rn_ctx_destroy(self.handle)
            self.handle = None


_tls = threading.local()


def get_ctx() -> Context:
    ctx = getattr(_tls, "ctx", None)
    if ctx is None:
        ctx = _tls.ctx = Context(getattr(_tls, "device", 0))
    return ctx


def set_device(device: int) -> None:
    old = getattr(_tls, "ctx", None)
    if old is not None and old.device != device:
        old.close()
        _tls.ctx = None
    _tls.device = device


class _DeviceBuffer:

    def __init__(self, ctx: Context, nbytes: int):
        self.ctx = ctx
        p = ctypes.c_void_p()
        L.check(L.lib().rn_malloc(ctx.handle, ctypes.byref(p), nbytes), "rn_malloc", ctx.handle)
        self.ptr = p.value or 0
        self.nbytes = nbytes

    @classmethod
    def adopt(cls, ctx: Context, ptr: int, nbytes: int) -> "_DeviceBuffer":
        self = cls.__new__(cls)
        self.ctx, self.ptr, self.nbytes = ctx, ptr, nbytes
        return self

    def __del__(self):
        try:
            if self.ptr and self.ctx.handle:
                L.lib().rn_free(self.ctx.handle, self.ptr)
        except Exception:
            pass
        self.ptr = 0


class Tensor:

    dtype = np.float32

    def __init__(self, shape=None, device: Device = Device.CPU, *, layout: int = L.RN_LAYOUT_NCHW,
                 _storage=None):
        if isinstance(shape, Device):
            device, shape = shape, None
        self.device = device
        self.layout = layout
        if shape is None:
            self._shape = Shape((0,))
            self._storage = None
            return
        self._shape = Shape(shape)
        assert len(self._shape) != 0
        if _storage is not None:
            self._storage = _storage
        elif self.numel() == 0:
            self._storage = None
        elif device == Device.CPU:
            self._storage = np.empty(self.numel(), dtype=np.float32)
        else:
            self._storage = _DeviceBuffer(get_ctx(), self.size())

    @staticmethod
    def loadToCpu(file_name: str) -> "Tensor":
        try:
            arr = np.fromfile(file_name, dtype=np.float32)
        except OSError as e:
            raise FileNotFoundError(f"Can't open {file_name}") from e
        assert arr.size > 0
        return Tensor((arr.size,), Device.CPU, _storage=arr)

    @staticmethod
    def loadToCuda(file_name: str) -> "Tensor":
        ctx = get_ctx()
        p, n = ctypes.c_void_p(), ctypes.c_uint64()
        L.check(L.lib().rn_load_f32_file(ctx.handle, file_name.encode(), ctypes.byref(p),
                                         ctypes.byref(n)), "rn_load_f32_file", ctx.handle)
        return Tensor((n.value,), Device.GPU,
                      _storage=_DeviceBuffer.adopt(ctx, p.value, n.value * 4))

    @staticmethod
    def from_numpy(arr: np.ndarray, device: Device = Device.CPU, layout: int = L.RN_LAYOUT_NCHW):
        a = np.ascontiguousarray(arr, dtype=np.float32)
        t = Tensor(a.shape if a.ndim else (1,), Device.CPU, _storage=a.reshape(-1).copy())
        return t.cuda(layout) if device == Device.GPU else t

    def save(self, file_name: str) -> None:
        assert self.device == Device.CPU
        self._storage.tofile(file_name)

    def view(self, new_shape) -> "Tensor":
        new_shape = Shape(new_shape)
        assert len(new_shape) != 0
        assert self._shape.numel() == new_shape.numel()
        return Tensor(new_shape, self.device, layout=self.layout, _storage=self._storage)

    def numel(self) -> int:
        return self._shape.numel()

    def size(self) -> int:
        return self.numel() * 4

    def toDevice(self, new_device: Device, layout: Optional[int] = None) -> "Tensor":
        ctx = get_ctx()
        ctx.sync()
        ret = Tensor(self._shape, new_device, layout=self.layout if layout is None else layout)
        if self.device == Device.CPU and new_device == Device.GPU:
            if self.numel():
                L.check(L.lib().rn_memcpy_h2d(ctx.handle, ret.data(), self._storage.ctypes.data,
                                              self.size()), "rn_memcpy_h2d", ctx.handle)
        elif self.device == Device.GPU and new_device == Device.CPU:
            if self.numel():
                L.check(L.lib().rn_memcpy_d2h(ctx.handle, ret._storage.ctypes.data, self.data(),
                                              self.size()), "rn_memcpy_d2h", ctx.handle)
        else:
            raise RuntimeError("Unsupported device transfer combination")
        return ret

    def cuda(self, layout: Optional[int] = None) -> "Tensor":
        return self.toDevice(Device.GPU, layout)

    def cpu(self) -> "Tensor":
        return self.toDevice(Device.CPU)

    def __bool__(self) -> bool:
        return self._storage is not None

    def shape(self) -> Shape:
        return self._shape

    def data(self):
        if self._storage is None:
            return None
        if self.device == Device.GPU:
# ... 16 lines not shown
```

Baseline: 15330 images/s.

## Add 512-thread eight-wave conv GEMM kernel selected per layer by autotuning

Adds a new conv GEMM kernel that runs 512 threads (eight waves) per block in three tile shapes, with resident-grid and one-block-per-tile variants and support for chunked tails. The per-conv autotuner times these variants against the best four-wave tile and stores the winner in the upper bits of the tuned tile word. The chunked-tail split and tile-order heuristics are generalised to take the slot count and blocks per CU into account. The aim is better latency hiding or reuse on fp32 convolutions, at the cost of extra kernel instantiations and longer tuning.

```diff
diff --git a/include/rn_hip.h b/include/rn_hip.h
--- a/include/rn_hip.h
+++ b/include/rn_hip.h
@@ -62,9 +62,16 @@
                                  uint64_t W, uint64_t kernel_size, uint64_t stride, uint64_t padding,
                                  uint64_t dilation, int tile, uint64_t *m_tiles, uint64_t *k_tiles,
                                  uint64_t *k_tiles_skipped, int *rule);
+#define RN_WAVE8_SHAPE_COUNT 3
+RN_API int rn_ctx_set_wave8(rn_ctx *ctx, int mode);
+RN_API int rn_ctx_wave8_stats(const rn_ctx *ctx, uint64_t *launches);
+RN_API int rn_conv_wave8_plan(int dtype, uint64_t B, uint64_t in_channels, uint64_t out_channels, uint64_t H, uint64_t W,
+                              uint64_t kernel_size, uint64_t stride, uint64_t padding, uint64_t dilation, int shape,
+                              int cus, int *bm, int *bn, int *chunked, uint64_t *tiles, uint64_t *tail_tiles, uint64_t *pieces);
 RN_API int rn_ctx_set_debug_stamps(rn_ctx *ctx, void *dev_buffer);
 RN_API void *rn_ctx_stream(rn_ctx *ctx);
 RN_API int rn_ctx_device(const rn_ctx *ctx);
+RN_API int rn_ctx_compute_units(const rn_ctx *ctx);
 RN_API int rn_sync(rn_ctx *ctx);
 RN_API const char *rn_last_error(const rn_ctx *ctx);
 RN_API const char *rn_status_string(int status);
diff --git a/resnet.c_amd/_lib.py b/resnet.c_amd/_lib.py
--- a/resnet.c_amd/_lib.py
+++ b/resnet.c_amd/_lib.py
@@ -12,6 +12,7 @@
 RN_LAYOUT_NCHW, RN_LAYOUT_NHWC = 0, 1
 RN_FWD_REFERENCE_OPS, RN_FWD_FUSED = 0, 1
 RN_DTYPE_F32, RN_DTYPE_BF16 = 0, 1
+RN_WAVE8_SHAPE_COUNT = 3
 RN_CONV_MAX_DILATION = 1024
 
 u64 = c_uint64
@@ -67,6 +68,10 @@
     "rn_ctx_set_tap_skip": (c_int, [c_void_p, c_int]),
     "rn_ctx_tap_skip_stats": (c_int, [c_void_p, POINTER(u64), POINTER(u64)]),
     "rn_conv_tap_skip_plan": (c_int, [c_int] + [u64] * 9 + [c_int] + [POINTER(u64)] * 3 + [POINTER(c_int)]),
+    "rn_ctx_set_wave8": (c_int, [c_void_p, c_int]),
+    "rn_ctx_compute_units": (c_int, [c_void_p]),
+    "rn_ctx_wave8_stats": (c_int, [c_void_p, POINTER(u64)]),
+    "rn_conv_wave8_plan": (c_int, [c_int] + [u64] * 9 + [c_int, c_int] + [POINTER(c_int)] * 3 + [POINTER(u64)] * 3),
     "rn_ctx_set_debug_stamps": (c_int, [c_void_p, c_void_p]),
     "rn_ctx_stream": (c_void_p, [c_void_p]),
     "rn_ctx_device": (c_int, [c_void_p]),
diff --git a/resnet.c_amd/csrc/rn_conv.hip b/resnet.c_amd/csrc/rn_conv.hip
--- a/resnet.c_amd/csrc/rn_conv.hip
+++ b/resnet.c_amd/csrc/rn_conv.hip
@@ -780,7 +780,7 @@
 }
 
 struct Choice {
-    enum Family { STRIP, WIDE, FOUR_WAVE } family;
+    enum Family { STRIP, WIDE, FOUR_WAVE, EIGHT_WAVE } family;
     int which;
     int BM, BN;
     bool persistent;
@@ -820,6 +820,20 @@
     return c;
 }
 
+Choice choose_eight_wave(int mode, const Choice &c, bool eligible)
+{
+    if (mode < 2 || mode >= 2 + 2 * RN_WAVE8_SHAPES || !eligible || c.family != Choice::FOUR_WAVE) return c;
+    Choice e = c;
+    e.family = Choice::EIGHT_WAVE;
+    e.which = (mode - 2) % RN_WAVE8_SHAPES;
+    e.persistent = mode - 2 < RN_WAVE8_SHAPES;
+    if (e.chunked && e.which == 0) e.which = 1;
+    rn_conv8_tile(e.which, &e.BM, &e.BN);
+    return e;
+}
+
+int blocks_per_cu(const Choice &c) { return c.family == Choice::EIGHT_WAVE ? 2 : tile_blocks_per_cu(c.BM, c.BN); }
+
 Choice choose(const rn_ctx *ctx, const Contraction &d, const GemmParams &p)
 {
     if (d.dt_in == RN_DTYPE_BF16 && d.dt_out == RN_DTYPE_BF16 && ctx->split_k <= 1) {
@@ -854,7 +868,8 @@
             return c;
         }
     }
-    return choose_four_wave(ctx->conv_tile, d, p);
+    const Choice c = choose_four_wave(ctx->conv_tile, d, p);
+    return choose_eight_wave(ctx->wave8, c, rn_conv8_eligible(p, d.dt_in, d.dt_out, ctx->split_k > 1));
 }
 
 struct TapSkipPlan {
@@ -951,15 +966,30 @@
     return RN_OK;
 }
 
-int split_chunked_tail(rn_ctx *ctx, const Contraction &d, int BM, GemmParams &p, FinishParams *fin)
-{
-    p.chunk_L = 2 * (int)rn_ceil_div((uint64_t)p.nk, 16);
-    const int S = (int)rn_ceil_div((uint64_t)p.nk, (uint64_t)p.chunk_L);
-    unsigned tail = p.total_tiles > 256 ? p.total_tiles % 256 : p.total_tiles;
+struct ChunkedTail {
+    int chunk_L, S;
+    unsigned tail;
+};
+
+ChunkedTail plan_chunked_tail(const GemmParams &p, unsigned slots, bool never_cut)
+{
+    ChunkedTail t{};
+    t.chunk_L = 2 * (int)rn_ceil_div((uint64_t)p.nk, 16);
+    const int S = t.S = (int)rn_ceil_div((uint64_t)p.nk, (uint64_t)t.chunk_L);
+    unsigned tail = p.total_tiles > slots ? p.total_tiles % slots : p.total_tiles;
     tail -= tail % (unsigned)p.tiles_n;
-    const bool cut = ctx->split_k <= 1 && tail > 0 && !p.out_nchw &&
-                     rn_ceil_div((uint64_t)tail * S, 256) < (uint64_t)S;
-    if (!cut) return RN_OK;
+    const bool cut = !never_cut && tail > 0 && rn_ceil_div((uint64_t)tail * S, slots) < (uint64_t)S;
+    t.tail = cut ? tail : 0;
+    return t;
+}
+
+int split_chunked_tail(rn_ctx *ctx, const Contraction &d, int BM, unsigned slots, GemmParams &p, FinishParams *fin)
+{
+    const ChunkedTail ct = plan_chunked_tail(p, slots, ctx->split_k > 1 || p.out_nchw);
+    const int S = ct.S;
+    const unsigned tail = ct.tail;
+    p.chunk_L = ct.chunk_L;
+    if (tail == 0) return RN_OK;
     const uint64_t row0 = (uint64_t)((p.total_tiles - tail) / (unsigned)p.tiles_n) * (uint64_t)BM;
     const uint64_t tail_elems = ((uint64_t)p.M - row0) * d.Cout;
     void *ws = nullptr;
@@ -972,7 +1002,7 @@
     return RN_OK;
 }
 
-void choose_tile_order(rn_ctx *ctx, GemmParams &p, unsigned remap_tiles, int BM, int BN)
+void choose_tile_order(rn_ctx *ctx, GemmParams &p, unsigned remap_tiles, int BM, int BN, int per_cu)
 {
     const unsigned tn = (unsigned)p.tiles_n;
     if (tn < 2 || remap_tiles < 8 * tn) return;
@@ -981,7 +1011,7 @@
         const double es = p.w_bytes / ((double)p.Cout * p.Ktot);
         const double w_slab = (double)BN * p.Ktot * es;
         const double a_slab = (double)BM * es * (p.Cs + (p.in2 ? p.Cs2 : 0));
-        const double R = 32.0 * tile_blocks_per_cu(BM, BN);
+        const double R = 32.0 * per_cu;
         const double A = (double)p.in_bytes + (p.in2 ? (double)p.in2_bytes / (p.stride2 * p.stride2) : 0.0);
         const double Wb = (double)p.w_bytes, MB = 1024.0 * 1024.0;
         const double panels = (double)(remap_tiles / tn);
@@ -1068,6 +1098,10 @@
 
 int dispatch(rn_ctx *ctx, const Contraction &d, const Choice &c, const GemmParams &p, bool fp32_partials)
 {
+    if (c.family == Choice::EIGHT_WAVE) {
+        RN_TRY(rn_conv8_launch(ctx, p, c.which, c.persistent, c.chunked));
+        return rn_after_launch(ctx, d.what);
+    }
     const bool xk = d.exact, dual = d.second && !xk;
     const int dt_out = fp32_partials ? RN_DTYPE_F32 : d.dt_out;
     const bool chunk = c.chunked && !fp32_partials, dil = p.dil != 1 && !xk;
@@ -1098,7 +1132,7 @@
             RN_REQUIRE(ctx, split_pixel_major(p, d, c.BM, c.BN), "too many tiles");
             if (c.chunked) p.chunk_L = 2 * (int)rn_ceil_div((uint64_t)p.nk, 16);
             else p.chunk_L = p.nk;
-            choose_tile_order(ctx, p, p.full_tiles, c.BM, c.BN);
+            choose_tile_order(ctx, p, p.full_tiles, c.BM, c.BN, blocks_per_cu(c));
             RN_TRY(dispatch(ctx, d, cp, p, false));
             ctx->tap_skip_launches += 1, ctx->tap_skip_k_tiles += t.k_skipped;
             return RN_OK;
@@ -1113,8 +1147,9 @@
     RN_TRY(split_k_loop(ctx, d, p, &fin));
     const bool k_split = fin.splits > 0;
     if (!k_split) {
-        if (c.chunked) RN_TRY(split_chunked_tail(ctx, d, c.BM, p, &fin));
-        choose_tile_order(ctx, p, p.full_tiles, c.BM, c.BN);
+        if (c.chunked)
+            RN_TRY(split_chunked_tail(ctx, d, c.BM, c.family == Choice::EIGHT_WAVE ? 2u * (unsigned)ctx->cus : 256u, p, &fin));
+        choose_tile_order(ctx, p, p.full_tiles, c.BM, c.BN, blocks_per_cu(c));
     }
     RN_TRY(dispatch(ctx, d, c, p, k_split));
     if (fin.splits == 0) return RN_OK;
@@ -1381,6 +1416,46 @@
     if (k_tiles) *k_tiles = t.k_tiles;
     if (k_tiles_skipped) *k_tiles_skipped = t.k_skipped;
     if (rule) *rule = t.rule ? 1 : 0;
+    return 1;
+}
+
+int rn_conv_wave8_plan(int dtype, uint64_t B, uint64_t in_channels, uint64_t out_channels, uint64_t H, uint64_t W,
+                       uint64_t kernel_size, uint64_t stride, uint64_t padding, uint64_t dilation, int shape, int cus,
+                       int *bm, int *bn, int *chunked, uint64_t *tiles, uint64_t *tail_tiles, uint64_t *pieces)
+{
+    if (bm) *bm = 0;
+    if (bn) *bn = 0;
+    if (chunked) *chunked = 0;
+    if (tiles) *tiles = 0;
+    if (tail_tiles) *tail_tiles = 0;
+    if (pieces) *pieces = 0;
+    if ((dtype != RN_DTYPE_F32 && dtype != RN_DTYPE_BF16) || shape < 0 || shape >= RN_WAVE8_SHAPES || cus < 1 || B == 0 ||
+        in_channels == 0 || out_channels == 0 || kernel_size == 0 || kernel_size > 15 || stride == 0 || dilation == 0)
+        return -1;
+    const uint64_t h_out = rn_conv_output_size_dilated(H, kernel_size, stride, padding, dilation);
+    const uint64_t w_out = rn_conv_output_size_dilated(W, kernel_size, stride, padding, dilation);
+    if (h_out == 0 || w_out == 0) return -1;
+    if (dtype != RN_DTYPE_F32 || in_channels % 32 != 0 ||
+        !gemm_eligible(nullptr, nullptr, nullptr, in_channels, kernel_size, B * H * W * in_channels,
+                       out_channels * kernel_size * kernel_size * in_channels, B * h_out * w_out * out_channels))
+        return 0;
+    Contraction d{};
+    d.dt_in = d.dt_out = dtype;
+    d.k = kernel_size, d.stride = stride, d.pad = padding, d.dil = kernel_size == 1 ? 1 : dilation;
+    d.h_out = h_out, d.w_out = w_out, d.B = B, d.Cin = in_channels, d.Cout = out_channels, d.H = H, d.W = W;
+    rn_ctx none{};
+    GemmParams p = describe(&none, d);
+    const Choice c = choose_eight_wave(2 + shape, choose_four_wave(0, d, p), rn_conv8_eligible(p, dtype, dtype, false));
+    if (c.family != Choice::EIGHT_WAVE || !split_whole_tiles(p, c.BM, c.BN)) return 0;
+    if (bm) *bm = c.BM;
+    if (bn) *bn = c.BN;
+    if (chunked) *chunked = c.chunked ? 1 : 0;
+    if (tiles) *tiles = p.total_tiles;
+    if (c.chunked) {
+        const ChunkedTail ct = plan_chunked_tail(p, 2u * (unsigned)cus, false);
+        if (tail_tiles) *tail_tiles = ct.tail;
+        if (pieces) *pieces = (uint64_t)ct.tail * (uint64_t)ct.S;
+    }
     return 1;
 }
 
diff --git a/resnet.c_amd/csrc/rn_conv8.hip b/resnet.c_amd/csrc/rn_conv8.hip
--- /dev/null
+++ b/resnet.c_amd/csrc/rn_conv8.hip
@@ -0,0 +1,379 @@
+#include <type_traits>
+
+#include "rn_conv_params.h"
+#include "rn_private.h"
+
+using namespace rn_gemm;
+
+namespace {
+
+constexpr int ROW_FLOATS = 32;
+constexpr int THREADS = 512;
+constexpr int STAMP_SLOT = 15;
+
+template <int BM, int BN, bool CHUNK>
+__global__ __launch_bounds__(THREADS, 4) void conv_gemm8_kernel(const GemmParams p)
+{
+    constexpr int WC = BM == 64 ? 4 : 2;
+    constexpr int WN = BN / WC;
+    constexpr int NI = WN / 32;
+    constexpr int AP = BM / 64;
+    constexpr int BP = BN / 64;
+    constexpr int STAGE = (BM + BN) * ROW_FLOATS;
+    static_assert(BM * BN <= 2 * STAGE, "the staged C tile reuses the two operand stages");
+    __shared__ __attribute__((aligned(16))) float lds[2 * STAGE];
+
+    __builtin_amdgcn_s_setprio(3);
+    stamp(p.stamps, STAMP_SLOT);
+    const unsigned total_tiles = CHUNK ? p.full_tiles : p.total_tiles;
+    auto logical_origin = [&](unsigned logical, int &m0_, int &n0_) {
+        n0_ = (int)(logical % (unsigned)p.tiles_n) * BN;
+        m0_ = (int)(logical / (unsigned)p.tiles_n) * BM;
+    };
+    auto tile_origin = [&](unsigned v, int &m0_, int &n0_) {
+        unsigned pos = xcd_deal(total_tiles, v);
+        if (p.xg > 0) {
+            const unsigned xg = (unsigned)p.xg, per_group = p.xrows * xg;
+            if (pos < p.xrows * (unsigned)p.tiles_n) {
+                const unsigned grp = pos / per_group, rem = pos - grp * per_group;
+                const unsigned mp = rem / xg, nn = rem - mp * xg;
+                pos = mp * (unsigned)p.tiles_n + grp * xg + nn;
+            }
+        }
+        logical_origin(pos, m0_, n0_);
+    };
+    auto work_item = [&](unsigned v, int &m0_, int &n0_, int &kb_, int &ke_, int &s_) {
+        if constexpr (CHUNK) {
+            if (v >= p.full_tiles) {
+                const unsigned qq = v - p.full_tiles, chunk = qq / p.tail_tiles;
+                logical_origin(p.full_tiles + (qq - chunk * p.tail_tiles), m0_, n0_);
+                kb_ = (int)chunk * p.chunk_L;
+                ke_ = min(kb_ + p.chunk_L, p.nk);
+                s_ = (int)chunk;
+                return;
+            }
+        }
+        tile_origin(v, m0_, n0_);
+        kb_ = 0;
+        ke_ = p.nk;
+        s_ = -1;
+    };
+    unsigned vtile = blockIdx.x;
+    int m0, n0, kb, ke, ks_idx;
+    work_item(vtile, m0, n0, kb, ke, ks_idx);
+
+    const int t = threadIdx.x;
+    const int c = t & 7;
+    const int r0 = t >> 3;
+
+    const __amdgpu_buffer_rsrc_t rsrc_a = make_rsrc(p.in, p.in_bytes);
+    const __amdgpu_buffer_rsrc_t rsrc_b = make_rsrc(p.w, p.w_bytes);
+
+    int a_off[AP], a_mask[AP], b_off[BP];
+    auto setup_rows = [&](int m0_, int n0_) {
+#pragma unroll
+        for (int j = 0; j < AP; ++j) {
+            const int m = m0_ + r0 + 64 * j;
+            if (m < p.M) {
+                const auto [b, oh, ow] = row_of(m, p);
+                const int ih0 = oh * p.stride - p.pad;
+                const int iw0 = ow * p.stride - p.pad;
+                a_off[j] = (((b * p.H + ih0) * p.W + iw0) * p.Cs + c * 4) * 4;
+                const int rlo = max(0, -ih0), rhi = min(p.KH, p.H - ih0);
+                const int rm = rhi > rlo ? ((1 << rhi) - 1) & ~((1 << rlo) - 1) : 0;
+                const int clo = max(0, -iw0), chi = min(p.KW, p.W - iw0);
+                const int cm = chi > clo ? ((1 << chi) - 1) & ~((1 << clo) - 1) : 0;
+                a_mask[j] = rm | (cm << 16);
+            } else {
+                a_off[j] = 0;
+                a_mask[j] = 0;
+            }
+        }
+#pragma unroll
+        for (int j = 0; j < BP; ++j) {
+            const int n = n0_ + r0 + 64 * j;
+            b_off[j] = n < p.Cout ? (n * p.Ktot + c * 4) * 4 : kOob;
+        }
+    };
+    setup_rows(m0, n0);
+
+    u32x4 ra[AP], rb[BP];
+    int a_cur[AP];
+
+    auto load_tile = [&](int kt, u32x4 (&xa)[AP], u32x4 (&xb)[BP], auto first_c) {
+        constexpr bool first = decltype(first_c)::value;
+        const unsigned s_kt = (unsigned)__builtin_amdgcn_readfirstlane(kt);
+        const TapSeg ts = tap_of(s_kt, p);
+        if (first || ts.seg == 0) {
+            const TapRowCol rc = tap_row_col(ts.tap, p);
+            const int toff = (rc.kh * p.W + rc.kw) * p.Cs * 4;
+#pragma unroll
+            for (int j = 0; j < AP; ++j) {
+                const bool ok = ((a_mask[j] >> rc.kh) & (a_mask[j] >> (16 + rc.kw)) & 1) != 0;
+                a_cur[j] = ok ? a_off[j] + toff : kOob;
+            }
+        }
+        const int seg = ts.seg * 128;
+#pragma unroll
+        for (int j = 0; j < AP; ++j) xa[j] = __builtin_amdgcn_raw_buffer_load_b128(rsrc_a, a_cur[j], seg, 0);
+        const int soff = (int)s_kt * 128;
+#pragma unroll
+        for (int j = 0; j < BP; ++j) xb[j] = __builtin_amdgcn_raw_buffer_load_b128(rsrc_b, b_off[j], soff, 0);
+    };
+
+    float *const stage_base = lds + r0 * ROW_FLOATS + RN_SWZ(c, r0) * 4;
+    auto store_tile = [&](auto buf_c, const u32x4 (&xa)[AP], const u32x4 (&xb)[BP]) {
+        constexpr int buf = decltype(buf_c)::value;
+#pragma unroll
+        for (int j = 0; j < AP; ++j)
+            *reinterpret_cast<u32x4 *>(stage_base + buf * STAGE + 64 * j * ROW_FLOATS) = xa[j];
+#pragma unroll
+        for (int j = 0; j < BP; ++j)
+            *reinterpret_cast<u32x4 *>(stage_base + buf * STAGE + (BM + 64 * j) * ROW_FLOATS) = xb[j];
+    };
+    using Buf0 = std::integral_constant<int, 0>;
+    using Buf1 = std::integral_constant<int, 1>;
+
+    const int lane = t & 63, wave = t >> 6;
+    const int wr = wave / WC, wc = wave % WC;
+    const int li = lane & 31, lh = lane >> 5;
+
+    f32x16 acc[NI];
+    [[maybe_unused]] f32x16 tot[CHUNK ? NI : 1];
+    [[maybe_unused]] auto fold_acc = [&](bool have_total) {
+        if constexpr (CHUNK) {
+#pragma unroll
+            for (int ni = 0; ni < NI; ++ni)
+#pragma unroll
+                for (int e = 0; e < 16; ++e) {
+                    const float t_ = have_total ? tot[ni][e] + acc[ni][e] : acc[ni][e];
+                    tot[ni][e] = t_;
+                    acc[ni][e] = 0.f;
+                }
+        }
+    };
+    [[maybe_unused]] auto finish_acc = [&]() {
+        if constexpr (CHUNK) {
+#pragma unroll
+            for (int ni = 0; ni < NI; ++ni)
+#pragma unroll
+                for (int e = 0; e < 16; ++e) acc[ni][e] = tot[ni][e] + acc[ni][e];
+        }
+    };
+
+    const float *frag_a[4], *frag_b[4];
+#pragma unroll
+    for (int ks = 0; ks < 4; ++ks) {
+        const int pc = RN_SWZ(2 * ks + lh, li) * 4;
+        frag_a[ks] = lds + (wr * 32 + li) * ROW_FLOATS + pc;
+        frag_b[ks] = lds + BM * ROW_FLOATS + (wc * WN + li) * ROW_FLOATS + pc;
+    }
+    auto compute_tile = [&](auto buf_c) {
+        constexpr int buf = decltype(buf_c)::value;
+        __builtin_amdgcn_s_setprio(0);
+#pragma unroll
+        for (int ks = 0; ks < 4; ++ks) {
+            u32x4 b[NI];
+            const u32x4 a = *reinterpret_cast<const u32x4 *>(frag_a[ks] + buf * STAGE);
+#pragma unroll
+            for (int ni = 0; ni < NI; ++ni)
+                b[ni] = *reinterpret_cast<const u32x4 *>(frag_b[ks] + buf * STAGE + ni * 32 * ROW_FLOATS);
+#pragma unroll
+            for (int ni = 0; ni < NI; ++ni)
+#pragma unroll
+                for (int j = 0; j < 4; ++j)
+                    acc[ni] = __builtin_amdgcn_mfma_f32_32x32x2f32(__uint_as_float(a[j]), __uint_as_float(b[ni][j]),
+                                                                   acc[ni], 0, 0, 0);
+        }
+        __builtin_amdgcn_s_setprio(3);
+    };
+
+    constexpr int EPT = OutVec<float>::EPT;
+    constexpr int CV = BN / EPT;
+    constexpr int RPP = THREADS / CV;
+    constexpr int PASSES = BM / RPP;
+    const int cv0 = t % CV, rr0 = t / CV;
+    const bool vec = (p.Cout % EPT) == 0;
+    const bool has_scale = p.scale != nullptr, has_shift = p.shift != nullptr;
+    const bool has_res = p.residual != nullptr;
+    const __amdgpu_buffer_rsrc_t rsrc_r = make_rsrc(has_res ? p.residual : p.out, has_res ? p.out_bytes : 0);
+    const __amdgpu_buffer_rsrc_t rsrc_sc = make_rsrc(has_scale ? (const void *)p.scale : p.out, has_scale ? p.Cout * 4 : 0);
+    const __amdgpu_buffer_rsrc_t rsrc_sh = make_rsrc(has_shift ? (const void *)p.shift : p.out, has_shift ? p.Cout * 4 : 0);
+
+    load_tile(kb, ra, rb, std::true_type{});
+    for (;;) {
+#pragma unroll
+        for (int ni = 0; ni < NI; ++ni)
+#pragma unroll
+            for (int e = 0; e < 16; ++e) acc[ni][e] = 0.f;
+        store_tile(Buf0{}, ra, rb);
+        __syncthreads();
+
+        const unsigned vnext = vtile + gridDim.x;
+        const bool has_next = vnext < p.total_work;
+        int m0n = 0, n0n = 0, kbn = 0, ken = 0, ksn = 0;
+        {
+            int kt = kb;
+            [[maybe_unused]] int fold_at = kb + p.chunk_L;
+            [[maybe_unused]] bool folded = false;
+            while (kt + 2 < ke) {
+                if constexpr (CHUNK) {
+                    if (kt == fold_at) {
+                        fold_acc(folded);
+                        folded = true;
+                        fold_at += p.chunk_L;
+                    }
+                }
+                load_tile(kt + 1, ra, rb, std::false_type{});
+                compute_tile(Buf0{});
+                store_tile(Buf1{}, ra, rb);
+                __syncthreads();
+                load_tile(kt + 2, ra, rb, std::false_type{});
+                compute_tile(Buf1{});
+                store_tile(Buf0{}, ra, rb);
+                __syncthreads();
+                kt += 2;
+            }
+            if constexpr (CHUNK) {
+                if (kt == fold_at) {
+                    fold_acc(folded);
+                    folded = true;
+                }
+            }
+            if (kt + 1 < ke) {
+                load_tile(kt + 1, ra, rb, std::false_type{});
+                compute_tile(Buf0{});
+                store_tile(Buf1{}, ra, rb);
+                __syncthreads();
+                compute_tile(Buf1{});
+            } else {
+                compute_tile(Buf0{});
+            }
+            if constexpr (CHUNK) {
+                if (folded) finish_acc();
+            }
+            __syncthreads();
+        }
+        if (has_next) {
+            work_item(vnext, m0n, n0n, kbn, ken, ksn);
+            setup_rows(m0n, n0n);
+            load_tile(kbn, ra, rb, std::true_type{});
+        }
+
+        int cv = cv0, rr = rr0;
+        asm volatile("" : "+v"(cv), "+v"(rr));
+        const int n = n0 + cv * EPT;
+        float *Cs = lds;
+#pragma unroll
+        for (int ni = 0; ni < NI; ++ni)
+            RN_STAGE_ACC(Cs + (wr * 32 + 4 * lh) * BN + wc * WN + ni * 32 + li, acc[ni], BN)
+        u32x4 resv[PASSES], scv, shv;
+        {
+            const bool col_ok = vec && n < p.Cout;
+            scv = __builtin_amdgcn_raw_buffer_load_b128(rsrc_sc, col_ok ? n * 4 : kOob, 0, 0);
+            shv = __builtin_amdgcn_raw_buffer_load_b128(rsrc_sh, col_ok ? n * 4 : kOob, 0, 0);
+#pragma unroll
+            for (int ps = 0; ps < PASSES; ++ps) {
+                const int m = m0 + rr + ps * RPP;
+                resv[ps] = __builtin_amdgcn_raw_buffer_load_b128(
+                    rsrc_r, (col_ok && m < p.M) ? (m * p.Cout + n) * 4 : kOob, 0, 0);
+            }
+        }
+        __syncthreads();
+
+        const bool raw = CHUNK && ks_idx >= 0;
+        void *const out_base = raw ? static_cast<char *>(p.ws) + (long long)ks_idx * p.ws_stride : p.out;
+        const __amdgpu_buffer_rsrc_t rsrc_o = make_rsrc(out_base, p.out_bytes);
+        if (vec) {
+            float sc[EPT], sh[EPT];
+#pragma unroll
+            for (int j = 0; j < 4; ++j) {
+                sc[j] = (has_scale && !raw) ? __uint_as_float(scv[j]) : 1.f;
+                sh[j] = (has_shift && !raw) ? __uint_as_float(shv[j]) : -0.f;
+            }
+            const bool col_ok = n < p.Cout;
+            auto rows_out = [&](auto with_res, auto with_relu) {
+                constexpr bool RES = decltype(with_res)::value, RELU = decltype(with_relu)::value;
+#pragma unroll
+                for (int ps = 0; ps < PASSES; ++ps) {
+                    const int row = rr + ps * RPP;
+                    const int m = m0 + row;
+                    RN_EPILOGUE_ROW(float, RES, RELU, Cs + row * BN + cv * EPT, resv[ps], sc, sh, v)
+                    const int off = (col_ok && m < p.M) ? (m * p.Cout + n) * 4 : kOob;
+                    __builtin_amdgcn_raw_buffer_store_b128(OutVec<float>::pack(v), rsrc_o, off, 0, 0);
+                }
+            };
+            const bool do_res = has_res && !raw, do_relu = p.relu && !raw;
+            RN_WITH_RES_RELU(do_res, do_relu, rows_out(with_res, with_relu))
+        } else if (n < p.Cout) {
+            for (int ps = 0; ps < PASSES; ++ps) {
+                const int row = rr + ps * RPP;
+                const int m = m0 + row;
+                if (m >= p.M) continue;
+                for (int j = 0; j < EPT; ++j) {
+                    if (n + j >= p.Cout) break;
+                    const size_t o = (size_t)m * p.Cout + n + j;
+                    float y = Cs[row * BN + cv * EPT + j];
+                    y = fmaf(y, has_scale ? p.scale[n + j] : 1.f, has_shift ? p.shift[n + j] : -0.f);
+                    if (has_res) y += OutVec<float>::load1(p.residual, o);
+                    y = p.relu ? fmaxf(y, 0.f) : y;
+                    OutVec<float>::store1(out_base, o, y);
+                }
+            }
+        }
+        if (!has_next) break;
+        __syncthreads();
+        vtile = vnext;
+        m0 = m0n;
+        n0 = n0n;
+        kb = kbn;
+        ke = ken;
+        ks_idx = ksn;
+    }
+}
+
+constexpr int kShapes[RN_WAVE8_SHAPES][2] = {{128, 128}, {128, 64}, {64, 128}};
+
+template <int BM, int BN, bool CHUNK>
+void launch_one(rn_ctx *ctx, const GemmParams &p, bool persistent, int *occupancy)
+{
+    unsigned grid = p.grid_items;
+    if (persistent) {
+        if (*occupancy == 0) {
+            int nb = 0;
+            if (hipOccupancyMaxActiveBlocksPerMultiprocessor(&nb, conv_gemm8_kernel<BM, BN, CHUNK>, THREADS, 0) !=
+                    hipSuccess ||
+                nb < 1)
+                nb = 1;
+            *occupancy = nb;
+        }
+        const unsigned slots = (unsigned)ctx->cus * (unsigned)*occupancy;
+        if (grid > slots) grid = slots;
+    }
+    conv_gemm8_kernel<BM, BN, CHUNK><<<dim3(grid), dim3(THREADS), 0, ctx->stream>>>(p);
+}
+
+}
+
+void rn_conv8_tile(int shape, int *bm, int *bn) { *bm = kShapes[shape][0], *bn = kShapes[shape][1]; }
+
+bool rn_conv8_eligible(const GemmParams &p, int dt_in, int dt_out, bool split_k)
+{
+    return dt_in == RN_DTYPE_F32 && dt_out == RN_DTYPE_F32 && p.Cs % 32 == 0 && p.chunk_dw == 0 && p.kreal == 0 &&
+           p.in2 == nullptr && p.dil == 1 && !p.out_nchw && !split_k;
+}
+
+int rn_conv8_launch(rn_ctx *ctx, const GemmParams &p, int shape, bool persistent, bool chunked)
+{
+    int *occ = &ctx->wave8_occupancy[2 * shape + (chunked ? 1 : 0)];
+    switch (2 * shape + (chunked ? 1 : 0)) {
+    case 0: launch_one<128, 128, false>(ctx, p, persistent, occ); break;
+    case 2: launch_one<128, 64, false>(ctx, p, persistent, occ); break;
+    case 3: launch_one<128, 64, true>(ctx, p, persistent, occ); break;
+    case 4: launch_one<64, 128, false>(ctx, p, persistent, occ); break;
+    case 5: launch_one<64, 128, true>(ctx, p, persistent, occ); break;
+    default: return rn_set_error(ctx, RN_ERR_UNSUPPORTED, "eight-wave contraction: no chunked 128x128 form");
+    }
+    ctx->wave8_launches[shape] += 1;
+    return RN_OK;
+}
diff --git a/resnet.c_amd/csrc/rn_conv_params.h b/resnet.c_amd/csrc/rn_conv_params.h
--- a/resnet.c_amd/csrc/rn_conv_params.h
+++ b/resnet.c_amd/csrc/rn_conv_params.h
@@ -104,6 +104,10 @@
 bool rn_conv_strip_eligible(const rn_gemm::GemmParams &p);
 void rn_conv_strip_launch(rn_ctx *ctx, const rn_gemm::GemmParams &p);
 
+bool rn_conv8_eligible(const rn_gemm::GemmParams &p, int dt_in, int dt_out, bool split_k);
+void rn_conv8_tile(int shape, int *bm, int *bn);
+int rn_conv8_launch(rn_ctx *ctx, const rn_gemm::GemmParams &p, int shape, bool persistent, bool chunked);
+
 bool rn_conv_nchw_eligible(uint64_t kernel_size, uint64_t stride, uint64_t padding, uint64_t B, uint64_t Cin,
                            uint64_t Cout, uint64_t H, uint64_t W);
 int rn_conv_nchw_launch(rn_ctx *ctx, const float *inp, float *out, const float *weight, uint64_t kernel_size,
diff --git a/resnet.c_amd/csrc/rn_ctx.hip b/resnet.c_amd/csrc/rn_ctx.hip
--- a/resnet.c_amd/csrc/rn_ctx.hip
+++ b/resnet.c_amd/csrc/rn_ctx.hip
@@ -209,6 +209,10 @@
         const int v = atoi(ts);
         if (v >= 0 && v <= 2) ctx->tap_skip = v;
     }
+    if (const char *w8 = getenv("RN_WAVE8")) {
+        const int v = atoi(w8);
+        if (v >= 0 && v < 2 + 2 * RN_WAVE8_SHAPES) ctx->wave8 = v;
+    }
     if (hip_stream) {
         ctx->stream = (hipStream_t)hip_stream;
         ctx->own_stream = false;
@@ -275,6 +279,7 @@
 
 int rn_ctx_graphs_live(const rn_ctx *ctx) { return ctx ? ctx->graphs_live : 0; }
 int rn_ctx_tap_skip_mode(const rn_ctx *ctx) { return ctx ? ctx->tap_skip : 0; }
+int rn_ctx_wave8_mode(const rn_ctx *ctx) { return ctx ? ctx->wave8 : 0; }
 int rn_ctx_scratch_slot(rn_ctx *ctx, int slot, uint64_t bytes, void **ptr)
 {
     if (!ctx || !ptr) return RN_ERR_INVALID;
@@ -339,6 +344,27 @@
     if (!ctx) return RN_ERR_INVALID;
     if (launches) *launches = ctx->tap_skip_launches;
     if (k_tiles_skipped) *k_tiles_skipped = ctx->tap_skip_k_tiles;
+    return RN_OK;
+}
+
+int rn_ctx_compute_units(const rn_ctx *ctx) { return ctx ? ctx->cus : 0; }
+
+int rn_ctx_set_wave8(rn_ctx *ctx, int mode)
+{
+    if (!ctx) return RN_ERR_INVALID;
+    if (mode < 0 || mode >= 2 + 2 * RN_WAVE8_SHAPES)
+        return rn_set_error(ctx, RN_ERR_INVALID,
+                            "wave8 mode %d: 0 (the library's decision), 1 (never), 2 + s (shape s, resident grid) or %d + s "
+                            "(shape s, one block per tile), s < %d",
+                            mode, 2 + RN_WAVE8_SHAPES, RN_WAVE8_SHAPES);
+    ctx->wave8 = mode;
+    return RN_OK;
+}
+
+int rn_ctx_wave8_stats(const rn_ctx *ctx, uint64_t *launches)
+{
+    if (!ctx || !launches) return RN_ERR_INVALID;
+    for (int s = 0; s < RN_WAVE8_SHAPES; ++s) launches[s] = ctx->wave8_launches[s];
     return RN_OK;
 }
 
diff --git a/resnet.c_amd/csrc/rn_internal.h b/resnet.c_amd/csrc/rn_internal.h
--- a/resnet.c_amd/csrc/rn_internal.h
+++ b/resnet.c_amd/csrc/rn_internal.h
@@ -15,6 +15,8 @@
 
 #define RN_CONV_GEMM_KERNELS 59
 
+#define RN_WAVE8_SHAPES RN_WAVE8_SHAPE_COUNT
+
 struct rn_ctx {
     int device;
     int cus;
@@ -30,6 +32,9 @@
     int xcd_groups;
     int tap_skip;
     uint64_t tap_skip_launches, tap_skip_k_tiles;
+    int wave8;
+    uint64_t wave8_launches[RN_WAVE8_SHAPES];
+    int wave8_occupancy[2 * RN_WAVE8_SHAPES];
     void *debug_stamps;
     void *scratch[6];
     uint64_t scratch_bytes[6];
diff --git a/resnet.c_amd/csrc/rn_model.c b/resnet.c_amd/csrc/rn_model.c
--- a/resnet.c_amd/csrc/rn_model.c
+++ b/resnet.c_amd/csrc/rn_model.c
@@ -950,6 +950,10 @@
     return &m->calls[m->n_calls++];
 }
 
+#define TILE_OF(word) ((word) & 0xff)
+#define WAVE8_OF(word) ((word) >> 8)
+#define RN_WAVE8_MODES (2 + 2 * RN_WAVE8_SHAPE_COUNT)
+
 static int tuned_tile(const rn_model *m, const int tile[2], const uint64_t tile_B[2], uint64_t B)
 {
     if (!m->tuned_B || m->tuned_mode != m->run.mode) return 0;
@@ -995,9 +999,14 @@
         *c = *k;
     }
     TRY(prof_begin(m, op, layer, flops, bytes));
-    rn_ctx_set_conv_tile(m->run.ctx, tuned_tile(m, tile, tile_B, k->B));
-    st = launch_call(m, m->run.ctx, k);
-    rn_ctx_set_conv_tile(m->run.ctx, 0);
+    {
+        const int tuned = tuned_tile(m, tile, tile_B, k->B), user8 = rn_ctx_wave8_mode(m->run.ctx);
+        rn_ctx_set_conv_tile(m->run.ctx, TILE_OF(tuned));
+        if (user8 == 0 && WAVE8_OF(tuned)) rn_ctx_set_wave8(m->run.ctx, WAVE8_OF(tuned));
+        st = launch_call(m, m->run.ctx, k);
+        rn_ctx_set_conv_tile(m->run.ctx, 0);
+        rn_ctx_set_wave8(m->run.ctx, user8);
+    }
     if (st != RN_OK) return st;
     return prof_end(m);
 }
@@ -1484,6 +1493,7 @@
         rn_ctx *run = i == 0 ? m->ctx : m->ctxn[i - 1];
         if (i > 0) {
             TRY(rn_ctx_set_tap_skip(run, rn_ctx_tap_skip_mode(m->ctx)));
+            TRY(rn_ctx_set_wave8(run, rn_ctx_wave8_mode(m->ctx)));
             TRY(rn_ctx_wait_event(run, m->ev_fork));
         }
         TRY(forward_part(m, run, lo, input_at(m, input, in_u8, lo), in_u8, hi - lo, logits + lo * m->classes,
@@ -1800,10 +1810,11 @@
 
 #define RN_TUNE_ROUNDS 6
 
-static int tune_at(rn_model *m, const float *input_nchw, uint64_t B, float *logits, int mode, int slot)
+static int tune_at(rn_model *m, const float *input_nchw, uint64_t B, float *logits, int mode, int slot, int alone)
 {
     rn_event *e0 = NULL, *e1 = NULL;
     const int ncand = rn_conv_tile_candidates();
+    const int user8 = rn_ctx_wave8_mode(m->ctx);
     float cand_ms[64];
     int i, c, r, st;
     if (ncand + 1 > 64) return RN_ERR_INVALID;
@@ -1843,6 +1854,33 @@
                 best_c = c;
             }
         }
+        if (st == RN_OK && alone && user8 == 0 && m->dtype == RN_DTYPE_F32 && k->pair_block < 0 && !k->exact && cv->dil <= 1 &&
+            cv->groups <= 1 && cv->cin % 32 == 0) {
+            float w8_ms[RN_WAVE8_MODES], ref_ms = 1e30f;
+            int w, best_w = 0;
+            for (w = 0; w < RN_WAVE8_MODES; ++w) w8_ms[w] = 1e30f;
+            for (r = 0; r < RN_TUNE_ROUNDS && st == RN_OK; ++r) {
+                for (w = 1; w < RN_WAVE8_MODES && st == RN_OK; ++w) {
+                    float t = 0.f;
+                    rn_ctx_set_conv_tile(m->ctx, best_c);
+                    rn_ctx_set_wave8(m->ctx, w);
+                    st = rn_event_record(m->ctx, e0);
+                    if (st == RN_OK) st = launch_call(m, m->ctx, k);
+                    if (st == RN_OK) st = rn_event_record(m->ctx, e1);
+                    if (st == RN_OK) st = rn_event_elapsed_ms(e0, e1, &t);
+                    if (r > 0 && t < w8_ms[w]) w8_ms[w] = t;
+                }
+            }
+            rn_ctx_set_wave8(m->ctx, 0);
+            ref_ms = w8_ms[1] < best ? w8_ms[1] : best;
+            for (w = 2; w < RN_WAVE8_MODES; ++w) {
+                if (w8_ms[w] < ref_ms * 0.99f) {
+                    ref_ms = w8_ms[w];
+                    best_w = w;
+                }
+            }
+            best_c |= best_w << 8;
+        }
         if (k->pair_block >= 0) {
             m->blocks[k->pair_block].pair_tile[slot] = best_c;
             m->blocks[k->pair_block].pair_tile_B[slot] = k->B;
@@ -1872,8 +1910,8 @@
     m->tuned_B = 0;
     for (c = 0; c < m->n_convs; ++c) m->convs[c].tile_B[0] = m->convs[c].tile_B[1] = 0;
     for (c = 0; c < m->n_blocks; ++c) m->blocks[c].pair_tile_B[0] = m->blocks[c].pair_tile_B[1] = 0;
-    st = tune_at(m, input_nchw, Bp, logits, mode, 0);
-    if (st == RN_OK && Bp != B) st = tune_at(m, input_nchw, B, logits, mode, 1);
+    st = tune_at(m, input_nchw, Bp, logits, mode, 0, Bp == B);
+    if (st == RN_OK && Bp != B) st = tune_at(m, input_nchw, B, logits, mode, 1, 1);
     if (st != RN_OK) return st;
     m->tuned_B = B;
     m->tuned_mode = mode;
@@ -1958,9 +1996,12 @@
         n_words != at + 4 * ((uint64_t)m->n_convs + (uint64_t)m->n_blocks))
         return RN_ERR_INVALID;
     for (c = 0; c < m->n_convs + m->n_blocks; ++c)
-        if (words[at + 4 * (uint64_t)c] > (uint64_t)rn_conv_tile_candidates() ||
-            words[at + 4 * (uint64_t)c + 2] > (uint64_t)rn_conv_tile_candidates())
-            return RN_ERR_INVALID;
+        for (k = 0; k < 2; ++k) {
+            const uint64_t word = words[at + 4 * (uint64_t)c + 2 * (uint64_t)k];
+            if (TILE_OF(word) > (uint64_t)rn_conv_tile_candidates() || WAVE8_OF(word) >= RN_WAVE8_MODES ||
+                WAVE8_OF(word) == 1)
+                return RN_ERR_INVALID;
+        }
     for (c = 0; c < m->n_convs; ++c)
         for (k = 0; k < 2; ++k) {
             m->convs[c].tile[k] = (int)words[at++];
diff --git a/resnet.c_amd/csrc/rn_private.h b/resnet.c_amd/csrc/rn_private.h
--- a/resnet.c_amd/csrc/rn_private.h
+++ b/resnet.c_amd/csrc/rn_private.h
@@ -9,6 +9,7 @@
 
 int rn_ctx_graphs_live(const rn_ctx *ctx);
 int rn_ctx_tap_skip_mode(const rn_ctx *ctx);
+int rn_ctx_wave8_mode(const rn_ctx *ctx);
 int rn_ctx_wait_event(rn_ctx *ctx, rn_event *ev);
 int rn_ctx_scratch_slot(rn_ctx *ctx, int slot, uint64_t bytes, void **ptr);
 int rn_ctx_is_capturing(rn_ctx *ctx);
diff --git a/resnet.c_amd/tensor.py b/resnet.c_amd/tensor.py
--- a/resnet.c_amd/tensor.py
+++ b/resnet.c_amd/tensor.py
@@ -81,6 +81,18 @@
         n, k = ctypes.c_uint64(), ctypes.c_uint64()
         L.check(L.lib().rn_ctx_tap_skip_stats(self.handle, ctypes.byref(n), ctypes.byref(k)), "rn_ctx_tap_skip_stats")
         return {"launches": int(n.value), "k_tiles_skipped": int(k.value)}
+
+    def set_wave8(self, mode: int) -> None:
+        L.check(L.lib().rn_ctx_set_wave8(self.handle, int(mode)), "rn_ctx_set_wave8", self.handle)
+
+    def compute_units(self) -> int:
+        return int(L.lib().rn_ctx_compute_units(self.handle))
+
+    def wave8_stats(self) -> list:
+        import ctypes
+        n = (ctypes.c_uint64 * L.RN_WAVE8_SHAPE_COUNT)()
+        L.check(L.lib().rn_ctx_wave8_stats(self.handle, n), "rn_ctx_wave8_stats")
+        return [int(x) for x in n]
 
     def set_weight_cache(self, on: bool) -> None:
         L.check(L.lib().rn_ctx_set_weight_cache(self.handle, int(on)), "rn_ctx_set_weight_cache")
```

Result: slower. 15130 images/s (-1.3%).
